# goruck/radar-ml

Hardware: AMD Instinct MI355X
Metric: radar frames/s (3D-proj->SVM) (higher is better)
Workload: dtype f32 volumes -> u8 codes, i8 MFMA (exact int32 dot), f64 epilogue; 1 GPU; configs[2]: max-projection + RBF-SVM decision_function, 3-class, 2562 SVs, batch 65536 frames/GPU of 64x64x128 f32 resident in HBM; parallelism=single GPU, global_frames=65536

## Files before the change

include/radarml.h:

```cpp
#ifndef RADARML_H
#define RADARML_H

#include <stdint.h>
#include <stddef.h>

#ifdef __cplusplus
extern "C" {
#endif

typedef enum rml_status {
    RML_OK = 0,
    RML_ERR_INVALID = -1,
    RML_ERR_UNSUPPORTED = -2,
    RML_ERR_HIP = -3,
    RML_ERR_NOMEM = -4,
    RML_ERR_STATE = -5
} rml_status;

typedef struct rml_ctx rml_ctx;
typedef struct rml_svm rml_svm;
typedef struct rml_linear rml_linear;

#define RML_MODE_MAX   0
#define RML_MODE_SLICE 1
#define RML_MODE_SUM   2
#define RML_MODE_MAX_NAN 3

#define RML_VOL_F32    0
#define RML_VOL_U8     1

#define RML_MASK_XZ 1u
#define RML_MASK_YZ 2u
#define RML_MASK_XY 4u
#define RML_MASK_ALL 7u

#define RML_KERNEL_RBF    0
#define RML_KERNEL_LINEAR 1

#define RML_PATH_AUTO  0
#define RML_PATH_F32   1
#define RML_PATH_I8    2
#define RML_PATH_F64   3
#define RML_PATH_DIGITS 4

const char* rml_version(void);
const char* rml_last_error(void);

int rml_ctx_create(int device, rml_ctx** out);
int rml_ctx_destroy(rml_ctx* ctx);
int rml_ctx_device(const rml_ctx* ctx);

#define RML_OPT_PROJECT_SHARE_CU 1
#define RML_OPT_WAVEFRAME 2
#define RML_OPT_LINPLANE 3
#define RML_OPT_STAGE_CODES 4
#define RML_OPT_SLICE_WAVE 5
#define RML_OPT_DERIVE_FUSED 6
#define RML_OPT_CODE_RMW 7
#define RML_OPT_GEMM_BIG 8
#define RML_OPT_CHUNK 9
#define RML_OPT_C1_PK 10
#define RML_OPT_SMO_LDS_ROWS 11
#define RML_SMO_LDS_ROWS_MAX 2768
#define RML_OPT_SGD_RESIDENT_D 12
#define RML_SGD_RESIDENT_D_MAX 10240
#define RML_OPT_CONV7 13
#define RML_CONV7_DEFAULT 3
#define RML_OPT_ZOOM_ROWS 14
int rml_ctx_set_option(rml_ctx* ctx, int option, int value);
int rml_ctx_get_option(const rml_ctx* ctx, int option, int* value);

int rml_ctx_reserve_workspace(rml_ctx* ctx, int64_t bytes);
int64_t rml_ctx_workspace_bytes(const rml_ctx* ctx);

int rml_profile_enable(rml_ctx* ctx, int on);
int rml_profile_read(rml_ctx* ctx, int64_t* launches, double* total_ms, int64_t* frames);
int rml_profile_read_gemm(rml_ctx* ctx, int64_t* launches, double* total_ms, double* ops);

int rml_probe_stream(rml_ctx* ctx, const void* buf, int64_t bytes, int reps, double* gb_per_s, void* stream);

int rml_code_rmw_default(int64_t D, int64_t frame_bytes, int derive, int u8);

int64_t rml_feature_len(int X, int Y, int Z, uint32_t mask);

int rml_project(rml_ctx* ctx, const void* V, int vdtype, int64_t B, int X, int Y, int Z, int mode,
                const int32_t* ijk, float scale_div, uint32_t mask,
                float* feat, int64_t ld_feat,
                uint8_t* feat_q, int64_t ld_q, int32_t* row_isum, int64_t* row_isq, int32_t* row_flags,
                void* stream);

int rml_project_slices(rml_ctx* ctx, const void* V, int vdtype, int64_t B, int X, int Y, int Z, int T,
                       const int32_t* ijk, float scale_div, uint32_t mask,
                       float* feat, int64_t ld_feat,
                       uint8_t* feat_q, int64_t ld_q, int32_t* row_isum, int64_t* row_isq, int32_t* row_flags,
                       void* stream);

int rml_project_planes(rml_ctx* ctx, const void* V, int vdtype, int64_t B, int X, int Y, int Z, int mode,
                       const int32_t* ijk, float* xz, float* yz, float* xy, void* stream);

int rml_derive_targets(rml_ctx* ctx, const void* V, int vdtype, int64_t B, int X, int Y, int Z,
                       int num_targets, int32_t* ijk, float* profiles, void* stream);

int rml_derive_slice(rml_ctx* ctx, const void* V, int vdtype, int64_t B, int X, int Y, int Z, int num_targets,
                     int32_t* ijk, float* profiles, float scale_div, uint32_t mask,
                     float* feat, int64_t ld_feat,
                     uint8_t* feat_q, int64_t ld_q, int32_t* row_isum, int64_t* row_isq, int32_t* row_flags,
                     void* stream);
int rml_derive_slice_supported(const rml_ctx* ctx, const void* V, int vdtype, int X, int Y, int Z, int num_targets);

int rml_assemble_features(rml_ctx* ctx, const float* xz, const float* yz, const float* xy,
                          int64_t B, int X, int Y, int Z, float scale_div, uint32_t mask,
                          float* feat, int64_t ld_feat, void* stream);

int rml_zoom_features(rml_ctx* ctx, const float* xz, const float* yz, const float* xy,
                      int64_t B, int X, int Y, int Z, const int32_t* out_shape,
                      float scale_div, uint32_t mask, float* feat, int64_t ld_feat, void* stream);

int rml_project_zoom(rml_ctx* ctx, const void* V, int vdtype, int64_t B, int X, int Y, int Z, int mode, const int32_t* ijk, int T,
                     const int32_t* out_shape, float scale_div, uint32_t mask, float* feat, int64_t ld_feat, void* stream);

int rml_quantize_rows(rml_ctx* ctx, const float* feat, int64_t N, int64_t D, int64_t ld_feat,
                      float scale_div, uint8_t* feat_q, int64_t ld_q,
                      int32_t* row_isum, int64_t* row_isq, int32_t* row_flags, void* stream);

int rml_svm_load(rml_ctx* ctx, const double* sv, int64_t M, int64_t D,
                 const double* dual_coef, const double* intercept, const int32_t* n_support,
                 int n_classes, int kernel, double gamma, double code_scale ,
                 const double* calib_a, const double* calib_b, rml_svm** out);
int rml_svm_free(rml_ctx* ctx, rml_svm* m);
int rml_svm_is_exact(const rml_svm* m);
int64_t rml_svm_num_sv(const rml_svm* m);
int64_t rml_svm_dim(const rml_svm* m);

int rml_svm_decision(rml_ctx* ctx, const rml_svm* m, int path,
// ... 277 lines not shown
```

radar-ml_amd/_lib.py:

```python
import ctypes as C
import os
import threading

HERE = os.path.dirname(os.path.abspath(__file__))
LIB_PATH = os.environ.get("RML_LIB") or os.path.join(HERE, "libradarml_hip.so")


class RadarMLError(RuntimeError):
    pass


_lib = None
_lock = threading.RLock()
_ctx = {}

c_void_p, c_int, c_int64, c_uint32, c_uint64, c_float, c_double = (
    C.c_void_p, C.c_int, C.c_int64, C.c_uint32, C.c_uint64, C.c_float, C.c_double)

SIGNATURES = {
    "rml_version": (C.c_char_p, []),
    "rml_last_error": (C.c_char_p, []),
    "rml_ctx_create": (c_int, [c_int, C.POINTER(c_void_p)]),
    "rml_ctx_destroy": (c_int, [c_void_p]),
    "rml_ctx_device": (c_int, [c_void_p]),
# ... 105 lines not shown
                                  c_void_p, c_void_p, c_float, c_int, c_void_p, c_void_p, c_int64, c_void_p]),
    "rml_dense_tail_lrelu_f32": (c_int, [c_void_p, c_void_p, c_int64, c_int64, c_int64, c_void_p, c_void_p, c_void_p, c_void_p, c_void_p,
                                         c_void_p, c_int, c_float, c_void_p, c_int64, c_void_p, c_void_p]),
    "rml_dnn_train_supported":(c_int, [c_int, c_int, c_int]),
    "rml_dnn_train_workspace_bytes": (c_int64, [c_int, c_int, c_int, c_int]),
    "rml_dnn_train_step": (c_int, [c_void_p, c_void_p, c_void_p, c_void_p, c_void_p, c_void_p, c_int, c_int64, c_int, c_int, c_void_p, c_int,
                                   c_void_p, c_void_p, c_int, c_uint64, c_int64, c_float, c_int, c_void_p, c_int64, c_void_p, c_void_p,
                                   c_void_p, c_void_p]),
    "rml_dnn_dropout_mask": (c_int, [c_uint64, c_int64, c_int, c_int, c_int, c_float, c_void_p]),
    "rml_bn_workspace_floats": (c_int64, [c_void_p, c_int]),
    "rml_bn_lrelu_pad_forward": (c_int, [c_void_p, c_void_p, c_int, c_int64, c_int, c_int, c_int, c_int, c_int, c_void_p, c_void_p,
                                         c_float, c_float, c_float, c_void_p, c_void_p, c_void_p, c_void_p, c_void_p, c_void_p, c_void_p]),
    "rml_bn_lrelu_pad_backward": (c_int, [c_void_p, c_void_p, c_void_p, c_int, c_int64, c_int, c_int, c_int, c_int, c_int, c_void_p,
                                          c_void_p, c_void_p, c_void_p, c_float, c_void_p, c_void_p, c_void_p, c_void_p, c_void_p]),
    "rml_conv1_bn_lrelu_pad_forward": (c_int, [c_void_p, c_void_p, c_void_p, c_int, c_int64, c_int, c_int, c_int, c_int, c_int, c_void_p,
                                               c_void_p, c_float, c_float, c_float, c_void_p, c_void_p, c_void_p, c_void_p, c_void_p,
                                               c_void_p, c_void_p, c_void_p]),
    "rml_conv1_bn_lrelu_pad_backward": (c_int, [c_void_p, c_void_p, c_void_p, c_void_p, c_int, c_int64, c_int, c_int, c_int, c_int, c_int,
                                                c_void_p, c_void_p, c_void_p, c_void_p, c_void_p, c_float, c_void_p, c_void_p, c_void_p,
                                                c_void_p, c_void_p]),
    "rml_conv7_tanh_supported": (c_int, [c_int, c_int, c_int]),
    "rml_conv7_workspace_floats": (c_int64, [c_void_p, c_int64, c_int, c_int, c_int]),
    "rml_conv7_tanh_forward": (c_int, [c_void_p, c_void_p, c_int, c_int64, c_int, c_int, c_int, c_void_p, c_void_p, c_void_p, c_void_p]),
    "rml_conv7_tanh_backward": (c_int, [c_void_p, c_void_p, c_void_p, c_void_p, c_int, c_int64, c_int, c_int, c_int, c_void_p, c_void_p,
                                        c_void_p, c_void_p, c_void_p, c_void_p]),
    "rml_gen_up_supported": (c_int, [c_int, c_int, c_int]),
    "rml_gen_up_forward": (c_int, [c_void_p, c_void_p, c_int, c_int64, c_int, c_int, c_int, c_void_p, c_void_p, c_void_p, c_void_p]),
    "rml_sgan_generate_workspace_bytes": (c_int64, [c_int64, c_int, c_int, c_int]),
    "rml_sgan_generate": (c_int, [c_void_p, c_void_p, c_int64, c_int, c_int, c_int, c_int, c_int, c_void_p, c_void_p, c_void_p, c_void_p,
                                  c_void_p, c_void_p, c_void_p, c_void_p, c_void_p, c_void_p, c_int64, c_void_p]),
    "rml_conv3s2_supported": (c_int, [c_int, c_int, c_int, c_int]),
    "rml_conv3s2_workspace_bytes": (c_int64, [c_void_p, c_int64, c_int, c_int, c_int, c_int, c_int]),
    "rml_conv3s2_forward": (c_int, [c_void_p, c_void_p, c_void_p, c_int, c_int64, c_int, c_int, c_int, c_int, c_void_p, c_void_p, c_int64,
                                    c_void_p]),
    "rml_conv3s2_dgrad": (c_int, [c_void_p, c_void_p, c_void_p, c_int, c_int64, c_int, c_int, c_int, c_int, c_void_p, c_void_p, c_int64,
                                  c_void_p]),
    "rml_conv3s2_wgrad": (c_int, [c_void_p, c_void_p, c_void_p, c_int, c_int64, c_int, c_int, c_int, c_int, c_void_p, c_void_p, c_int64,
                                  c_void_p]),
    "rml_convt4s2_supported": (c_int, [c_int, c_int, c_int, c_int]),
    "rml_convt4s2_workspace_bytes": (c_int64, [c_void_p, c_int64, c_int, c_int, c_int, c_int, c_int]),
    "rml_convt4s2_forward": (c_int, [c_void_p, c_void_p, c_void_p, c_int, c_int64, c_int, c_int, c_int, c_int, c_void_p, c_void_p, c_int64,
                                     c_void_p]),
    "rml_convt4s2_dgrad": (c_int, [c_void_p, c_void_p, c_void_p, c_int, c_int64, c_int, c_int, c_int, c_int, c_void_p, c_void_p, c_int64,
                                   c_void_p]),
    "rml_convt4s2_wgrad": (c_int, [c_void_p, c_void_p, c_void_p, c_int, c_int64, c_int, c_int, c_int, c_int, c_void_p, c_void_p, c_int64,
                                   c_void_p]),
    "rml_adam_entry_bytes": (c_int, []),
    "rml_adam_step": (c_int, [c_void_p, c_void_p, c_int, c_int64, c_float, c_float, c_float, c_float, c_void_p, c_void_p, c_void_p,
                              c_void_p, c_int, c_float, c_float, c_int, c_void_p]),
    "rml_augment": (c_int, [c_void_p, c_int, c_void_p, c_int64, c_int, c_int, c_void_p, c_void_p, c_void_p]),
    "rml_augment_chain": (c_int, [c_void_p, c_int, c_void_p, c_int64, c_int64, c_int, c_int, c_float, c_float, c_float, c_float, c_void_p,
                                  c_void_p, c_void_p]),
    "rml_code_rmw_default": (c_int, [c_int64, c_int64, c_int, c_int]),
    "rml_probe_stream": (c_int, [c_void_p, c_void_p, c_int64, c_int, c_void_p, c_void_p]),
    "rml_synth_volumes": (c_int, [c_void_p, c_uint64, c_int64, c_int64, c_int, c_int, c_int, c_int, c_void_p, c_void_p,
                                  c_void_p]),
}

MODE_MAX, MODE_SLICE, MODE_SUM, MODE_MAX_NAN = 0, 1, 2, 3
OPT_PROJECT_SHARE_CU, OPT_WAVEFRAME, OPT_LINPLANE, OPT_STAGE_CODES, OPT_SLICE_WAVE, OPT_DERIVE_FUSED, OPT_CODE_RMW, OPT_GEMM_BIG, OPT_CHUNK, OPT_C1_PK, OPT_SMO_LDS_ROWS, OPT_SGD_RESIDENT_D, OPT_CONV7, OPT_ZOOM_ROWS = range(1, 15)
OPTIONS = {"project_share_cu": OPT_PROJECT_SHARE_CU, "waveframe": OPT_WAVEFRAME, "linplane": OPT_LINPLANE, "stage_codes": OPT_STAGE_CODES,
           "slice_wave": OPT_SLICE_WAVE, "derive_fused": OPT_DERIVE_FUSED, "code_rmw": OPT_CODE_RMW, "gemm_big": OPT_GEMM_BIG,
           "chunk": OPT_CHUNK, "c1_pk": OPT_C1_PK}
SOLVER_OPTIONS = {"smo_lds_rows": OPT_SMO_LDS_ROWS, "sgd_resident_d": OPT_SGD_RESIDENT_D}
NN_OPTIONS = {"conv7": OPT_CONV7}
ZOOM_OPTIONS = {"zoom_rows": OPT_ZOOM_ROWS}
SMO_LDS_ROWS_MAX = 2768
SGD_RESIDENT_D_MAX = 10240
SGD_MAX_ROWS = 8192
SGD_L1, SGD_L2, SGD_ELASTICNET = 1, 2, 3
DNN_TRAIN, DNN_EVAL = 0, 1
DNN_TRAIN_MAX_BATCH = 64
ENV_OPTIONS = {"RML_WAVE_SHARE": "project_share_cu", "RML_WAVEFRAME": "waveframe", "RML_LINPLANE": "linplane", "RML_STAGE_CODES": "stage_codes",
               "RML_SLICE_WAVE": "slice_wave", "RML_DERIVE_FUSED": "derive_fused", "RML_CODE_RMW": "code_rmw", "RML_GEMM_BIG": "gemm_big",
               "RML_CHUNK": "chunk", "RML_C1_PK": "c1_pk", "RML_SMO_LDS_ROWS": "smo_lds_rows", "RML_SGD_RESIDENT_D": "sgd_resident_d",
               "RML_CONV7": "conv7"}
AUG_ROTATE, AUG_ZOOM, AUG_NOISE = 0, 1, 2
CHAIN_ROTATE, CHAIN_ZOOM, CHAIN_NOISE = 1, 2, 4
VOL_F32, VOL_U8 = 0, 1
MODES = {"max": MODE_MAX, "slice": MODE_SLICE, "sum": MODE_SUM, "max_nan": MODE_MAX_NAN}
KERNEL_RBF, KERNEL_LINEAR = 0, 1
PATH_AUTO, PATH_F32, PATH_I8, PATH_F64, PATH_DIGITS = 0, 1, 2, 3, 4
GRAM_LINEAR, GRAM_RBF = 0, 1
PATHS = {"auto": PATH_AUTO, "f32": PATH_F32, "i8": PATH_I8, "f64": PATH_F64, "digits": PATH_DIGITS}


def option_id(name):
    name = name.lower()
    for table in (OPTIONS, SOLVER_OPTIONS, ZOOM_OPTIONS):
        if name in table:
            return table[name]
    return NN_OPTIONS[name]


def load():
    global _lib
    with _lock:
        if _lib is not None:
            return _lib
        if not os.path.exists(LIB_PATH):
            raise RadarMLError(
                "libradarml_hip.so is not built (%s missing): run `python radar-ml_amd/build.py`; "
                "there is no CPU fallback for the HIP path" % LIB_PATH)
        try:
            import torch
        except Exception:
            pass
        try:
            lib = C.CDLL(LIB_PATH, mode=C.RTLD_GLOBAL)
        except OSError as e:
            raise RadarMLError("cannot load %s: %s" % (LIB_PATH, e))
        for name, (res, args) in SIGNATURES.items():
            try:
                fn = getattr(lib, name)
            except AttributeError:
                raise RadarMLError("libradarml_hip.so does not export %s" % name)
            fn.restype = res
            fn.argtypes = args
        _lib = lib
        return lib


def check(rc, what=""):
    if rc != 0:
        msg = load().rml_last_error()
        raise RadarMLError("%s failed (status %d): %s" % (what or "radarml call", rc, msg.decode() if msg else ""))


def context(device=None):
    import torch
    if not torch.cuda.is_available():
        raise RadarMLError("no HIP device is visible: the radar-ml HIP path needs an MI355X (no CPU fallback)")
    if device is None:
        device = torch.cuda.current_device()
    elif isinstance(device, torch.device):
        device = device.index if device.index is not None else torch.cuda.current_device()
    index = int(device)
    lib = load()
    with _lock:
        h = _ctx.get(device)
    if h is None:
        new = c_void_p()
# ... 62 lines not shown
```

radar-ml_amd/csrc/context.hip:

```cpp
#include "rml_internal.h"
#include <stdarg.h>
#include <stdio.h>
#include <stdlib.h>
#include <new>

namespace {
thread_local char g_err[512] = "";
}

void rml_set_error(const char* fmt, ...) {
    va_list ap;
    va_start(ap, fmt);
    vsnprintf(g_err, sizeof(g_err), fmt, ap);
    va_end(ap);
}

int rml_hip_fail(hipError_t e, const char* what, const char* file, int line) {
    rml_set_error("HIP error %d (%s) in %s at %s:%d", (int)e, hipGetErrorString(e), what, file, line);
    return RML_ERR_HIP;
}

static void ws_release_retired(rml_ctx* ctx, bool all) {
    size_t k = 0;
    for (size_t i = 0; i < ctx->ws_retired.size(); ++i) {
// ... 82 lines not shown
    RML_HIP(hipEventRecord(ctx->ev_stage, st));
    ctx->ev_stage_valid = true;
    return RML_OK;
}

extern "C" int rml_ctx_reserve_workspace(rml_ctx* ctx, int64_t bytes) {
    RML_REQUIRE(ctx != nullptr && bytes >= 0, RML_ERR_INVALID, "rml_ctx_reserve_workspace: bad arguments");
    std::lock_guard<std::recursive_mutex> lk(ctx->mu);
    int prev = -1;
    RML_HIP(hipGetDevice(&prev));
    RML_HIP(hipSetDevice(ctx->device));
    RML_HIP(hipDeviceSynchronize());
    ws_release_retired(ctx, true);
    int rc = RML_OK;
    if ((size_t)bytes > ctx->ws_bytes) {
        if (ctx->ws) { (void)hipFree(ctx->ws); ctx->ws = nullptr; ctx->ws_bytes = 0; }
        rc = ws_grow(ctx, (size_t)bytes, nullptr, false);
    }
    if (prev >= 0) (void)hipSetDevice(prev);
    return rc;
}

extern "C" int64_t rml_ctx_workspace_bytes(const rml_ctx* ctx) { return ctx ? (int64_t)ctx->ws_bytes : 0; }

extern "C" const char* rml_version(void) { return "radarml-hip 0.1 (gfx950)"; }
extern "C" const char* rml_last_error(void) { return g_err; }

extern "C" int rml_ctx_create(int device, rml_ctx** out) {
    RML_REQUIRE(out != nullptr, RML_ERR_INVALID, "rml_ctx_create: out is NULL");
    *out = nullptr;
    int n = 0;
    RML_HIP(hipGetDeviceCount(&n));
    RML_REQUIRE(device >= 0 && device < n, RML_ERR_INVALID, "rml_ctx_create: device %d out of range (%d devices)", device, n);
    struct restore_device {
        int prev = -1;
        restore_device() { if (hipGetDevice(&prev) != hipSuccess) { (void)hipGetLastError(); prev = -1; } }
        ~restore_device() { if (prev >= 0) (void)hipSetDevice(prev); }
    } restore;
    RML_HIP(hipSetDevice(device));
    hipDeviceProp_t prop;
    RML_HIP(hipGetDeviceProperties(&prop, device));
    rml_ctx* c = new (std::nothrow) rml_ctx();
    RML_REQUIRE(c != nullptr, RML_ERR_NOMEM, "rml_ctx_create: out of host memory");
    c->device = device;
    c->num_cu = prop.multiProcessorCount;
    hipError_t e = hipStreamCreateWithFlags(&c->aux_stream, hipStreamNonBlocking);
    if (e == hipSuccess) e = hipEventCreateWithFlags(&c->ev_fork, hipEventDisableTiming);
    if (e == hipSuccess) e = hipEventCreateWithFlags(&c->ev_join, hipEventDisableTiming);
    if (e == hipSuccess) e = hipEventCreateWithFlags(&c->ev_last, hipEventDisableTiming);
    for (int i = 0; i < 2 && e == hipSuccess; ++i) {
        e = hipEventCreateWithFlags(&c->ev_proj[i], hipEventDisableTiming);
        if (e == hipSuccess) e = hipEventCreateWithFlags(&c->ev_done[i], hipEventDisableTiming);
    }
    if (e != hipSuccess) {
        delete c;
        return rml_hip_fail(e, "stream/event creation", __FILE__, __LINE__);
    }
    *out = c;
    return RML_OK;
}

extern "C" int rml_ctx_destroy(rml_ctx* ctx) {
    if (!ctx) return RML_OK;
    int prev = -1;
    if (hipGetDevice(&prev) != hipSuccess) { (void)hipGetLastError(); prev = -1; }
    (void)hipSetDevice(ctx->device);
    (void)hipDeviceSynchronize();
    ws_release_retired(ctx, true);
    if (ctx->ws) (void)hipFree(ctx->ws);
    if (ctx->ev_fork) (void)hipEventDestroy(ctx->ev_fork);
    if (ctx->ev_join) (void)hipEventDestroy(ctx->ev_join);
    if (ctx->ev_last) (void)hipEventDestroy(ctx->ev_last);
    if (ctx->ev_stage) (void)hipEventDestroy(ctx->ev_stage);
    if (ctx->stage) (void)hipHostFree(ctx->stage);
    for (int i = 0; i < 2; ++i) {
        if (ctx->ev_proj[i]) (void)hipEventDestroy(ctx->ev_proj[i]);
        if (ctx->ev_done[i]) (void)hipEventDestroy(ctx->ev_done[i]);
    }
    for (hipEvent_t e : ctx->prof_ev) (void)hipEventDestroy(e);
    for (hipEvent_t e : ctx->prof_ev_g) (void)hipEventDestroy(e);
    for (const rml_resize_tab& t : ctx->resize_tabs) (void)hipFree(const_cast<double*>(t.kk));
    for (const rml_pre_tab& t : ctx->pre_tabs) (void)hipFree(t.dev);
    if (ctx->aux_stream) (void)hipStreamDestroy(ctx->aux_stream);
    delete ctx;
    if (prev >= 0) (void)hipSetDevice(prev);
    return RML_OK;
}

static bool stream_is_capturing(hipStream_t st) {
    hipStreamCaptureStatus cs = hipStreamCaptureStatusNone;
    if (hipStreamIsCapturing(st, &cs) != hipSuccess) (void)hipGetLastError();
    return cs != hipStreamCaptureStatusNone;
}

void rml_prof_mark(rml_ctx* ctx, hipStream_t st) {
    if (!ctx->profiling || stream_is_capturing(st)) return;
    if (ctx->prof_used == ctx->prof_ev.size()) {
        hipEvent_t e;
        if (hipEventCreate(&e) != hipSuccess) { (void)hipGetLastError(); return; }
        ctx->prof_ev.push_back(e);
    }
    (void)hipEventRecord(ctx->prof_ev[ctx->prof_used++], st);
}

void rml_prof_mark_gemm(rml_ctx* ctx, hipStream_t st) {
    if (!ctx->profiling || stream_is_capturing(st)) return;
    if (ctx->prof_used_g == ctx->prof_ev_g.size()) {
        hipEvent_t e;
        if (hipEventCreate(&e) != hipSuccess) { (void)hipGetLastError(); return; }
        ctx->prof_ev_g.push_back(e);
    }
    (void)hipEventRecord(ctx->prof_ev_g[ctx->prof_used_g++], st);
}

extern "C" int rml_profile_read_gemm(rml_ctx* ctx, int64_t* launches, double* total_ms, double* ops) {
    RML_REQUIRE(ctx != nullptr, RML_ERR_INVALID, "rml_profile_read_gemm: ctx is NULL");
    std::lock_guard<std::recursive_mutex> lk(ctx->mu);
    RML_HIP(hipSetDevice(ctx->device));
    double tot = 0.0;
    int64_t n = 0;
    for (size_t i = 0; i + 1 < ctx->prof_used_g; i += 2) {
        RML_HIP(hipEventSynchronize(ctx->prof_ev_g[i + 1]));
        float ms = 0.0f;
        RML_HIP(hipEventElapsedTime(&ms, ctx->prof_ev_g[i], ctx->prof_ev_g[i + 1]));
        tot += ms;
        ++n;
    }
    if (launches) *launches = n;
    if (total_ms) *total_ms = tot;
    if (ops) *ops = ctx->prof_ops_g;
    ctx->prof_used_g = 0;
    ctx->prof_ops_g = 0.0;
    return RML_OK;
}

extern "C" int rml_profile_enable(rml_ctx* ctx, int on) {
    RML_REQUIRE(ctx != nullptr, RML_ERR_INVALID, "rml_profile_enable: ctx is NULL");
    std::lock_guard<std::recursive_mutex> lk(ctx->mu);
    ctx->profiling = on != 0;
    ctx->prof_used = 0;
    ctx->prof_frames = 0;
    ctx->prof_used_g = 0;
    ctx->prof_ops_g = 0.0;
    return RML_OK;
}

extern "C" int rml_profile_read(rml_ctx* ctx, int64_t* launches, double* total_ms, int64_t* frames) {
    RML_REQUIRE(ctx != nullptr, RML_ERR_INVALID, "rml_profile_read: ctx is NULL");
    std::lock_guard<std::recursive_mutex> lk(ctx->mu);
    RML_HIP(hipSetDevice(ctx->device));
    double tot = 0.0;
    int64_t n = 0;
    for (size_t i = 0; i + 1 < ctx->prof_used; i += 2) {
        RML_HIP(hipEventSynchronize(ctx->prof_ev[i + 1]));
        float ms = 0.0f;
        RML_HIP(hipEventElapsedTime(&ms, ctx->prof_ev[i], ctx->prof_ev[i + 1]));
        tot += ms;
        ++n;
    }
    if (launches) *launches = n;
    if (total_ms) *total_ms = tot;
    if (frames) *frames = ctx->prof_frames;
    ctx->prof_used = 0;
    ctx->prof_frames = 0;
    return RML_OK;
}

extern "C" int rml_ctx_device(const rml_ctx* ctx) { return ctx ? ctx->device : RML_ERR_INVALID; }

static int* opt_slot(rml_opts& o, int option) {
    switch (option) {
        case RML_OPT_PROJECT_SHARE_CU: return &o.project_share_cu;
        case RML_OPT_WAVEFRAME: return &o.waveframe;
        case RML_OPT_LINPLANE: return &o.linplane;
        case RML_OPT_STAGE_CODES: return &o.stage_codes;
        case RML_OPT_SLICE_WAVE: return &o.slice_wave;
        case RML_OPT_DERIVE_FUSED: return &o.derive_fused;
        case RML_OPT_CODE_RMW: return &o.code_rmw;
        case RML_OPT_GEMM_BIG: return &o.gemm_big;
        case RML_OPT_C1_PK: return &o.c1_pk;
        default: return nullptr;
    }
}

extern "C" int rml_ctx_set_option(rml_ctx* ctx, int option, int value) {
    RML_REQUIRE(ctx != nullptr, RML_ERR_INVALID, "rml_ctx_set_option: ctx is NULL");
    std::lock_guard<std::recursive_mutex> lk(ctx->mu);
    if (option == RML_OPT_SMO_LDS_ROWS) {
        RML_REQUIRE(value >= 0 && value <= RML_SMO_LDS_ROWS_MAX, RML_ERR_INVALID, "rml_ctx_set_option: RML_OPT_SMO_LDS_ROWS is 0..%d rows",
                    RML_SMO_LDS_ROWS_MAX);
        ctx->opt.smo_lds_rows = value;
        return RML_OK;
    }
    if (option == RML_OPT_SGD_RESIDENT_D) {
        RML_REQUIRE(value >= 0 && value <= RML_SGD_RESIDENT_D_MAX, RML_ERR_INVALID, "rml_ctx_set_option: RML_OPT_SGD_RESIDENT_D is 0..%d "
                    "features", RML_SGD_RESIDENT_D_MAX);
        ctx->opt.sgd_resident_d = value;
        return RML_OK;
    }
    if (option == RML_OPT_CONV7) {
        RML_REQUIRE(value >= 0 && value <= 3, RML_ERR_INVALID, "rml_ctx_set_option: RML_OPT_CONV7 is 0..3 (bit 0 forward, bit 1 backward)");
        ctx->opt.conv7 = value;
        return RML_OK;
    }
    if (option == RML_OPT_ZOOM_ROWS) {
        RML_REQUIRE(value >= 0 && value <= 2, RML_ERR_INVALID, "rml_ctx_set_option: RML_OPT_ZOOM_ROWS is 0 (by LDS size), 1 (whole row) or 2 (plane by plane)");
        ctx->opt.zoom_rows = value;
        return RML_OK;
    }
    if (option == RML_OPT_CHUNK) {
        RML_REQUIRE(value == 0 || value >= 128, RML_ERR_INVALID, "rml_ctx_set_option: RML_OPT_CHUNK is 0 (automatic) or >= 128 rows");
        ctx->opt.chunk = value;
        return RML_OK;
    }
    int* slot = opt_slot(ctx->opt, option);
    RML_REQUIRE(slot != nullptr, RML_ERR_INVALID, "rml_ctx_set_option: unknown option %d", option);
    switch (option) {
        case RML_OPT_WAVEFRAME: RML_REQUIRE(value >= 0 && value <= 3, RML_ERR_INVALID, "rml_ctx_set_option: RML_OPT_WAVEFRAME is 0..3"); *slot = value; break;
        case RML_OPT_CODE_RMW: case RML_OPT_GEMM_BIG: *slot = value < 0 ? -1 : (value ? 1 : 0); break;
        default: *slot = value ? 1 : 0;
    }
    return RML_OK;
}

extern "C" int rml_ctx_get_option(const rml_ctx* ctx, int option, int* value) {
    RML_REQUIRE(ctx != nullptr && value != nullptr, RML_ERR_INVALID, "rml_ctx_get_option: NULL argument");
    rml_ctx* c = const_cast<rml_ctx*>(ctx);
    std::lock_guard<std::recursive_mutex> lk(c->mu);
    if (option == RML_OPT_CHUNK) { *value = (int)c->opt.chunk; return RML_OK; }
    if (option == RML_OPT_SMO_LDS_ROWS) { *value = c->opt.smo_lds_rows; return RML_OK; }
    if (option == RML_OPT_SGD_RESIDENT_D) { *value = c->opt.sgd_resident_d; return RML_OK; }
    if (option == RML_OPT_CONV7) { *value = c->opt.conv7; return RML_OK; }
    if (option == RML_OPT_ZOOM_ROWS) { *value = c->opt.zoom_rows; return RML_OK; }
    const int* slot = opt_slot(c->opt, option);
    RML_REQUIRE(slot != nullptr, RML_ERR_INVALID, "rml_ctx_get_option: unknown option %d", option);
    *value = *slot;
    return RML_OK;
}

namespace {
typedef float probe_v4 __attribute__((ext_vector_type(4)));
__global__ __launch_bounds__(256) void k_probe_stream(const probe_v4* __restrict__ src, int64_t n16, float* sink) {
    constexpr int PF = 16;
    const int64_t piece = (int64_t)256 * PF;
    probe_v4 m = {-INFINITY, -INFINITY, -INFINITY, -INFINITY};
    for (int64_t base = (int64_t)blockIdx.x * piece; base < n16; base += (int64_t)gridDim.x * piece) {
        probe_v4 v[PF];
#pragma unroll
        for (int u = 0; u < PF; ++u) {
            int64_t q = base + (int64_t)u * 256 + threadIdx.x;
            q = q < n16 ? q : n16 - 1;
            v[u] = __builtin_nontemporal_load(src + q);
        }
#pragma unroll
        for (int u = 0; u < PF; ++u) {
            m.x = fmaxf(m.x, v[u].x); m.y = fmaxf(m.y, v[u].y); m.z = fmaxf(m.z, v[u].z); m.w = fmaxf(m.w, v[u].w);
        }
    }
    const float r = fmaxf(fmaxf(m.x, m.y), fmaxf(m.z, m.w));
    if (r == 12345.678f) sink[blockIdx.x] = r;
}
}

extern "C" int rml_probe_stream(rml_ctx* ctx, const void* buf, int64_t bytes, int reps, double* gb_per_s, void* stream) {
    RML_REQUIRE(ctx && buf && gb_per_s, RML_ERR_INVALID, "rml_probe_stream: NULL argument");
    RML_REQUIRE(bytes >= (1 << 20) && reps >= 1 && (reinterpret_cast<uintptr_t>(buf) & 15) == 0, RML_ERR_INVALID,
                "rml_probe_stream: needs a 16-byte aligned buffer of at least 1 MiB and reps >= 1");
    RML_HIP(hipSetDevice(ctx->device));
    hipStream_t st = static_cast<hipStream_t>(stream);
    rml_ctx_guard guard(ctx, st);
    void* sink = nullptr;
    int rc = rml_ws_reserve(ctx, (size_t)4 * 2 * ctx->num_cu, &sink, st);
// ... 32 lines not shown
```

radar-ml_amd/csrc/mfma_tile.h:

```cpp
#pragma once
#include <stdint.h>
#include <hip/hip_runtime.h>

namespace {

typedef int v4i __attribute__((ext_vector_type(4)));
typedef float v4f __attribute__((ext_vector_type(4)));
typedef int v16i __attribute__((ext_vector_type(16)));
typedef float v16f __attribute__((ext_vector_type(16)));
typedef double v4d __attribute__((ext_vector_type(4)));

constexpr int kTile = 128;
constexpr int kStepBytes = 128;
constexpr int kTileBytes = kTile * kStepBytes;
constexpr int PATH_I8 = 0, PATH_F32 = 1, PATH_F64 = 2;

__device__ __forceinline__ void glds16(const void* g, void* l) {
    __builtin_amdgcn_global_load_lds((const __attribute__((address_space(1))) void*)g,
                                     (__attribute__((address_space(3))) void*)l, 16, 0, 0);
}

template <bool CLAMP>
__device__ __forceinline__ const uint8_t* stage_src(const uint8_t* base, int64_t ld, int64_t row0, int64_t rows, int wave, int q, int lane) {
    const int s = (wave * 4 + q) * 64 + lane;
    const int r = s >> 3;
    const int c = (s & 7) ^ ((r >> 1) & 7);
    int64_t gr = row0 + r;
    if (CLAMP) gr = gr < rows ? gr : rows - 1;
    return base + gr * ld + c * 16;
}

struct TileStager {
    const uint8_t* ga[4];
    const uint8_t* gb[4];
    int wave;
    template <bool CLAMP_B>
    __device__ __forceinline__ void init(const uint8_t* a, int64_t lda, int64_t a0, const uint8_t* b, int64_t ldb, int64_t b0, int64_t b_rows,
                                         int wave_, int lane) {
        wave = wave_;
#pragma unroll
        for (int q = 0; q < 4; ++q) {
            ga[q] = stage_src<false>(a, lda, a0, 0, wave, q, lane);
            gb[q] = stage_src<CLAMP_B>(b, ldb, b0, b_rows, wave, q, lane);
        }
    }
    __device__ __forceinline__ void stage(unsigned char* smem, int kt, int buf) const {
        unsigned char* base = smem + buf * 2 * kTileBytes;
        const int64_t ko = (int64_t)kt * kStepBytes;
#pragma unroll
        for (int q = 0; q < 4; ++q) {
            glds16(ga[q] + ko, base + (wave * 4 + q) * 1024);
            glds16(gb[q] + ko, base + kTileBytes + (wave * 4 + q) * 1024);
        }
    }
};

template <class KStep>
__device__ __forceinline__ void tile_k_loop(const TileStager& sg, unsigned char* smem, int kt0, int kt1, KStep kstep) {
    sg.stage(smem, kt0, 0);
    for (int kt = kt0; kt < kt1; ++kt) {
        __syncthreads();
        if (kt + 1 < kt1) sg.stage(smem, kt + 1, (kt + 1 - kt0) & 1);
        const unsigned char* sA = smem + ((kt - kt0) & 1) * 2 * kTileBytes;
        kstep(sA, sA + kTileBytes);
    }
}

template <int T>
struct Frag32 {
    int off[T], sw[T];
    __device__ __forceinline__ void init(int row0, int lane) {
#pragma unroll
        for (int t = 0; t < T; ++t) {
            const int r = row0 + t * 32 + (lane & 31);
            off[t] = r * kStepBytes; sw[t] = (r >> 1) & 7;
        }
    }
    __device__ __forceinline__ v4i read(const unsigned char* img, int t, int ch) const {
        return *reinterpret_cast<const v4i*>(img + off[t] + ((ch ^ sw[t]) << 4));
    }
};

struct Frag64 {
    int off[4], sw[4];
    __device__ __forceinline__ void init(int row0, int lane) {
#pragma unroll
        for (int t = 0; t < 4; ++t) {
            const int r = row0 + t * 16 + (lane & 15);
            off[t] = r * kStepBytes; sw[t] = (r >> 1) & 7;
        }
    }
    __device__ __forceinline__ v4f read(const unsigned char* img, int t, int ch) const {
        return *reinterpret_cast<const v4f*>(img + off[t] + ((ch ^ sw[t]) << 4));
    }
};

__device__ __forceinline__ int cd32_row(int row0, int r, int lane) { return row0 + (r & 3) + 8 * (r >> 2) + 4 * (lane >> 5); }
__device__ __forceinline__ int cd32_col(int col0, int lane) { return col0 + (lane & 31); }
__device__ __forceinline__ int cd64_row(int row0, int r, int lane) { return row0 + (lane >> 4) + 4 * r; }
__device__ __forceinline__ int cd64_col(int col0, int lane) { return col0 + (lane & 15); }

template <int PATH, class Acc>
__device__ __forceinline__ void kstep_32(Acc (&acc)[2][2], const unsigned char* sA, const unsigned char* sB, const Frag32<2>& fa,
                                         const Frag32<2>& fb, int chalf) {
    v4i af[2][2], bf[2][2];
#pragma unroll
    for (int t = 0; t < 2; ++t) {
        af[0][t] = fa.read(sA, t, chalf);
        bf[0][t] = fb.read(sB, t, chalf);
    }
#pragma unroll
    for (int kk = 0; kk < 4; ++kk) {
        if (kk < 3) {
            const int ch = 2 * (kk + 1) + chalf;
#pragma unroll
            for (int t = 0; t < 2; ++t) {
                af[(kk + 1) & 1][t] = fa.read(sA, t, ch);
                bf[(kk + 1) & 1][t] = fb.read(sB, t, ch);
            }
        }
// ... 76 lines not shown
```

radar-ml_amd/csrc/project.hip:

```cpp
#include "project_shared.h"

namespace {

using namespace rmlproj;

template <typename VT, int MODE, int LPR, int NM, bool FULL, bool PRED>
__global__ __launch_bounds__(kThreads) void k_project_fast(ProjParams a) {
    extern __shared__ __align__(16) float lds[];
    if constexpr (PRED) { if (*a.o.skip_if_set) return; }
    const int X = a.X, Y = a.Y, Z = a.Z, ZQ = a.ZQ;
    float* xz_lds = lds;
    float* xy_lds = lds + (size_t)X * Z;
    int64_t* red = reinterpret_cast<int64_t*>(xy_lds + (((size_t)X * Y + 3) & ~(size_t)3));

    constexpr int RPW = 64 / LPR;
    constexpr int NSLOT = 4 * RPW;
    const int tid = threadIdx.x, lane = tid & 63, wave = tid >> 6;
    const int slot = wave * RPW + lane / LPR;
    const int kq = lane % LPR;
    const bool act = FULL || (kq < ZQ);
    const int64_t b = blockIdx.x;
    typedef typename Quad<VT>::T QT;
    const QT* __restrict__ Vb = reinterpret_cast<const QT*>(static_cast<const VT*>(a.V) + b * (int64_t)X * Y * Z);

// ... 241 lines not shown
                    if constexpr (j < NY) {
                        float4 v = buf[u & 1][r];
                        if constexpr (MODE == RML_MODE_SUM) v = (act && j < Y) ? v : id4;
                        yz[j] = op4_raw<MODE>(yz[j], v);
                        asm volatile("" : "+v"(yz[j].x), "+v"(yz[j].y), "+v"(yz[j].z), "+v"(yz[j].w));
                        xz = op4_raw<MODE>(xz, v);
                        xyl[j * kXyStride + lane] = op_raw<MODE>(op_raw<MODE>(v.x, v.y), op_raw<MODE>(v.z, v.w));
                    }
                });
                asm volatile("" : "+v"(xz.x), "+v"(xz.y), "+v"(xz.z), "+v"(xz.w));
                __builtin_amdgcn_sched_barrier(0);
                if constexpr (g == NG - 1) {
                    const int i = ci + (NG == 1 ? u : 0);
                    int lane_e = lane;
                    asm volatile("" : "+v"(lane_e));
                    for (int off = ZQr; off < ZQ; off <<= 1) {
                        float4 o;
                        o.x = __shfl_xor(xz.x, off); o.y = __shfl_xor(xz.y, off); o.z = __shfl_xor(xz.z, off); o.w = __shfl_xor(xz.w, off);
                        xz = op4<MODE>(xz, o);
                    }
                    if (lane_e < ZQr) em.put4(0, (int64_t)i * Zr + 4 * lane_e, xz);
                    for (int jr = lane_e; jr < Yr; jr += 64) {
                        const float* rowp = xyl + (jr / RPL) * kXyStride + (jr % RPL) * ZQr;
                        float m = id;
                        for (int q = 0; q < ZQr; q += 4) {
                            const float4 t = *reinterpret_cast<const float4*>(rowp + q);
                            m = Op<MODE>::f(m, Op<MODE>::f(Op<MODE>::f(t.x, t.y), Op<MODE>::f(t.z, t.w)));
                        }
                        em.put1(2, (int64_t)i * Yr + jr, m);
                    }
                    xz = id4;
                }
            });
        }
        int lane_f = lane, Y_f = Y;
        asm volatile("" : "+v"(lane_f), "+s"(Y_f));
        const bool act_f = lane_f < ZQ;
        static_for<NY>([&](auto jc) {
            constexpr int j = decltype(jc)::value;
            if (j < Y_f && act_f) em.put4(1, (int64_t)j * Z + 4 * lane_f, yz[j]);
        });
        em.flush_wave(lane_f);
        em.finish_wave(lane_f);
    }
}

template <typename VT, int MODE, int NY, int G>
void launch_wave(const ProjParams& pp_in, int num_cu, hipStream_t st) {
    ProjParams pp = pp_in;
    constexpr int per_cu_max = (NY + 2 * G) * 4 + 40 > 256 ? 1 : 2;
    const size_t mine = (size_t)4 * NY * 68 * sizeof(float);
    pp.stage_bytes = code_stage_bytes(pp, sizeof(VT));
    if (mine + (size_t)4 * pp.stage_bytes > 160 * 1024) pp.stage_bytes = 0;
    const size_t stage = (size_t)4 * pp.stage_bytes;
    int per_cu = pp.o.share_cu ? 1 : per_cu_max;
    if (per_cu * (mine + stage) > 160 * 1024) per_cu = 1;
    const int64_t want = (pp.B + 3) / 4;
    const int64_t cap = (int64_t)num_cu * per_cu;
    dim3 grid((unsigned)(want < cap ? want : cap)), block(kThreads);
    size_t pad = stage;
    if (pp.o.share_cu && per_cu == 1 && !pp.o.no_pad && mine + stage < 81 * 1024) pad = 81 * 1024 - mine;
    if (pp.o.skip_if_set) {
        RML_MAX_DYN_LDS(160 * 1024 - (int)mine, &k_project_wave<VT, MODE, NY, G, true>);
        hipLaunchKernelGGL((k_project_wave<VT, MODE, NY, G, true>), grid, block, pad, st, pp);
    } else {
        RML_MAX_DYN_LDS(160 * 1024 - (int)mine, &k_project_wave<VT, MODE, NY, G, false>);
        hipLaunchKernelGGL((k_project_wave<VT, MODE, NY, G, false>), grid, block, pad, st, pp);
    }
}

int wave_kernel_rpl(int ZQ, int Y) {
    if (ZQ > 32 && ZQ <= 64) return Y <= 32 ? 1 : 0;
    if (ZQ == 32 || ZQ == 16) {
        const int rpl = 64 / ZQ;
        return (Y % rpl == 0 && Y / rpl <= 32) ? rpl : 0;
    }
    return 0;
}

bool wave_kernel_wanted(int ZQ, int Y, bool share_cu, int64_t B, int num_cu, int knob) {
    if (B < 2 * (int64_t)num_cu) return false;
    const int rpl = wave_kernel_rpl(ZQ, Y);
    if (knob == 0 || rpl == 0) return false;
    return rpl == 1 || share_cu || knob == 3;
}

template <typename VT, int MODE>
bool try_launch_wave(const ProjParams& pp_in, int num_cu, hipStream_t st) {
    const int knob = pp_in.k_waveframe;
    if (!wave_kernel_wanted(pp_in.ZQ, pp_in.Y, pp_in.o.share_cu != 0, pp_in.B, num_cu, knob)) return false;
    ProjParams pp = pp_in;
    pp.rpl = wave_kernel_rpl(pp.ZQ, pp.Y);
    const int Y = pp.Y / wave_kernel_rpl(pp.ZQ, pp.Y);
    const bool quarter = knob == 2 || (pp.X & 1) || pp.o.share_cu;
#define RML_WAVE_CASE(NYV)                                                                     \
    { if (quarter) launch_wave<VT, MODE, NYV, (NYV + 3) / 4>(pp, num_cu, st);                 \
      else launch_wave<VT, MODE, NYV, NYV>(pp, num_cu, st); return true; }
    if (Y <= 8) RML_WAVE_CASE(8)
    if (Y <= 16) RML_WAVE_CASE(16)
    if (Y <= 24) RML_WAVE_CASE(24)
    if (Y == 31) RML_WAVE_CASE(31)
    RML_WAVE_CASE(32)
#undef RML_WAVE_CASE
}

template <typename VT, int MODE>
// ... 141 lines not shown
    } else {
        RML_MAX_DYN_LDS(160 * 1024, &k_project_rowgroup<VT, MODE, NM, false>);
        hipLaunchKernelGGL((k_project_rowgroup<VT, MODE, NM, false>), grid, block, lds_bytes, st, pp, R);
    }
}

int gcd_int(int a, int b) { while (b) { int t = a % b; a = b; b = t; } return a; }

template <typename VT, int MODE>
int launch_mode(const ProjParams& pp, int num_cu, hipStream_t st, bool* used_fast) {
    const int X = pp.X, Y = pp.Y, Z = pp.Z;
    *used_fast = false;
    if constexpr (sizeof(VT) == 1 && MODE == RML_MODE_MAX) {
        if (try_launch_u8_max(pp, st)) { *used_fast = true; return 0; }
    }
    bool fast_ok = (Z % 4 == 0) && (Z / 4 <= 64) && ((reinterpret_cast<uintptr_t>(pp.V) & (4 * sizeof(VT) - 1)) == 0);
    size_t lds_bytes = ((size_t)X * Z + (((size_t)X * Y + 3) & ~(size_t)3)) * 4 + 64 * 8;
    if (lds_bytes > 150 * 1024) fast_ok = false;
    if constexpr (sizeof(VT) == 4) {
        if (fast_ok && wave_kernel_wanted(pp.ZQ, pp.Y, pp.o.share_cu != 0, pp.B, num_cu, pp.k_waveframe) && try_launch_lin(pp, MODE, num_cu, st)) {
            *used_fast = true;
            return 0;
        }
    }
    if (fast_ok && try_launch_wave<VT, MODE>(pp, num_cu, st)) { *used_fast = true; return 0; }
    if (fast_ok && (Z / 4) != next_pow2(Z / 4) && (Z / 4) >= 8) {
        const int zq = Z / 4;
        int R = 64 / gcd_int(zq, 64);
        while (R * zq < 512 && 2 * R * zq <= 1024 && 2 * R <= Y) R *= 2;
        if (R * zq <= 1024) {
            const int nm = (Y + R - 1) / R;
            if (nm <= 2) { launch_rowgroup<VT, MODE, 2>(pp, R, lds_bytes, st); *used_fast = true; return 0; }
            if (nm <= 4) { launch_rowgroup<VT, MODE, 4>(pp, R, lds_bytes, st); *used_fast = true; return 0; }
            if (nm <= 8) { launch_rowgroup<VT, MODE, 8>(pp, R, lds_bytes, st); *used_fast = true; return 0; }
        }
    }
    if (fast_ok) {
        int zq = Z / 4;
        int lpr = next_pow2(zq); if (lpr < 16) lpr = 16;
        int nslot = 4 * (64 / lpr);
        int nm = (Y + nslot - 1) / nslot;
        int rc = 1;
        if (lpr == 16) rc = launch_fast_nm<VT, MODE, 16>(pp, nm, lds_bytes, st);
        else if (lpr == 32) rc = launch_fast_nm<VT, MODE, 32>(pp, nm, lds_bytes, st);
        else rc = launch_fast_nm<VT, MODE, 64>(pp, nm, lds_bytes, st);
        if (rc == 0) { *used_fast = true; return 0; }
    }
    hipLaunchKernelGGL((k_project_generic<VT, MODE>), dim3((unsigned)pp.B), dim3(kThreads), 0, st, pp);
    return 0;
}

void fill_params(ProjParams& pp, const rml_ctx* ctx, const void* V, int64_t B, int X, int Y, int Z, const int32_t* ijk, const ProjOut& o) {
    pp.V = V; pp.B = B; pp.X = X; pp.Y = Y; pp.Z = Z; pp.ZQ = Z / 4; pp.ijk = ijk; pp.tpf = 1; pp.rpl = 1; pp.o = o;
    pp.ntgt = 1; pp.ijk_out = nullptr; pp.profiles = nullptr; pp.wave_lds = 0; pp.stage_bytes = 0;
    const rml_opts def;
    const rml_opts& op = ctx ? ctx->opt : def;
    pp.k_waveframe = op.waveframe; pp.k_linplane = op.linplane; pp.k_stage_codes = op.stage_codes; pp.k_slice_wave = op.slice_wave;
    pp.k_derive_fused = op.derive_fused;
    if (op.project_share_cu) pp.o.share_cu = 1;
    for (int pl = 0; pl < 3; ++pl)
        pp.vec_ok[pl] = o.p[pl] && ((reinterpret_cast<uintptr_t>(o.p[pl]) & 15) == 0) && (o.stride[pl] % 4 == 0);
}

}

namespace {
template <typename VT>
int launch_project_t(const ProjParams& pp, int mode, int num_cu, hipStream_t st) {
    bool fast = false;
    if (mode == RML_MODE_MAX) launch_mode<VT, RML_MODE_MAX>(pp, num_cu, st, &fast);
    else if (mode == RML_MODE_SUM) launch_mode<VT, RML_MODE_SUM>(pp, num_cu, st, &fast);
    else if (mode == RML_MODE_SLICE) {
        RML_REQUIRE(pp.ijk != nullptr, RML_ERR_INVALID, "rml_project: mode SLICE needs ijk");
        if (!try_launch_slice(pp, (int)sizeof(VT), st))
            hipLaunchKernelGGL(k_project_slice<VT>, dim3((unsigned)pp.B), dim3(kThreads), 0, st, pp);
    } else {
        RML_REQUIRE(false, RML_ERR_INVALID, "rml_project: unknown mode %d", mode);
    }
    return RML_OK;
}
}

bool rml_project_uses_wave_kernel(const rml_ctx* ctx, int vdtype, int mode, int X, int Y, int Z, bool share_cu, int64_t B) {
    (void)X;
    const int num_cu = ctx ? ctx->num_cu : 256, knob = ctx ? ctx->opt.waveframe : 1;
    if (mode != RML_MODE_MAX && mode != RML_MODE_SUM) return false;
    if (vdtype == RML_VOL_U8 && mode == RML_MODE_MAX && Z % 16 == 0) return false;
    return Z % 4 == 0 && wave_kernel_wanted(Z / 4, Y, share_cu, B, num_cu, knob);
}

int rml_launch_project(rml_ctx* ctx, const void* V, int vdtype, int64_t B, int X, int Y, int Z, int mode,
                       const int32_t* ijk, const ProjOut& o, hipStream_t st, int targets_per_frame) {
    if (B == 0) return RML_OK;
    RML_REQUIRE(vdtype == RML_VOL_F32 || vdtype == RML_VOL_U8, RML_ERR_INVALID, "rml_project: unknown volume dtype %d", vdtype);
    if (mode == RML_MODE_MAX_NAN) mode = RML_MODE_MAX;
    RML_REQUIRE(targets_per_frame == 1 || mode == RML_MODE_SLICE, RML_ERR_INVALID, "rml_project: several targets per frame only in mode SLICE");
    ProjParams pp;
    fill_params(pp, ctx, V, B, X, Y, Z, ijk, o);
    pp.tpf = targets_per_frame;
    const int num_cu = !ctx ? 256 : ctx->num_cu;
    const int rc = vdtype == RML_VOL_U8 ? launch_project_t<uint8_t>(pp, mode, num_cu, st) : launch_project_t<float>(pp, mode, num_cu, st);
    if (rc) return rc;
    RML_HIP(hipGetLastError());
    return RML_OK;
}

namespace {
constexpr int kFinalThreads = 1024;
__global__ __launch_bounds__(kFinalThreads) void k_project_finalize(ProjParams a, const float* __restrict__ scr, int S, int Xs, int64_t ldv) {
    __shared__ int64_t red[64];
    const int X = a.X, Y = a.Y, Z = a.Z;
    const int64_t b = blockIdx.x;
    const float* __restrict__ fr = scr + b * S * ldv;
    const int64_t oyz = (int64_t)Xs * Z, oxy = oyz + (int64_t)Y * Z;
    Emitter em(a, b);
    em.rmw = false;
    const int tid = threadIdx.x;
    for (int idx = tid; idx < (X * Z) >> 2; idx += kFinalThreads) {
        const int i = (idx * 4) / Z, k = idx * 4 - i * Z, s = i / Xs;
        em.put4(0, (int64_t)idx * 4, *reinterpret_cast<const float4*>(fr + s * ldv + (int64_t)(i - s * Xs) * Z + k));
    }
    for (int idx = tid; idx < (Y * Z) >> 2; idx += kFinalThreads) {
        const float* __restrict__ q0 = fr + oyz + (int64_t)idx * 4;
        float4 v = *reinterpret_cast<const float4*>(q0);
        for (int s0 = 1; s0 < S; s0 += 8) {
            float4 t[8];
#pragma unroll
            for (int u = 0; u < 8; ++u) t[u] = *reinterpret_cast<const float4*>(q0 + (int64_t)(s0 + u < S ? s0 + u : 0) * ldv);
#pragma unroll
            for (int u = 0; u < 8; ++u) v = op4<RML_MODE_MAX>(v, t[u]);
        }
        em.put4(1, (int64_t)idx * 4, v);
    }
    const int nxy = X * Y;
    if ((Y & 3) == 0) {
        for (int idx = tid; idx < nxy >> 2; idx += kFinalThreads) {
            const int i = (idx * 4) / Y, j = idx * 4 - i * Y, s = i / Xs;
            em.put4(2, (int64_t)idx * 4, *reinterpret_cast<const float4*>(fr + s * ldv + oxy + (int64_t)(i - s * Xs) * Y + j));
        }
    } else {
        for (int idx = tid; idx < nxy >> 2; idx += kFinalThreads) {
            float v[4];
#pragma unroll
            for (int e = 0; e < 4; ++e) {
                const int t = idx * 4 + e, i = t / Y, j = t - i * Y, s = i / Xs;
                v[e] = fr[s * ldv + oxy + (int64_t)(i - s * Xs) * Y + j];
            }
            em.put4(2, (int64_t)idx * 4, make_float4(v[0], v[1], v[2], v[3]));
        }
        for (int t = (nxy & ~3) + tid; t < nxy; t += kFinalThreads) {
            const int i = t / Y, j = t - i * Y, s = i / Xs;
            em.put1(2, t, fr[s * ldv + oxy + (int64_t)(i - s * Xs) * Y + j]);
        }
    }
    em.finish(red);
// ... 132 lines not shown
                RML_ERR_INVALID, "rml_derive_slice: feat_q needs ld_q >= D, ld_q %% 4 == 0 and 4-byte alignment");
    RML_HIP(hipSetDevice(ctx->device));
    hipStream_t st = static_cast<hipStream_t>(stream);
    ProjOut o{};
    rows_out(o, X, Y, Z, mask, scale_div, feat, ld_feat, feat_q, ld_q, row_isum, row_isq, row_flags);
    int rc = rml_launch_derive_slice(ctx, V, vdtype, B, X, Y, Z, num_targets, ijk, profiles, o, st);
    if (rc != RML_ERR_UNSUPPORTED) return rc;
    rml_ctx_guard guard(ctx, st);
    int32_t* ijk_w = ijk;
    if (!ijk_w) {
        const size_t planes = (size_t)B * ((size_t)X * Z + (size_t)Y * Z) * sizeof(float);
        void* ws = nullptr;
        rc = rml_ws_reserve(ctx, planes + (size_t)B * num_targets * 3 * sizeof(int32_t), &ws, st);
        if (rc) return rc;
        ijk_w = reinterpret_cast<int32_t*>(static_cast<unsigned char*>(ws) + planes);
    }
    rc = derive_two_kernels(ctx, V, vdtype, B, X, Y, Z, num_targets, ijk_w, profiles, st);
    if (rc) return rc;
    return rml_launch_project(ctx, V, vdtype, B * num_targets, X, Y, Z, RML_MODE_SLICE, ijk_w, o, st, num_targets);
}

static int project_rows(rml_ctx* ctx, const void* V, int vdtype, int64_t B, int X, int Y, int Z, int mode, int tpf,
                        const int32_t* ijk, float scale_div, uint32_t mask,
                        float* feat, int64_t ld_feat, uint8_t* feat_q, int64_t ld_q,
                        int32_t* row_isum, int64_t* row_isq, int32_t* row_flags, void* stream) {
    RML_REQUIRE(ctx && B >= 0 && X > 0 && Y > 0 && Z > 0, RML_ERR_INVALID, "rml_project: bad arguments");
    if (B == 0) return RML_OK;
    RML_REQUIRE(V != nullptr, RML_ERR_INVALID, "rml_project: V is NULL");
    RML_REQUIRE((mask & RML_MASK_ALL) != 0, RML_ERR_INVALID, "rml_project: empty projection mask");
    RML_REQUIRE(B < (int64_t)1 << 31, RML_ERR_UNSUPPORTED, "rml_project: B too large for one launch");
    const int64_t D = rml_feature_len(X, Y, Z, mask);
    RML_REQUIRE(!feat || ld_feat >= D, RML_ERR_INVALID, "rml_project: ld_feat < D");
    RML_REQUIRE(!feat_q || (ld_q >= D && ld_q % 4 == 0 && (reinterpret_cast<uintptr_t>(feat_q) & 3) == 0),
                RML_ERR_INVALID, "rml_project: feat_q needs ld_q >= D, ld_q %% 4 == 0 and 4-byte alignment");
    RML_HIP(hipSetDevice(ctx->device));
    ProjOut o{};
    int64_t off = 0;
    for (int pl = 0; pl < 3; ++pl) {
        if (mask & (1u << pl)) {
            o.p[pl] = feat ? feat + off : nullptr;
            o.stride[pl] = ld_feat;
            o.q[pl] = feat_q ? feat_q + off : nullptr;
            off += plane_len(pl, X, Y, Z);
        }
    }
    o.sel = mask & RML_MASK_ALL;
    o.qstride = ld_q;
    o.qrow = feat_q; o.qD = D;
    o.row_isum = row_isum; o.row_isq = row_isq; o.row_flags = row_flags;
    o.scale_div = scale_div;
    return rml_launch_project(ctx, V, vdtype, B, X, Y, Z, mode, ijk, o, static_cast<hipStream_t>(stream), tpf);
}

extern "C" int rml_project_planes(rml_ctx* ctx, const void* V, int vdtype, int64_t B, int X, int Y, int Z, int mode,
                                  const int32_t* ijk, float* xz, float* yz, float* xy, void* stream) {
    RML_REQUIRE(ctx && B >= 0 && X > 0 && Y > 0 && Z > 0, RML_ERR_INVALID, "rml_project_planes: bad arguments");
    if (B == 0) return RML_OK;
    RML_REQUIRE(V != nullptr, RML_ERR_INVALID, "rml_project_planes: V is NULL");
    RML_REQUIRE(B < (int64_t)1 << 31, RML_ERR_UNSUPPORTED, "rml_project_planes: B too large for one launch");
    RML_HIP(hipSetDevice(ctx->device));
    ProjOut o{};
    o.p[0] = xz; o.stride[0] = (int64_t)X * Z;
    o.p[1] = yz; o.stride[1] = (int64_t)Y * Z;
    o.p[2] = xy; o.stride[2] = (int64_t)X * Y;
    o.sel = (xz ? 1u : 0u) | (yz ? 2u : 0u) | (xy ? 4u : 0u);
    o.scale_div = 0.0f;
    return rml_launch_project(ctx, V, vdtype, B, X, Y, Z, mode, ijk, o, static_cast<hipStream_t>(stream));
}

extern "C" int rml_derive_targets(rml_ctx* ctx, const void* V, int vdtype, int64_t B, int X, int Y, int Z,
                                  int num_targets, int32_t* ijk, float* profiles, void* stream) {
    RML_REQUIRE(ctx && B >= 0 && X > 0 && Y > 0 && Z > 0, RML_ERR_INVALID, "rml_derive_targets: bad arguments");
    if (B == 0) return RML_OK;
    RML_REQUIRE(V && ijk, RML_ERR_INVALID, "rml_derive_targets: NULL argument");
    RML_REQUIRE(num_targets >= 1 && num_targets <= X && num_targets <= Y && num_targets <= Z, RML_ERR_INVALID,
                "rml_derive_targets: num_targets out of range");
    RML_HIP(hipSetDevice(ctx->device));
    if (B == 0) return RML_OK;
    hipStream_t st = static_cast<hipStream_t>(stream);
    ProjOut none{};
    int rc1 = rml_launch_derive_slice(ctx, V, vdtype, B, X, Y, Z, num_targets, ijk, profiles, none, st);
    if (rc1 != RML_ERR_UNSUPPORTED) return rc1;
    rml_ctx_guard guard(ctx, st);
    return derive_two_kernels(ctx, V, vdtype, B, X, Y, Z, num_targets, ijk, profiles, st);
}

static int derive_two_kernels(rml_ctx* ctx, const void* V, int vdtype, int64_t B, int X, int Y, int Z, int num_targets, int32_t* ijk,
                              float* profiles, hipStream_t st) {
    size_t need = (size_t)B * ((size_t)X * Z + (size_t)Y * Z) * sizeof(float);
    void* ws = nullptr;
    int rc = rml_ws_reserve(ctx, need, &ws, st);
    if (rc) return rc;
    return derive_two_kernels_at(ctx, V, vdtype, B, X, Y, Z, num_targets, ijk, profiles, static_cast<float*>(ws), st);
}

static int derive_two_kernels_at(rml_ctx* ctx, const void* V, int vdtype, int64_t B, int X, int Y, int Z, int num_targets, int32_t* ijk,
                                 float* profiles, float* xzs, hipStream_t st) {
    int rc;
    float* yzs = xzs + (size_t)B * X * Z;
    ProjOut o{};
    o.p[0] = xzs; o.stride[0] = (int64_t)X * Z;
    o.p[1] = yzs; o.stride[1] = (int64_t)Y * Z;
    o.sel = 3u;
    o.scale_div = 0.0f;
    rc = rml_launch_project(ctx, V, vdtype, B, X, Y, Z, RML_MODE_SUM, nullptr, o, st);
    if (rc) return rc;
// ... 54 lines not shown
```

radar-ml_amd/csrc/project_lin.hip:

```cpp
#include "project_shared.h"

namespace {

using namespace rmlproj;

template <int MODE, int ZQ4, int NI, int RG, int NGRP, int NMASK, bool PRED>
__global__ __launch_bounds__(256, 2) void k_project_lin(ProjParams a) {
    if constexpr (PRED) { if (*a.o.skip_if_set) return; }
    static_assert(NGRP % 2 == 0 && RG % 8 == 0 && NMASK >= 1 && NMASK <= NGRP,
                  "an even number of groups per plane (the row buffers alternate statically); xz folds 8 rows per wait");
    constexpr int NT = NI * NGRP;
    const int X = a.X, Y = a.Y, Z = a.Z, ZQ = a.ZQ;
    const int lane = threadIdx.x & 63;
    const int wave = __builtin_amdgcn_readfirstlane(threadIdx.x >> 6);
    const int64_t stride = (int64_t)gridDim.x * 4;
    int64_t cf = (int64_t)blockIdx.x * 4 + wave;
    if (cf >= a.B) return;
    const float4* __restrict__ Vall = reinterpret_cast<const float4*>(a.V);
    const int pq = Y * ZQ;
    const int64_t fq = (int64_t)X * pq;
    const float id = Op<MODE>::ident();
    const float4 id4 = make_float4(id, id, id, id);
    extern __shared__ __align__(16) unsigned char lin_smem[];
    float4* img = reinterpret_cast<float4*>(lin_smem) + wave * (NI * 64);
// ... 60 lines not shown
                {
                    int lane_x = lane;
                    asm volatile("" : "+v"(lane_x));
                    const float4* col = img + (lane_x < ZQ ? lane_x : ZQ - 1);
                    static_for<RG / 8>([&](auto hc) {
                        constexpr int h = decltype(hc)::value;
                        float4 c8[8];
                        static_for<8>([&](auto rc) { constexpr int r = decltype(rc)::value; c8[r] = col[(h * 8 + r) * ZQ]; });
                        __builtin_amdgcn_sched_barrier(0);
                        static_for<8>([&](auto rc) { constexpr int r = decltype(rc)::value; xz = op4_raw<MODE>(xz, c8[r]); });
                        __builtin_amdgcn_sched_barrier(0);
                    });
                    asm volatile("" : "+v"(xz.x), "+v"(xz.y), "+v"(xz.z), "+v"(xz.w));
                }
                if constexpr (g == NGRP - 1) {
                    int lane_e = lane;
                    asm volatile("" : "+v"(lane_e));
                    if (lane_e < ZQ) em.put4(0, (int64_t)ci * Z + 4 * lane_e, xz);
                    if (lane_e < Y) {
                        const float* rowp = xyl + lane_e * ZQ;
                        float m = id;
                        float4 r4[ZQ4];
                        static_for<ZQ4>([&](auto qc) { constexpr int q = decltype(qc)::value; r4[q] = *reinterpret_cast<const float4*>(rowp + 4 * q); });
                        static_for<ZQ4>([&](auto qc) {
                            constexpr int q = decltype(qc)::value;
                            m = Op<MODE>::f(m, Op<MODE>::f(Op<MODE>::f(r4[q].x, r4[q].y), Op<MODE>::f(r4[q].z, r4[q].w)));
                        });
                        em.put1(2, (int64_t)ci * Y + lane_e, m);
                    }
                    xz = id4;
                }
                __builtin_amdgcn_sched_barrier(0);
            });
        }
        int lane_f = lane, pq_f = pq;
        asm volatile("" : "+v"(lane_f), "+s"(pq_f));
        static_for<NT>([&](auto tc) {
            constexpr int t = decltype(tc)::value;
            const int q = t * 64 + lane_f;
            if (q < pq_f) em.put4(1, (int64_t)q * 4, yz[t]);
        });
        em.flush_wave(lane_f);
        em.finish_wave(lane_f);
    }
}

template <int MODE, int ZQ4, int NI, int RG, int NGRP, int NMASK>
void launch_lin(const ProjParams& pp_in, int num_cu, hipStream_t st) {
    ProjParams pp = pp_in;
    pp.stage_bytes = code_stage_bytes(pp, 4);
    constexpr size_t kMaxLds = 160 * 1024;
    const size_t images = (size_t)4 * (NI * 64 * 16 + NI * NGRP * 64 * 4);
    if (images + (size_t)4 * pp.stage_bytes > kMaxLds) pp.stage_bytes = 0;
    const size_t mine = images + (size_t)4 * pp.stage_bytes;
    int per_cu = pp.o.share_cu ? 1 : 2;
    if (per_cu * mine > 160 * 1024) per_cu = 1;
    const int64_t want = (pp.B + 3) / 4;
    const int64_t cap = (int64_t)num_cu * per_cu;
    dim3 grid((unsigned)(want < cap ? want : cap)), block(kThreads);
    const size_t lds = (pp.o.share_cu && per_cu == 1 && !pp.o.no_pad && mine < 81 * 1024) ? 81 * 1024 : mine;
    if (pp.o.skip_if_set) {
        RML_MAX_DYN_LDS(kMaxLds, &k_project_lin<MODE, ZQ4, NI, RG, NGRP, NMASK, true>);
        hipLaunchKernelGGL((k_project_lin<MODE, ZQ4, NI, RG, NGRP, NMASK, true>), grid, block, lds, st, pp);
    } else {
        RML_MAX_DYN_LDS(kMaxLds, &k_project_lin<MODE, ZQ4, NI, RG, NGRP, NMASK, false>);
        hipLaunchKernelGGL((k_project_lin<MODE, ZQ4, NI, RG, NGRP, NMASK, false>), grid, block, lds, st, pp);
    }
}

template <int ZQ>
bool launch_lin8(const ProjParams& pp, int num_cu, hipStream_t st) {
    if (pp.Y > 8 && pp.Y <= 16) { launch_lin<RML_MODE_MAX, ZQ / 4, ZQ / 8, 8, 2, 1>(pp, num_cu, st); return true; }
    if (pp.Y > 16 && pp.Y <= 32) { launch_lin<RML_MODE_MAX, ZQ / 4, ZQ / 8, 8, 4, 2>(pp, num_cu, st); return true; }
    return false;
}

}

namespace rmlproj {

bool try_launch_lin(const ProjParams& pp, int mode, int num_cu, hipStream_t st) {
    if (pp.Z != 4 * pp.ZQ) return false;
    if (pp.B < 2 * (int64_t)num_cu) return false;
    if (!pp.k_linplane) return false;
    if (pp.ZQ == 44) {
        if (pp.Y <= 16 || pp.Y > 32) return false;
        if (mode == RML_MODE_MAX) launch_lin<RML_MODE_MAX, 11, 11, 16, 2, 1>(pp, num_cu, st);
        else if (mode == RML_MODE_SUM) launch_lin<RML_MODE_SUM, 11, 11, 16, 2, 1>(pp, num_cu, st);
        else return false;
        return true;
    }
    if (mode != RML_MODE_MAX) return false;
    if (pp.ZQ == 40) return launch_lin8<40>(pp, num_cu, st);
    if (pp.ZQ == 48) return launch_lin8<48>(pp, num_cu, st);
    if (pp.ZQ == 56) return launch_lin8<56>(pp, num_cu, st);
    return false;
}

}
```

radar-ml_amd/csrc/project_shared.h:

```cpp
#pragma once
#include "rml_internal.h"
#include <math.h>
#include <stdlib.h>
#include <type_traits>

namespace rmlproj {

constexpr int kThreads = 256;

struct ProjParams {
    const void* V;
    int64_t B;
    int X, Y, Z, ZQ;
    const int32_t* ijk;
    int tpf;
    int rpl;
    ProjOut o;
    int vec_ok[3];
    int ntgt;
    int32_t* ijk_out;
    float* profiles;
    int wave_lds;
    int stage_bytes;
    int k_waveframe, k_linplane, k_stage_codes, k_slice_wave, k_derive_fused;
};

template <int MODE> struct Op;
template <> struct Op<RML_MODE_MAX> {
    static __device__ __forceinline__ float ident() { return -INFINITY; }
    static __device__ __forceinline__ float f(float a, float b) { return __builtin_elementwise_maximum(a, b); }
    static __device__ __forceinline__ uint32_t key(float v) {
        const uint32_t b = __float_as_uint(v);
        const uint32_t k = b ^ ((uint32_t)((int32_t)b >> 31) | 0x80000000u);
        return v != v ? 0xFFFFFFFFu : k;
    }
    static __device__ __forceinline__ float lds_ident() { return __uint_as_float(key(-INFINITY)); }
    static __device__ __forceinline__ float lds_value(float stored) {
        const uint32_t k = __float_as_uint(stored);
        const uint32_t b = (k & 0x80000000u) ? (k ^ 0x80000000u) : ~k;
        return k == 0xFFFFFFFFu ? __uint_as_float(0x7FC00000u) : __uint_as_float(b);
    }
    static __device__ __forceinline__ void lds_atomic(float* p, float v) {
        __hip_atomic_fetch_max(reinterpret_cast<uint32_t*>(p), key(v), __ATOMIC_RELAXED, __HIP_MEMORY_SCOPE_WORKGROUP);
    }
};
template <> struct Op<RML_MODE_SUM> {
    static __device__ __forceinline__ float ident() { return 0.0f; }
    static __device__ __forceinline__ float f(float a, float b) { return a + b; }
    static __device__ __forceinline__ float lds_ident() { return 0.0f; }
    static __device__ __forceinline__ float lds_value(float stored) { return stored; }
    static __device__ __forceinline__ void lds_atomic(float* p, float v) {
        __hip_atomic_fetch_add(p, v, __ATOMIC_RELAXED, __HIP_MEMORY_SCOPE_WORKGROUP);
    }
};

template <int MODE> __device__ __forceinline__ float4 op4(float4 a, float4 b) {
    return make_float4(Op<MODE>::f(a.x, b.x), Op<MODE>::f(a.y, b.y), Op<MODE>::f(a.z, b.z), Op<MODE>::f(a.w, b.w));
}

__device__ __forceinline__ float4 bytes_to_float4(uint32_t w) {
    return make_float4((float)(w & 0xFFu), (float)((w >> 8) & 0xFFu), (float)((w >> 16) & 0xFFu), (float)(w >> 24));
}

struct Emitter {
    const ProjParams& a;
    int64_t b;
    __device__ __forceinline__ int64_t qb() const { return b; }
    int32_t isum = 0;
    uint32_t isq = 0;
    int ok = 1;
    double nsq = 0.0;
    bool want_stats;
    bool rmw;
    typedef __attribute__((address_space(3))) uint8_t lds_u8;
    typedef __attribute__((address_space(3))) uint32_t lds_u32;
    typedef uint32_t u32x4 __attribute__((ext_vector_type(4)));
    typedef __attribute__((address_space(3))) u32x4 lds_u128;
    lds_u8* stage = nullptr;
    int staged = 0;
    int stage_xy = 0;
    __device__ __forceinline__ void set_stage(unsigned char* p, int xy_off) { stage = (lds_u8*)p; staged = 1; stage_xy = xy_off; }

    __device__ Emitter(const ProjParams& a_, int64_t b_) : a(a_), b(b_) {
        want_stats = a.o.row_isum || a.o.row_isq || a.o.row_flags || a.o.q[0] || a.o.q[1] || a.o.q[2];
        rmw = a.o.q_rmw != 0;
    }
    __device__ __forceinline__ float scaled(float v) const {
        return (a.o.scale_div > 1.0f) ? __fdiv_rn(v, a.o.scale_div) : v;
    }
    __device__ __forceinline__ uint32_t code(float v) {
        int c = (int)v;
        bool good = ((float)c == v) && c >= 0 && c <= 255;
        ok &= good ? 1 : 0;
        c = good ? c : 0;
        isum += c;
        isq += (uint32_t)(c * c);
        return (uint32_t)(c ^ 0x80);
    }
    __device__ __forceinline__ void put_code1(int pl, int64_t idx, int c, bool good) {
        ok &= good ? 1 : 0;
        c = good ? c : 0;
        isum += c;
        isq += (uint32_t)(c * c);
        if (a.o.q[pl]) a.o.q[pl][b * a.o.qstride + idx] = (uint8_t)(c ^ 0x80);
    }
    __device__ __forceinline__ void put1(int pl, int64_t idx, float v) {
        if (!((a.o.sel >> pl) & 1u)) return;
        if (a.o.p[pl]) a.o.p[pl][b * a.o.stride[pl] + idx] = scaled(v);
        if (a.o.row_nsq) { double t = (double)scaled(v); nsq += t * t; }
        if (want_stats) {
            uint32_t c = code(v);
            if (a.o.q[pl]) {
                if (staged && pl != 1) stage[(pl == 2 ? stage_xy : 0) + idx] = (uint8_t)c;
                else a.o.q[pl][b * a.o.qstride + idx] = (uint8_t)c;
            }
        }
    }
    __device__ __forceinline__ uint32_t old_word(int pl, int64_t idx) const {
        if (!(rmw && a.o.q[pl] && ((a.o.sel >> pl) & 1u))) return 0u;
        return *reinterpret_cast<const uint32_t*>(a.o.q[pl] + qb() * a.o.qstride + idx);
    }
    __device__ __forceinline__ uint32_t old_word_nocheck(int pl, int64_t idx) const {
        return *reinterpret_cast<const uint32_t*>(a.o.q[pl] + qb() * a.o.qstride + idx);
    }
    __device__ __forceinline__ void put_bytes4(int pl, int64_t idx, uint32_t w, bool have_old = false, uint32_t old = 0u) {
        if (!((a.o.sel >> pl) & 1u)) return;
        if (a.o.p[pl] || a.o.row_nsq) { put4(pl, idx, bytes_to_float4(w), have_old, old); return; }
        if (want_stats) {
            isum += (int32_t)__builtin_amdgcn_udot4(w, 0x01010101u, 0u, false);
            isq = __builtin_amdgcn_udot4(w, w, isq, false);
            if (a.o.q[pl]) {
                uint32_t* dq = reinterpret_cast<uint32_t*>(a.o.q[pl] + qb() * a.o.qstride + idx);
                const uint32_t nv = w ^ 0x80808080u;
                if (!rmw || (have_old ? old : *dq) != nv) *dq = nv;
            }
        }
    }
    __device__ __forceinline__ void put4(int pl, int64_t idx, float4 v, bool have_old = false, uint32_t old = 0u) {
        if (!((a.o.sel >> pl) & 1u)) return;
        if (a.o.p[pl]) {
            float* dst = a.o.p[pl] + b * a.o.stride[pl] + idx;
            float4 s = make_float4(scaled(v.x), scaled(v.y), scaled(v.z), scaled(v.w));
            if (a.o.row_nsq) {
                nsq += (double)s.x * (double)s.x + (double)s.y * (double)s.y;
                nsq += (double)s.z * (double)s.z + (double)s.w * (double)s.w;
            }
            if (a.vec_ok[pl]) {
                *reinterpret_cast<float4*>(dst) = s;
            } else {
                typedef float f32x4u __attribute__((ext_vector_type(4), aligned(4)));
                *reinterpret_cast<f32x4u*>(dst) = f32x4u{s.x, s.y, s.z, s.w};
            }
        }
        if (want_stats) {
            uint32_t c0 = code(v.x), c1 = code(v.y), c2 = code(v.z), c3 = code(v.w);
            if (a.o.q[pl]) {
                uint32_t packed = c0 | (c1 << 8) | (c2 << 16) | (c3 << 24);
                if (staged && pl != 1) *(lds_u32*)(stage + (pl == 2 ? stage_xy : 0) + idx) = packed;
                else {
                    uint32_t* dq = reinterpret_cast<uint32_t*>(a.o.q[pl] + qb() * a.o.qstride + idx);
                    if (!rmw || (have_old ? old : *dq) != packed) *dq = packed;
                }
            }
        }
    }
    __device__ __forceinline__ void reset(int64_t b_) { b = b_; isum = 0; isq = 0; ok = 1; nsq = 0.0; }
    __device__ void flush_wave(int lane) {
        if (!staged) return;
        __builtin_amdgcn_fence(__ATOMIC_ACQ_REL, "wavefront");
        const int len[2] = {a.X * a.Z, a.X * a.Y};
        lds_u8* src[2] = {stage, stage + stage_xy};
        uint8_t* dst[2] = {a.o.q[0] + qb() * a.o.qstride, a.o.q[2] + qb() * a.o.qstride};
#pragma unroll
        for (int r = 0; r < 2; ++r) {
            int done = 0;
            if ((reinterpret_cast<uintptr_t>(dst[r]) & 15) == 0) {
                for (int i = lane; i < (len[r] >> 4); i += 64) {
                    reinterpret_cast<u32x4*>(dst[r])[i] = ((lds_u128*)src[r])[i];
                }
                done = len[r] & ~15;
            }
            for (int i = done + 4 * lane; i + 4 <= len[r]; i += 256)
                *reinterpret_cast<uint32_t*>(dst[r] + i) = *(lds_u32*)(src[r] + i);
            for (int i = (len[r] & ~3) + lane; i < len[r]; i += 64) dst[r][i] = src[r][i];
        }
        __builtin_amdgcn_fence(__ATOMIC_ACQ_REL, "wavefront");
    }
    __device__ void finish_wave(int lane) {
        if (a.o.qrow) {
            for (int64_t c = a.o.qD + lane; c < a.o.qstride; c += 64) a.o.qrow[b * a.o.qstride + c] = 0;
        }
        if (a.o.prow) {
            for (int64_t c = a.o.pD + lane; c < a.o.pstride; c += 64) a.o.prow[b * a.o.pstride + c] = 0.0f;
        }
        if (!(a.o.row_isum || a.o.row_isq || a.o.row_flags || a.o.row_nsq)) return;
        int64_t s = isum, q = isq;
        int g = ok;
        double nn = nsq;
#pragma unroll
        for (int off = 32; off >= 1; off >>= 1) {
            s += __shfl_xor(s, off);
            q += __shfl_xor(q, off);
            g &= __shfl_xor(g, off);
            nn += __shfl_xor(nn, off);
        }
        if (lane == 0) {
            if (a.o.row_isum) a.o.row_isum[b] = (int32_t)s;
            if (a.o.row_isq) a.o.row_isq[b] = q;
            if (a.o.row_flags) a.o.row_flags[b] = (int32_t)g;
            if (a.o.row_nsq) a.o.row_nsq[b] = nn;
        }
    }
    __device__ void finish(int64_t* red) {
        if (a.o.qrow) {
            for (int64_t c = a.o.qD + threadIdx.x; c < a.o.qstride; c += blockDim.x) a.o.qrow[b * a.o.qstride + c] = 0;
        }
        if (a.o.prow) {
            for (int64_t c = a.o.pD + threadIdx.x; c < a.o.pstride; c += blockDim.x) a.o.prow[b * a.o.pstride + c] = 0.0f;
        }
        if (!(a.o.row_isum || a.o.row_isq || a.o.row_flags || a.o.row_nsq)) return;
        int64_t s = isum, q = isq;
        int g = ok;
        double nn = nsq;
#pragma unroll
        for (int off = 32; off >= 1; off >>= 1) {
            s += __shfl_xor(s, off);
            q += __shfl_xor(q, off);
            g &= __shfl_xor(g, off);
            nn += __shfl_xor(nn, off);
        }
        int lane = threadIdx.x & 63, wave = threadIdx.x >> 6;
        double* redd = reinterpret_cast<double*>(red + 48);
        __syncthreads();
        if (lane == 0) { red[wave * 3 + 0] = s; red[wave * 3 + 1] = q; red[wave * 3 + 2] = g; redd[wave] = nn; }
        __syncthreads();
        if (threadIdx.x == 0) {
            int64_t S = 0, Q = 0, G = 1;
            double NN = 0.0;
            for (int w = 0; w < (int)(blockDim.x + 63) / 64; ++w) { S += red[w * 3]; Q += red[w * 3 + 1]; G &= red[w * 3 + 2]; NN += redd[w]; }
// ... 19 lines not shown
template <> struct Quad<float> { typedef float4 T; };
template <> struct Quad<uint8_t> { typedef uint32_t T; };

template <int MODE, int LPR> __device__ __forceinline__ float row_reduce(float r) {
#pragma unroll
    for (int off = LPR / 2; off >= 1; off >>= 1) r = Op<MODE>::f(r, __shfl_xor(r, off));
    return r;
}

template <int CTRL, int ROW_MASK, bool BOUND>
__device__ __forceinline__ float dpp_mov(float old, float v) {
    return __int_as_float(__builtin_amdgcn_update_dpp(__float_as_int(old), __float_as_int(v), CTRL, ROW_MASK, 0xF, BOUND));
}
template <int MODE> __device__ __forceinline__ float wave_reduce_uniform(float r) {
    const float id = Op<MODE>::ident();
    r = Op<MODE>::f(r, dpp_mov<0xB1, 0xF, true>(id, r));
    r = Op<MODE>::f(r, dpp_mov<0x4E, 0xF, true>(id, r));
    r = Op<MODE>::f(r, dpp_mov<0x141, 0xF, true>(id, r));
    r = Op<MODE>::f(r, dpp_mov<0x140, 0xF, true>(id, r));
    r = Op<MODE>::f(r, dpp_mov<0x142, 0xA, false>(id, r));
    r = Op<MODE>::f(r, dpp_mov<0x143, 0xC, false>(id, r));
    return __int_as_float(__builtin_amdgcn_readlane(__float_as_int(r), 63));
}

template <int N, typename F> __device__ __forceinline__ void static_for(F&& f) {
    if constexpr (N > 0) {
        static_for<N - 1>(f);
        f(std::integral_constant<int, N - 1>{});
    }
}
template <int J> __device__ __forceinline__ float park_lane(float acc, float uniform_val) {
    asm("v_writelane_b32 %0, %1, %2" : "+v"(acc) : "s"(uniform_val), "n"(J));
    return acc;
}

template <int MODE> __device__ __forceinline__ float op_raw(float a, float b) {
    if constexpr (MODE == RML_MODE_MAX) {
        float r;
        asm("v_maximum3_f32 %0, %1, %2, %2" : "=v"(r) : "v"(a), "v"(b));
        return r;
    } else
    {
        return Op<MODE>::f(a, b);
    }
}
template <int MODE> __device__ __forceinline__ float4 op4_raw(float4 a, float4 b) {
    return make_float4(op_raw<MODE>(a.x, b.x), op_raw<MODE>(a.y, b.y), op_raw<MODE>(a.z, b.z), op_raw<MODE>(a.w, b.w));
}

inline int code_stage_bytes(const ProjParams& pp, size_t voxel_bytes) {
    const ProjOut& o = pp.o;
    if (voxel_bytes != 4 || o.p[0] || o.p[1] || o.p[2] || o.row_nsq || !o.q[0] || !o.q[2] || o.skip_if_set) return 0;
    if (!pp.k_stage_codes) return 0;
    const int bytes = ((pp.X * pp.Z + 15) & ~15) + ((pp.X * pp.Y + 15) & ~15);
    return bytes <= 16 * 1024 ? bytes : 0;
}

bool try_launch_lin(const ProjParams& pp, int mode, int num_cu, hipStream_t st);

bool try_launch_slice(const ProjParams& pp, int vbytes, hipStream_t st);
bool try_launch_derive_slice(const ProjParams& pp, int vbytes, int num_cu, hipStream_t st);
bool derive_slice_shape_ok(int X, int Y, int Z, int ntgt);

bool try_launch_u8_max(const ProjParams& pp, hipStream_t st);

}
```

radar-ml_amd/csrc/rml_internal.h:

```cpp
#pragma once
#include <hip/hip_runtime.h>
#include <stdint.h>
#include <cstdlib>
#include <atomic>
#include <mutex>
#include <string>
#include <vector>
#include "../../include/radarml.h"

struct rml_resize_tab {
    int in, out, ksize;
    const int* bounds;
    const double* kk;
};

struct rml_pre_tab {
    int X, Y, Z, OH, OW;
    void* dev;
    size_t off[6];
};

struct rml_opts {
    int project_share_cu = 0;
    int waveframe = 1;
    int linplane = 1;
    int stage_codes = 1;
    int slice_wave = 1;
    int derive_fused = 1;
    int code_rmw = -1;
    int gemm_big = -1;
    int c1_pk = 1;
    int64_t chunk = 0;
    int smo_lds_rows = RML_SMO_LDS_ROWS_MAX;
    int conv7 = RML_CONV7_DEFAULT;
    int sgd_resident_d = RML_SGD_RESIDENT_D_MAX;
    int zoom_rows = 0;
};

struct rml_ws_retired {
    void* p;
    hipEvent_t ev;
};

struct rml_ctx {
    int device = 0;
    int num_cu = 256;
    void* ws = nullptr;
    size_t ws_bytes = 0;
    std::vector<rml_ws_retired> ws_retired;
    rml_opts opt;
    hipEvent_t ev_fork = nullptr, ev_join = nullptr;
    hipEvent_t ev_proj[2] = {nullptr, nullptr}, ev_done[2] = {nullptr, nullptr};
    hipStream_t aux_stream = nullptr;
    bool profiling = false;
    std::vector<hipEvent_t> prof_ev;
    size_t prof_used = 0;
    int64_t prof_frames = 0;
    std::vector<hipEvent_t> prof_ev_g;
    size_t prof_used_g = 0;
    double prof_ops_g = 0.0;
    std::vector<rml_resize_tab> resize_tabs;
    std::vector<rml_pre_tab> pre_tabs;
    std::recursive_mutex mu;
    hipEvent_t ev_last = nullptr;
    bool ev_last_valid = false;
    void* stage = nullptr;
    size_t stage_bytes = 0;
    hipEvent_t ev_stage = nullptr;
    bool ev_stage_valid = false;
};

struct rml_ctx_guard {
    rml_ctx* ctx;
    hipStream_t st;
    bool capturing = false;
    explicit rml_ctx_guard(rml_ctx* c, hipStream_t stream) : ctx(c), st(stream) {
        ctx->mu.lock();
        hipStreamCaptureStatus cs = hipStreamCaptureStatusNone;
        if (hipStreamIsCapturing(st, &cs) != hipSuccess) (void)hipGetLastError();
        capturing = cs != hipStreamCaptureStatusNone;
        if (!capturing && ctx->ev_last_valid) (void)hipStreamWaitEvent(st, ctx->ev_last, 0);
    }
    ~rml_ctx_guard() {
        if (!capturing && ctx->ev_last && hipEventRecord(ctx->ev_last, st) == hipSuccess) ctx->ev_last_valid = true;
        ctx->mu.unlock();
    }
    rml_ctx_guard(const rml_ctx_guard&) = delete;
    rml_ctx_guard& operator=(const rml_ctx_guard&) = delete;
};

void rml_prof_mark(rml_ctx* ctx, hipStream_t st);
void rml_prof_mark_gemm(rml_ctx* ctx, hipStream_t st);

struct rml_once_per_device {
    std::atomic<uint64_t> mask{0};
    bool first(int dev) { const uint64_t bit = 1ull << (dev & 63); return !(mask.fetch_or(bit) & bit); }
};
#define RML_MAX_DYN_LDS(bytes, ...)                                                                                     \
    do {                                                                                                                \
        static rml_once_per_device _once;                                                                               \
        int _dev = 0;                                                                                                   \
        (void)hipGetDevice(&_dev);                                                                                      \
        if (_once.first(_dev))                                                                                          \
            (void)hipFuncSetAttribute(reinterpret_cast<const void*>(__VA_ARGS__), hipFuncAttributeMaxDynamicSharedMemorySize, (bytes)); \
    } while (0)

void rml_set_error(const char* fmt, ...);
int rml_hip_fail(hipError_t e, const char* what, const char* file, int line);

#define RML_HIP(call)                                                        \
    do {                                                                     \
        hipError_t _e = (call);                                              \
        if (_e != hipSuccess) return rml_hip_fail(_e, #call, __FILE__, __LINE__); \
    } while (0)

#define RML_REQUIRE(cond, status, ...)      \
    do {                                    \
        if (!(cond)) {                      \
            rml_set_error(__VA_ARGS__);     \
            return (status);                \
        }                                   \
    } while (0)

int rml_ws_reserve(rml_ctx* ctx, size_t bytes, void** out, hipStream_t st);

int rml_stage_reserve(rml_ctx* ctx, size_t bytes, void** host);
int rml_stage_upload(rml_ctx* ctx, void* dst, size_t bytes, hipStream_t st);

struct ProjOut {
    float* p[3];
    int64_t stride[3];
    uint32_t sel;
    uint8_t* q[3];
    int64_t qstride;
    uint8_t* qrow;
    int64_t qD;
    int32_t* row_isum;
    int64_t* row_isq;
    int32_t* row_flags;
    float scale_div;
    float* prow;
    int64_t pD, pstride;
    double* row_nsq;
    const int32_t* skip_if_set;
    int share_cu;
    int no_pad;
    int q_rmw;
};
inline int rml_code_rmw(int64_t D, int64_t frame_bytes, bool derive, bool u8) {
    if (derive) return 0;
    return u8 && D * 64 >= frame_bytes && D * 16 <= frame_bytes;
}

bool rml_project_uses_wave_kernel(const rml_ctx* ctx, int vdtype, int mode, int X, int Y, int Z, bool share_cu, int64_t B);

int rml_launch_project(rml_ctx* ctx, const void* V, int vdtype, int64_t B, int X, int Y, int Z, int mode,
                       const int32_t* ijk, const ProjOut& o, hipStream_t st, int targets_per_frame = 1);

constexpr int RML_SMALL_FRAMES = 8;
int rml_project_split_pieces(int X, int Y, int Z);
size_t rml_project_split_scratch_bytes(int64_t B, int X, int Y, int Z, int S);
int rml_launch_project_split(rml_ctx* ctx, const void* V, int vdtype, int64_t B, int X, int Y, int Z, const ProjOut& o, float* scratch, int S,
                             hipStream_t st);

int rml_launch_derive_slice(rml_ctx* ctx, const void* V, int vdtype, int64_t B, int X, int Y, int Z, int num_targets,
                            int32_t* ijk_out, float* profiles, const ProjOut& o, hipStream_t st);

int rml_launch_derive(rml_ctx* ctx, const void* V, int vdtype, int64_t B, int X, int Y, int Z, int num_targets, int32_t* ijk,
                      float* sums, hipStream_t st);

struct rml_zoom_plan {
    int vdtype, X, Y, Z, T; uint32_t mask; int32_t out_shape[6];
    bool codes;
    bool derive;
    int64_t Dsrc, Dout, ld_src;
    size_t lds; int by_plane;
};
int rml_zoom_plan_make(const rml_ctx* ctx, const char* who, int vdtype, int mode, int X, int Y, int Z, int T, bool derive, const int32_t* out_shape,
                       uint32_t mask, rml_zoom_plan* zp);
size_t rml_zoom_stage_bytes(const rml_zoom_plan& zp, int64_t frames);
int rml_zoom_stage_run(rml_ctx* ctx, const rml_zoom_plan& zp, void* scratch, const void* V, int64_t frames, int mode, const int32_t* ijk,
                       float scale_div, float* feat, int64_t ld_feat, int64_t pad_to, double* row_nsq, int32_t* row_flags, hipStream_t st);

struct rml_svm {
    int64_t M = 0, Mpad = 0, D = 0;
    int64_t Kq = 0;
    int64_t Kf = 0;
    int64_t Dq = 0;
    int64_t Df = 0;
    int C = 0, P = 0, PT = 0, kernel = 0;
    double gamma = 0, code_scale = 1;
    bool exact = false, has_calib = false;
    float* sv_f32 = nullptr;
    double* sv_nsq = nullptr;
    uint8_t* sv_q = nullptr;
    double* sv_term_q = nullptr;
    double* W = nullptr;
    double* intercept = nullptr;
    double* calib = nullptr;
    double* platt = nullptr;
    bool dig_ok = false;
    double dig_c0 = 0, dig_s = 1;
    int8_t* sv_dig = nullptr;
    double* sv_dig_nsq = nullptr;
    uint32_t mask_hint = 0;
};

struct rml_svm_pack {
    std::vector<double> W, nsq, term, dnsq;
    std::vector<float> svf;
    std::vector<uint8_t> svq;
    std::vector<int8_t> svd;
};
int rml_svm_pack_host(const double* sv, int64_t M, int64_t D, const double* dual_coef, const int32_t* n_support,
                      int n_classes, int kernel, double gamma, double code_scale, bool has_calib, rml_svm* m, rml_svm_pack* pk);
size_t rml_svm_ws_bytes(const rml_svm* m, int64_t CH, unsigned needs);

struct rml_linear {
    int64_t D = 0;
    int C = 0;
    bool has_calib = false;
    double* coef = nullptr;
    double* intercept = nullptr;
    double* calib = nullptr;
};
```

radar-ml_amd/csrc/svm.hip:

```cpp
#include "rml_internal.h"
#include "svm_tile.h"
#include "svm_ring.h"
#include "svm_small.h"
#include "svm_rows.h"
#include "svm_finish.h"
#include <math.h>
#include <vector>
#include <stdlib.h>
#include <type_traits>
#include <algorithm>
#include <new>

namespace {

inline bool use_dig_gemm(const rml_svm* m, int policy, int64_t n, int num_cu) {
    if (!m->dig_ok) return false;
    if (policy == RML_PATH_DIGITS) return true;
    if (policy != RML_PATH_AUTO) return false;
    const int64_t wgs = ((n + kBig - 1) / kBig) * ((m->Mpad + kBig - 1) / kBig);
    return wgs * 2 >= (int64_t)num_cu;
}

inline bool use_big_gemm(const rml_svm* m, int64_t n, int num_cu, int knob) {
    if (knob == 0 || m->PT > 6) return false;
// ... 9 lines not shown
    RML_HIP(hipMalloc(reinterpret_cast<void**>(dst), h.size() * sizeof(T)));
    RML_HIP(hipMemcpy(*dst, h.data(), h.size() * sizeof(T), hipMemcpyHostToDevice));
    return RML_OK;
}

RingArgs ring_args_from(const GemmArgs& ga) {
    RingArgs ra{};
    ra.sv = ga.sv; ra.x = ga.x; ra.ld_sv = ga.ld_sv; ra.ld_x = ga.ld_x; ra.KT = ga.KT;
    ra.N = ga.N; ra.Mpad = ga.Mpad; ra.sv_rows = ga.sv_rows; ra.ST = ga.ST; ra.FT = ga.FT;
    ra.tile_exact = ga.tile_exact; ra.want = ga.want; ra.x_isum = ga.x_isum; ra.x_isq = ga.x_isq;
    ra.sv_term = ga.sv_term; ra.W = ga.W; ra.gs = ga.gs; ra.kernel = ga.kernel; ra.partial = ga.partial; ra.Npart = ga.Npart;
    return ra;
}
int launch_gemm_big(const rml_svm* m, const GemmArgs& ga, hipStream_t st) { return launch_gemm_ring<0>(m, ring_args_from(ga), st); }
SmallArgs small_args_from(const GemmArgs& ga, int32_t* G, int64_t g_sm, int64_t g_sn) {
    SmallArgs sa{};
    sa.N = (int)ga.N; sa.Mpad = ga.Mpad; sa.tile_exact = ga.tile_exact; sa.G = G; sa.g_sm = g_sm; sa.g_sn = g_sn;
    sa.x_isum = ga.x_isum; sa.x_isq = ga.x_isq; sa.sv_term = ga.sv_term; sa.W = ga.W; sa.gs = ga.gs; sa.kernel = ga.kernel;
    sa.partial = ga.partial; sa.Npart = ga.Npart;
    return sa;
}
inline bool ring_takes(const rml_ctx* ctx, const rml_svm* m, int64_t n) { return use_big_gemm(m, n, ctx->num_cu, ctx->opt.gemm_big); }

int64_t pick_chunk_opt(const rml_ctx* ctx, int64_t fallback) { return ctx->opt.chunk >= 128 ? round_up(ctx->opt.chunk, kTile) : fallback; }
int64_t pick_chunk(const rml_ctx* ctx, const rml_svm* m, int64_t rows, int64_t fallback, bool dig) {
    const int64_t env = pick_chunk_opt(ctx, 0);
    const int num_cu = ctx->num_cu;
    int64_t ch = fallback;
    if (env) ch = env;
    else if (dig || (m->exact && ring_takes(ctx, m, 32768))) {
        const int64_t st2 = (m->Mpad + kBig - 1) / kBig;
        auto rounds = [&](int64_t n) { return n <= 0 ? (int64_t)0 : (((n + kBig - 1) / kBig) * st2 + num_cu - 1) / num_cu; };
        const int64_t total = round_up(rows, kBig);
        int64_t best = -1;
        const int64_t cmax = dig ? std::max<int64_t>(4096 / 4, std::min<int64_t>(32768, (2048 / st2) * kBig)) : 32768;
        for (int64_t c = std::min<int64_t>(4096, cmax); c <= cmax; c += kBig) {
            const int64_t nfull = total / c, rem = total % c;
            const int64_t cost = 20 * (nfull * rounds(c) + rounds(rem)) + 3 * (nfull + (rem ? 1 : 0));
            if (best < 0 || cost <= best) { best = cost; ch = c; }
            if (c >= total) break;
        }
    }
    return std::min<int64_t>(round_up(rows, kTile), ch);
}

struct ChunkWs {
    uint8_t* q; float* f32; int32_t* isum; int64_t* isq; double* nsq; int32_t* flags;
    int32_t* tile_exact; int32_t* all_exact; double* partial;
    int8_t* dig; int64_t dig_plane; double* dnsq; int32_t* dflags;
    int32_t* stash;
    int32_t* ijk;
    int32_t* gsmall;
    int32_t* gsplit;
    size_t bytes;
};

struct ChunkNeeds { bool q, f32, dig, ijk; };
constexpr int64_t kSplitRows = 2048;

ChunkWs carve(const rml_svm* m, int64_t CH, unsigned char* base, const ChunkNeeds& need) {
    ChunkWs w{}; size_t off = 0;
    auto take = [&](size_t bytes) { size_t o = off; off = (off + bytes + 255) & ~(size_t)255; return base && bytes ? base + o : (unsigned char*)nullptr; };
    w.q = (uint8_t*)take(need.q ? (size_t)CH * m->Dq : 0);
    w.f32 = (float*)take(need.f32 ? (size_t)CH * m->Df * 4 : 0);
    w.isum = (int32_t*)take((size_t)CH * 4); w.isq = (int64_t*)take((size_t)CH * 8);
    w.nsq = (double*)take((size_t)CH * 8); w.flags = (int32_t*)take((size_t)CH * 4);
    w.tile_exact = (int32_t*)take((size_t)(CH / kTile + 1) * 4); w.all_exact = (int32_t*)take(256);
    w.partial = (double*)take((size_t)(m->Mpad / kTile) * CH * m->PT * 8);
    w.dig_plane = CH * m->Dq;
    w.dig = (int8_t*)take(need.dig ? (size_t)4 * CH * m->Dq : 0);
    w.dnsq = (double*)take(need.dig ? (size_t)CH * 8 : 0); w.dflags = (int32_t*)take(need.dig ? (size_t)CH * 4 : 0);
    w.stash = (int32_t*)take(need.dig ? (size_t)ring_grid((int)((CH + kBig - 1) / kBig), (int)((m->Mpad + kBig - 1) / kBig)) * 2 * kDigStashBytes : 0);
    w.ijk = (int32_t*)take(need.ijk ? (size_t)CH * 12 : 0);
    w.gsmall = (int32_t*)take(need.q ? (size_t)RML_SMALL_FRAMES * m->Mpad * 4 : 0);
    w.gsplit = (int32_t*)take(need.q && CH <= kSplitRows ? (size_t)m->Mpad * CH * 4 : 0);
    w.bytes = off;
    return w;
}

int reserve_chunks(rml_ctx* ctx, const rml_svm* m, int64_t CH, const ChunkNeeds& need, hipStream_t st, ChunkWs* w, int nbuf,
                   size_t extra = 0, void** extra_at = nullptr) {
    const size_t each = carve(m, CH, nullptr, need).bytes;
    void* ws = nullptr;
    if (int rc = rml_ws_reserve(ctx, (size_t)nbuf * each + extra, &ws, st)) return rc;
    unsigned char* base = static_cast<unsigned char*>(ws);
    for (int i = 0; i < nbuf; ++i) w[i] = carve(m, CH, base + (size_t)i * each, need);
    if (extra_at) *extra_at = base + (size_t)nbuf * each;
    return RML_OK;
}

struct DecisionOut {
    double* dec_ovo; double* dec_ovr; double* proba; int32_t* label_vote; int32_t* label_calib;
    DecisionOut at(int64_t r0, int C, int P) const {
        auto adv = [r0](auto* p, int64_t per_row) { return p ? p + r0 * per_row : p; };
        return DecisionOut{adv(dec_ovo, P), adv(dec_ovr, C == 2 ? 1 : C), adv(proba, C), adv(label_vote, 1), adv(label_calib, 1)};
    }
};

struct ChunkOps { int64_t n; const uint8_t* q; int64_t ld_q; const int32_t* isum; const int64_t* isq; const int32_t* flags; const float* f32; const double* nsq; };
ChunkOps ws_rows(const rml_svm* m, const ChunkWs& w, int64_t n) { return ChunkOps{n, w.q, m->Dq, w.isum, w.isq, w.flags, w.f32, w.nsq}; }

struct ChunkPlan {
    int policy;
    bool tiles_done;
    bool all_exact_known;
    bool allow_big;
    bool dig_ready;
    double* kmat; int64_t ld_k;
    int FT, ST, group; bool run_i8, run_gen, gen_f32, big, run_dig, small, split;
};

ChunkPlan plan_chunk(const rml_ctx* ctx, const rml_svm* m, ChunkPlan p, const ChunkOps& x, const ChunkWs& w) {
    p.FT = (int)((x.n + kTile - 1) / kTile); p.ST = (int)(m->Mpad / kTile);
    p.run_i8 = m->exact && x.q && (p.policy == RML_PATH_AUTO || p.policy == RML_PATH_I8);
    p.run_gen = x.f32 && p.policy != RML_PATH_I8; p.gen_f32 = (p.policy == RML_PATH_F32);
    p.big = p.allow_big && p.run_i8 && !p.kmat && ring_takes(ctx, m, x.n);
    p.run_dig = p.dig_ready && w.dig && p.run_gen && !p.gen_f32 && !p.kmat && m->dig_ok;
    p.group = (p.big || p.run_dig) ? 2 : 1;
    p.small = p.run_i8 && !p.kmat && x.n <= RML_SMALL_FRAMES && w.gsmall && (m->Mpad % kSmallSv) == 0;
    p.split = p.run_i8 && !p.kmat && !p.small && !p.big && w.gsplit && x.n <= kSplitRows && (int64_t)p.FT * p.ST < ctx->num_cu &&
              m->Kq / kStepBytes >= 8;
    return p;
}

void launch_tile_flags(const rml_svm* m, const ChunkOps& x, const ChunkPlan& p, const ChunkWs& w, int32_t* all_exact, hipStream_t st) {
    const int blocks = (p.FT + p.group - 1) / p.group + (all_exact ? 1 : 0);
    hipLaunchKernelGGL(k_tile_flags, dim3(blocks), dim3(128 * p.group), 0, st, x.flags, x.n, p.FT, p.run_i8 ? (p.run_gen ? 0 : 2) : 1,
                       (int)m->exact, w.tile_exact, all_exact, p.group);
}
void launch_tile_dig(const ChunkOps& x, const ChunkPlan& p, const ChunkWs& w, hipStream_t st) {
    hipLaunchKernelGGL(k_tile_dig, dim3((p.FT + 1) / 2), dim3(256), 0, st, w.dflags, x.n, p.FT, w.tile_exact, (const int32_t*)nullptr);
}
void launch_digit_rows(const rml_svm* m, const ChunkWs& w, int64_t n, hipStream_t st) {
    hipLaunchKernelGGL(k_digit_rows, dim3((unsigned)n), dim3(256), 0, st, w.f32, m->Df, m->D, m->Dq, w.dig_plane, w.dig, w.dnsq,
                       w.dflags, m->dig_c0, 2147483648.0 / m->dig_s, (const int32_t*)nullptr);
}

int run_finish(const rml_svm* m, const ChunkOps& x, const ChunkPlan& p, const ChunkWs& w, const DecisionOut& out, hipStream_t st) {
    FinishArgs fa{};
    fa.partial = w.partial; fa.Npart = x.n; fa.ST = p.ST; fa.PT = m->PT; fa.N = x.n; fa.C = m->C; fa.P = m->P;
    fa.intercept = m->intercept; fa.calib = m->calib; fa.has_calib = m->has_calib;
    fa.row_flags = p.all_exact_known ? nullptr : x.flags; fa.tile_exact = p.all_exact_known ? nullptr : w.tile_exact;
    fa.forced_i8 = p.run_i8 && !p.run_gen;
    fa.dec_ovo = out.dec_ovo; fa.dec_ovr = out.dec_ovr; fa.proba = out.proba; fa.label_vote = out.label_vote; fa.label_calib = out.label_calib;
    hipLaunchKernelGGL(k_svm_finish, dim3((unsigned)((x.n + 255) / 256)), dim3(256), 0, st, fa);
    RML_HIP(hipGetLastError());
    return RML_OK;
}

int launch_epi(const rml_svm* m, const SmallArgs& sa, int ST, int64_t n, hipStream_t st) {
    const dim3 ge((unsigned)ST, (unsigned)n);
    switch (m->PT) {
        case 1: hipLaunchKernelGGL(k_svm_epi_small<1>, ge, dim3(128), 0, st, sa); break;
        case 3: hipLaunchKernelGGL(k_svm_epi_small<3>, ge, dim3(128), 0, st, sa); break;
        case 6: hipLaunchKernelGGL(k_svm_epi_small<6>, ge, dim3(128), 0, st, sa); break;
        case 10: hipLaunchKernelGGL(k_svm_epi_small<10>, ge, dim3(128), 0, st, sa); break;
        case 15: hipLaunchKernelGGL(k_svm_epi_small<15>, ge, dim3(128), 0, st, sa); break;
        default: RML_REQUIRE(false, RML_ERR_UNSUPPORTED, "svm: unsupported pair count");
    }
    RML_HIP(hipGetLastError());
    return RML_OK;
}

int launch_small(const rml_svm* m, const GemmArgs& ga, int32_t* G, hipStream_t st) {
    SmallArgs sa = small_args_from(ga, G, 1, ga.Mpad);
    sa.sv = ga.sv; sa.ld_sv = ga.ld_sv; sa.x = ga.x; sa.ld_x = ga.ld_x; sa.Kb = (int64_t)ga.KT * kStepBytes;
    const dim3 gd((unsigned)(ga.Mpad / kSmallSv));
    if (ga.N <= 1) hipLaunchKernelGGL(k_svm_dot_small<1>, gd, dim3(256), 0, st, sa);
    else if (ga.N <= 2) hipLaunchKernelGGL(k_svm_dot_small<2>, gd, dim3(256), 0, st, sa);
    else if (ga.N <= 4) hipLaunchKernelGGL(k_svm_dot_small<4>, gd, dim3(256), 0, st, sa);
    else hipLaunchKernelGGL(k_svm_dot_small<8>, gd, dim3(256), 0, st, sa);
    return launch_epi(m, sa, ga.ST, ga.N, st);
}

int launch_split(const rml_svm* m, const GemmArgs& ga, int32_t* G, int num_cu, hipStream_t st) {
    const int64_t ldg = (int64_t)ga.FT * kTile;
    const int64_t n16 = ga.Mpad * ldg / 4;
    hipLaunchKernelGGL(k_zero16, dim3((unsigned)((n16 + 255) / 256)), dim3(256), 0, st, reinterpret_cast<v4i*>(G), n16);
    SplitArgs sp{};
    sp.sv = ga.sv; sp.ld_sv = ga.ld_sv; sp.x = ga.x; sp.ld_x = ga.ld_x; sp.KT = ga.KT; sp.N = ga.N; sp.FT = ga.FT;
    sp.tile_exact = ga.tile_exact; sp.G = G; sp.ldg = ldg;
    const int tiles = ga.FT * ga.ST;
    int KS = (2 * num_cu + tiles - 1) / tiles;
    if (KS > ga.KT / 4) KS = ga.KT / 4;
    if (KS < 1) KS = 1;
    sp.per = (ga.KT + KS - 1) / KS;
    KS = (ga.KT + sp.per - 1) / sp.per;
    hipLaunchKernelGGL(k_svm_gemm_splitk, dim3((unsigned)tiles, (unsigned)KS), dim3(256), 0, st, sp);
    return launch_epi(m, small_args_from(ga, G, ldg, 1), ga.ST, ga.N, st);
}

RingArgs digit_args(const rml_svm* m, const ChunkOps& x, const ChunkPlan& p, const ChunkWs& w) {
    RingArgs ra{};
    ra.sv = reinterpret_cast<const uint8_t*>(m->sv_dig); ra.x = reinterpret_cast<const uint8_t*>(w.dig);
    ra.ld_sv = m->Dq; ra.ld_x = m->Dq; ra.sv_plane = m->Mpad * m->Dq; ra.x_plane = w.dig_plane;
    ra.KT = (int)(m->Kq / kStepBytes); ra.N = x.n; ra.Mpad = m->Mpad; ra.sv_rows = m->Mpad; ra.ST = p.ST; ra.FT = p.FT;
    ra.tile_exact = w.tile_exact; ra.want = 2; ra.x_nsq = w.dnsq; ra.sv_term = m->sv_dig_nsq; ra.W = m->W;
    ra.gs = m->gamma * m->dig_s * m->dig_s; ra.kernel = RML_KERNEL_RBF; ra.partial = w.partial; ra.Npart = x.n; ra.stash = w.stash;
    return ra;
}

int run_chunk(const rml_ctx* ctx, const rml_svm* m, const ChunkOps& x, const ChunkPlan& asked, const ChunkWs& w, const DecisionOut& out,
              hipStream_t st) {
    const ChunkPlan p = plan_chunk(ctx, m, asked, x, w);
    RML_REQUIRE(p.run_i8 || p.run_gen, RML_ERR_STATE, "svm: no usable operand path (model exact=%d)", (int)m->exact);
    if (!p.tiles_done) {
        launch_tile_flags(m, x, p, w, nullptr, st);
        if (p.run_dig) launch_tile_dig(x, p, w, st);
    }
    GemmArgs ga{};
    ga.N = x.n; ga.ST = p.ST; ga.FT = p.FT; ga.tile_exact = p.all_exact_known ? nullptr : w.tile_exact;
    ga.W = m->W; ga.Mpad = m->Mpad; ga.kernel = m->kernel; ga.partial = w.partial; ga.Npart = x.n;
    ga.kmat = p.kmat; ga.ld_k = p.ld_k; ga.M = m->M; ga.sv_rows = m->Mpad;
    int rc = RML_OK;
    if (p.run_i8) {
        ga.sv = m->sv_q; ga.ld_sv = m->Dq; ga.x = x.q; ga.ld_x = x.ld_q; ga.KT = (int)(m->Kq / kStepBytes);
        ga.want = 1; ga.x_isum = x.isum; ga.x_isq = x.isq; ga.sv_term = m->sv_term_q;
        ga.gs = (m->kernel == RML_KERNEL_RBF ? m->gamma : 1.0) / (m->code_scale * m->code_scale);
        if (p.kmat) rc = launch_gemm<PATH_I8, true>(m, ga, st);
        else if (p.small) rc = launch_small(m, ga, w.gsmall, st);
        else if (p.split) rc = launch_split(m, ga, w.gsplit, ctx->num_cu, st);
        else if (p.big) rc = launch_gemm_big(m, ga, st);
        else rc = launch_gemm<PATH_I8>(m, ga, st);
        if (rc) return rc;
    }
    if (p.run_dig && (rc = launch_gemm_ring<1>(m, digit_args(m, x, p, w), st))) return rc;
    if (p.run_gen) {
        ga.sv = reinterpret_cast<const uint8_t*>(m->sv_f32); ga.ld_sv = m->Df * 4;
        ga.x = reinterpret_cast<const uint8_t*>(x.f32); ga.ld_x = m->Df * 4; ga.KT = (int)(m->Kf * 4 / kStepBytes);
        ga.want = 0; ga.x_nsq = x.nsq; ga.sv_term = m->sv_nsq; ga.gs = m->gamma;
        rc = p.gen_f32 ? launch_gemm<PATH_F32>(m, ga, st)
                       : (p.kmat ? launch_gemm<PATH_F64, true>(m, ga, st) : launch_gemm<PATH_F64>(m, ga, st));
        if (rc) return rc;
    }
    if (p.kmat) { RML_HIP(hipGetLastError()); return RML_OK; }
    return run_finish(m, x, p, w, out, st);
}
}

int rml_svm_pack_host(const double* sv, int64_t M, int64_t D, const double* dual_coef, const int32_t* n_support,
                      int n_classes, int kernel, double gamma, double code_scale, bool has_calib, rml_svm* m, rml_svm_pack* pk) {
    RML_REQUIRE(sv && dual_coef && n_support && m && pk, RML_ERR_INVALID, "rml_svm_load: NULL argument");
    RML_REQUIRE(M > 0 && D > 0, RML_ERR_INVALID, "rml_svm_load: empty model");
    RML_REQUIRE(n_classes >= 2 && n_classes <= kMaxC, RML_ERR_UNSUPPORTED, "rml_svm_load: %d classes (supported: 2..%d)", n_classes, kMaxC);
    RML_REQUIRE(kernel == RML_KERNEL_RBF || kernel == RML_KERNEL_LINEAR, RML_ERR_UNSUPPORTED, "rml_svm_load: kernel %d", kernel);
    int64_t msum = 0;
    for (int c = 0; c < n_classes; ++c) { RML_REQUIRE(n_support[c] >= 0, RML_ERR_INVALID, "rml_svm_load: negative n_support"); msum += n_support[c]; }
    RML_REQUIRE(msum == M, RML_ERR_INVALID, "rml_svm_load: sum(n_support)=%lld != M=%lld", (long long)msum, (long long)M);
    m->M = M; m->D = D; m->C = n_classes; m->P = n_classes * (n_classes - 1) / 2;
    m->PT = m->P <= 1 ? 1 : (m->P <= 3 ? 3 : (m->P <= 6 ? 6 : (m->P <= 10 ? 10 : 15)));
    m->kernel = kernel; m->gamma = gamma; m->code_scale = code_scale > 1.0 ? code_scale : 1.0;
    m->Mpad = round_up(M, kTile);
    m->Kq = round_up(D, kStepBytes); m->Kf = round_up(D, 32);
    m->Dq = ((m->Kq / 128) & 1) ? m->Kq : m->Kq + 128;
    m->Df = ((m->Kf / 32) & 1) ? m->Kf : m->Kf + 32;
    m->has_calib = has_calib;

    std::vector<double>& W = pk->W;
    W.assign((size_t)m->PT * m->Mpad, 0.0);
    {
        std::vector<int64_t> start(n_classes, 0);
        for (int c = 1; c < n_classes; ++c) start[c] = start[c - 1] + n_support[c - 1];
        int p = 0;
        for (int i = 0; i < n_classes; ++i)
            for (int j = i + 1; j < n_classes; ++j, ++p) {
                for (int64_t k = 0; k < n_support[i]; ++k) W[(size_t)p * m->Mpad + start[i] + k] = dual_coef[(size_t)(j - 1) * M + start[i] + k];
                for (int64_t k = 0; k < n_support[j]; ++k) W[(size_t)p * m->Mpad + start[j] + k] = dual_coef[(size_t)i * M + start[j] + k];
            }
    }
    std::vector<float>& svf = pk->svf;
    std::vector<double>& nsq = pk->nsq;
    svf.assign((size_t)m->Mpad * m->Df, 0.0f);
    nsq.assign(m->Mpad, 0.0);
    std::vector<uint8_t>& svq = pk->svq;
    std::vector<double>& term = pk->term;
    svq.assign((size_t)m->Mpad * m->Dq, 0);
    term.assign(m->Mpad, 0.0);
    bool exact = true;
    const float fscale = (float)m->code_scale;
    for (int64_t r = 0; r < M; ++r) {
        double nn = 0.0; int64_t isum = 0, isq = 0;
        for (int64_t d = 0; d < D; ++d) {
            const double v = sv[(size_t)r * D + d];
            const float vf = (float)v;
            svf[(size_t)r * m->Df + d] = vf;
            nn += (double)vf * (double)vf;
            if (exact) {
                double c = nearbyint(v * m->code_scale);
                bool good = c >= 0.0 && c <= 255.0;
                if (good) {
                    double back = m->code_scale > 1.0 ? (double)((float)c / fscale) : c;
                    good = (back == v);
                }
                if (!good) exact = false;
                else { int ci = (int)c; svq[(size_t)r * m->Dq + d] = (uint8_t)(ci ^ 0x80); isum += ci; isq += (int64_t)ci * ci; }
            }
        }
        nsq[r] = nn;
        term[r] = (kernel == RML_KERNEL_RBF) ? (double)(isq - 256 * isum + 32768 * D) : (double)(128 * isum - 16384 * D);
    }
    if (m->Kq >= 131072) exact = false;
    m->exact = exact;
    std::vector<int8_t>& svd = pk->svd;
    std::vector<double>& dnsq = pk->dnsq;
    svd.clear(); dnsq.clear();
    m->dig_ok = false;
    if (kernel == RML_KERNEL_RBF && m->Kq < 32768 && m->PT <= 6) {
        double lo = sv[0], hi = sv[0];
        bool finite = true;
        for (size_t i = 0; i < (size_t)M * D; ++i) { const double v = sv[i]; finite &= std::isfinite(v); lo = v < lo ? v : lo; hi = v > hi ? v : hi; }
        if (finite && hi > lo) {
            int e = 0;
            (void)frexp(hi - lo, &e);
            double sd = ldexp(1.0, e);
            if (ldexp(1.0, e - 1) == hi - lo) sd = hi - lo;
            const double c0 = nearbyint(0.5 * (lo + hi) / sd * 256.0) / 256.0 * sd;
            const double k31 = 2147483648.0 / sd;
            svd.assign((size_t)4 * m->Mpad * m->Dq, 0);
            dnsq.assign(m->Mpad, 0.0);
            const size_t plane = (size_t)m->Mpad * m->Dq;
            bool ok = true;
            for (int64_t r = 0; r < M && ok; ++r) {
                double nn = 0.0;
                for (int64_t d = 0; d < D; ++d) {
                    const double t = nearbyint((sv[(size_t)r * D + d] - c0) * k31);
                    if (!(t >= -2147483648.0 && t <= 2139062143.0)) { ok = false; break; }
                    const int32_t I = (int32_t)t;
                    const double u = (double)I * 0x1p-31;
                    nn += u * u;
                    const uint32_t pk4 = ((uint32_t)I + 0x00808080u) ^ 0x00808080u;
                    for (int dg = 0; dg < 4; ++dg) svd[(size_t)dg * plane + (size_t)r * m->Dq + d] = (int8_t)((pk4 >> (8 * (3 - dg))) & 255u);
                }
                dnsq[r] = nn;
            }
            if (ok) { m->dig_ok = true; m->dig_c0 = c0; m->dig_s = sd; }
        }
    }
    return RML_OK;
}

extern "C" int rml_svm_load(rml_ctx* ctx, const double* sv, int64_t M, int64_t D,
                            const double* dual_coef, const double* intercept, const int32_t* n_support,
                            int n_classes, int kernel, double gamma, double code_scale,
                            const double* calib_a, const double* calib_b, rml_svm** out) {
    RML_REQUIRE(ctx && sv && dual_coef && intercept && n_support && out, RML_ERR_INVALID, "rml_svm_load: NULL argument");
    RML_REQUIRE((calib_a == nullptr) == (calib_b == nullptr), RML_ERR_INVALID, "rml_svm_load: calib_a/calib_b must both be given");
    *out = nullptr;
    rml_svm* m = new (std::nothrow) rml_svm();
    RML_REQUIRE(m != nullptr, RML_ERR_NOMEM, "rml_svm_load: out of host memory");
    rml_svm_pack pk;
    int rc = rml_svm_pack_host(sv, M, D, dual_coef, n_support, n_classes, kernel, gamma, code_scale, calib_a != nullptr, m, &pk);
    if (rc) { delete m; return rc; }
    {
        hipError_t e = hipSetDevice(ctx->device);
        if (e != hipSuccess) { delete m; RML_HIP(e); }
    }
    const bool exact = m->exact;
    do {
        if ((rc = dev_upload(&m->W, pk.W))) break;
        if ((rc = dev_upload(&m->sv_f32, pk.svf))) break;
        if ((rc = dev_upload(&m->sv_nsq, pk.nsq))) break;
        if (exact) {
            if ((rc = dev_upload(&m->sv_q, pk.svq))) break;
            if ((rc = dev_upload(&m->sv_term_q, pk.term))) break;
        }
        if (m->dig_ok) {
            if ((rc = dev_upload(&m->sv_dig, pk.svd))) break;
            if ((rc = dev_upload(&m->sv_dig_nsq, pk.dnsq))) break;
        }
        std::vector<double> ic(intercept, intercept + m->P);
        if ((rc = dev_upload(&m->intercept, ic))) break;
        if (m->has_calib) {
            std::vector<double> cal(2 * n_classes);
            const int ncal = n_classes == 2 ? 1 : n_classes;
            for (int c = 0; c < n_classes; ++c) { cal[c] = c < ncal ? calib_a[c] : 0.0; cal[n_classes + c] = c < ncal ? calib_b[c] : 0.0; }
            if ((rc = dev_upload(&m->calib, cal))) break;
        }
    } while (0);
    if (rc) { rml_svm_free(ctx, m); return rc; }
    *out = m;
    return RML_OK;
}

extern "C" int rml_svm_free(rml_ctx* ctx, rml_svm* m) {
    if (!m) return RML_OK;
    if (ctx) (void)hipSetDevice(ctx->device);
    (void)hipDeviceSynchronize();
    void* bufs[] = {m->sv_f32, m->sv_nsq, m->sv_q, m->sv_term_q, m->W, m->intercept, m->calib, m->platt, m->sv_dig, m->sv_dig_nsq};
    for (void* b : bufs) if (b) (void)hipFree(b);
    delete m;
    return RML_OK;
}

extern "C" int rml_svm_is_exact(const rml_svm* m) { return m && m->exact ? 1 : 0; }
extern "C" int64_t rml_svm_num_sv(const rml_svm* m) { return m ? m->M : 0; }
extern "C" int64_t rml_svm_dim(const rml_svm* m) { return m ? m->D : 0; }

size_t rml_svm_ws_bytes(const rml_svm* m, int64_t CH, unsigned needs) {
    return carve(m, CH, nullptr, ChunkNeeds{(needs & 1u) != 0, (needs & 2u) != 0, (needs & 4u) != 0, (needs & 8u) != 0}).bytes;
}

namespace {
int run_float_rows(const rml_ctx* ctx, const rml_svm* m, const float* feat, int64_t ld_feat, int64_t N, int64_t CH, const ChunkWs& w,
                   const ChunkPlan& plan, const DecisionOut& out, hipStream_t st) {
    for (int64_t r0 = 0; r0 < N; r0 += CH) {
        const int64_t n = std::min(CH, N - r0);
        hipLaunchKernelGGL(k_prepare_rows, dim3((unsigned)n), dim3(256), 0, st, feat + r0 * ld_feat, ld_feat, m->D,
                           (float)m->code_scale, w.f32, m->Df, w.nsq, w.q, m->Dq, w.isum, w.isq, w.flags);
        if (w.dig) launch_digit_rows(m, w, n, st);
        RML_HIP(hipGetLastError());
        ChunkPlan p = plan; if (p.kmat) p.kmat += r0 * p.ld_k;
        if (int rc = run_chunk(ctx, m, ws_rows(m, w, n), p, w, out.at(r0, m->C, m->P), st)) return rc;
    }
    return RML_OK;
}
}

extern "C" int rml_svm_decision(rml_ctx* ctx, const rml_svm* m, int path,
                                const float* feat, int64_t ld_feat,
                                const uint8_t* feat_q, int64_t ld_q, const int32_t* row_isum, const int64_t* row_isq,
                                const int32_t* row_flags, int64_t N,
                                double* dec_ovo, double* dec_ovr, double* proba,
                                int32_t* label_vote, int32_t* label_calib, void* stream) {
    RML_REQUIRE(ctx && m && N >= 0, RML_ERR_INVALID, "rml_svm_decision: bad arguments");
    if (N == 0) return RML_OK;
    RML_REQUIRE(feat || feat_q, RML_ERR_INVALID, "rml_svm_decision: need feat or feat_q");
    RML_REQUIRE(!feat || ld_feat >= m->D, RML_ERR_INVALID, "rml_svm_decision: ld_feat < D");
    RML_REQUIRE(path >= RML_PATH_AUTO && path <= RML_PATH_DIGITS, RML_ERR_INVALID, "rml_svm_decision: bad path %d", path);
    RML_REQUIRE(path != RML_PATH_DIGITS || m->dig_ok, RML_ERR_STATE, "rml_svm_decision: multi-digit path requested but the model has no digit frame "
                "(RBF kernel, D < 32768 and at most 6 class pairs)");
    RML_REQUIRE(!(proba || label_calib) || m->has_calib, RML_ERR_STATE, "rml_svm_decision: model has no calibrators");
    RML_REQUIRE(path != RML_PATH_I8 || m->exact, RML_ERR_STATE, "rml_svm_decision: exact path requested but the model is not on the code grid");
    if (!feat) {
        RML_REQUIRE(m->exact, RML_ERR_STATE, "rml_svm_decision: code rows given but the model is not on the code grid");
        RML_REQUIRE(path == RML_PATH_AUTO || path == RML_PATH_I8, RML_ERR_INVALID, "rml_svm_decision: the float paths need float rows");
        RML_REQUIRE(row_isum && row_isq, RML_ERR_INVALID, "rml_svm_decision: code rows need row_isum/row_isq");
        RML_REQUIRE(ld_q >= m->Kq && ld_q % 16 == 0 && (reinterpret_cast<uintptr_t>(feat_q) & 15) == 0, RML_ERR_INVALID,
                    "rml_svm_decision: code rows need ld_q >= %lld, ld_q %% 16 == 0 and 16-byte alignment", (long long)m->Kq);
    }
    RML_HIP(hipSetDevice(ctx->device));
    hipStream_t st = static_cast<hipStream_t>(stream);
    rml_ctx_guard guard(ctx, st);
    const DecisionOut out{dec_ovo, dec_ovr, proba, label_vote, label_calib};
    ChunkNeeds need{};
    need.q = feat && m->exact && (path == RML_PATH_AUTO || path == RML_PATH_I8); need.f32 = feat != nullptr;
    need.dig = feat && use_dig_gemm(m, path, N, ctx->num_cu);
    const bool dig_rounds = need.dig && !m->exact;
    const int64_t CH = (dig_rounds || m->exact) ? pick_chunk(ctx, m, N, 8192, dig_rounds) : std::min<int64_t>(round_up(N, kTile), 8192);
    ChunkWs w; int rc = reserve_chunks(ctx, m, CH, need, st, &w, 1);
    if (rc) return rc;
    ChunkPlan plan{};
    plan.policy = feat ? path : RML_PATH_I8; plan.allow_big = true; plan.dig_ready = need.dig;
    if (feat) return run_float_rows(ctx, m, feat, ld_feat, N, CH, w, plan, out, st);
    for (int64_t r0 = 0; r0 < N && !rc; r0 += CH) {
        const ChunkOps x{std::min(CH, N - r0), feat_q + r0 * ld_q, ld_q, row_isum + r0, row_isq + r0, row_flags ? row_flags + r0 : nullptr,
                         nullptr, nullptr};
        rc = run_chunk(ctx, m, x, plan, w, out.at(r0, m->C, m->P), st);
    }
    return rc;
}

extern "C" int rml_svm_kernel_matrix(rml_ctx* ctx, const rml_svm* m, int path, const float* feat, int64_t ld_feat, int64_t N,
                                     double* kmat, int64_t ld_k, void* stream) {
    RML_REQUIRE(ctx && m && N >= 0, RML_ERR_INVALID, "rml_svm_kernel_matrix: bad arguments");
    if (N == 0) return RML_OK;
    RML_REQUIRE(feat && kmat, RML_ERR_INVALID, "rml_svm_kernel_matrix: NULL argument");
    RML_REQUIRE(ld_feat >= m->D && ld_k >= m->M, RML_ERR_INVALID, "rml_svm_kernel_matrix: ld_feat < D or ld_k < M");
    RML_REQUIRE(path == RML_PATH_AUTO || path == RML_PATH_I8 || path == RML_PATH_F64, RML_ERR_INVALID,
                "rml_svm_kernel_matrix: path must be AUTO, I8 or F64");
    RML_REQUIRE(path != RML_PATH_I8 || m->exact, RML_ERR_STATE, "rml_svm_kernel_matrix: exact path requested but the model is not on the code grid");
    RML_HIP(hipSetDevice(ctx->device));
    hipStream_t st = static_cast<hipStream_t>(stream);
    rml_ctx_guard guard(ctx, st);
    const int64_t CH = std::min<int64_t>(round_up(N, kTile), 8192);
    ChunkNeeds need{};
    need.q = m->exact && (path == RML_PATH_AUTO || path == RML_PATH_I8); need.f32 = true;
    ChunkWs w; ChunkPlan plan{};
    if (int rc = reserve_chunks(ctx, m, CH, need, st, &w, 1)) return rc;
    plan.policy = path; plan.kmat = kmat; plan.ld_k = ld_k;
    return run_float_rows(ctx, m, feat, ld_feat, N, CH, w, plan, DecisionOut{}, st);
}

namespace {
struct FrontCall {
    rml_ctx* ctx; const rml_svm* m; hipStream_t caller;
    const void* V; int vdtype; int64_t B; int X, Y, Z; int mode; const int32_t* ijk; bool derive; int32_t* ijk_out;
    float scale_div; uint32_t mask; DecisionOut out;
    bool grid_ok;
    int share_cu, q_rmw;
    bool use_dig; ChunkPlan plan;
    bool u8() const { return vdtype == RML_VOL_U8; }
    int64_t frame_bytes() const { return (int64_t)X * Y * Z * (u8() ? 1 : 4); }
    int64_t plane_len(int pl) const { return pl == 0 ? (int64_t)X * Z : (pl == 1 ? (int64_t)Y * Z : (int64_t)X * Y); }
};

ProjOut code_rows_out(const FrontCall& f, const ChunkWs& w) {
    ProjOut o{}; int64_t off = 0;
    for (int pl = 0; pl < 3; ++pl)
        if (f.mask & (1u << pl)) { o.q[pl] = w.q + off; off += f.plane_len(pl); }
    o.sel = f.mask & RML_MASK_ALL;
    o.qstride = f.m->Dq; o.qrow = w.q; o.qD = f.m->D;
    o.row_isum = w.isum; o.row_isq = w.isq; o.row_flags = f.u8() ? nullptr : w.flags; o.scale_div = f.scale_div;
    o.share_cu = f.share_cu; o.q_rmw = f.q_rmw;
    return o;
}
ProjOut float_rows_out(const FrontCall& f, const ChunkWs& w) {
    ProjOut o{}; int64_t off = 0;
    for (int pl = 0; pl < 3; ++pl)
        if (f.mask & (1u << pl)) { o.p[pl] = w.f32 + off; o.stride[pl] = f.m->Df; off += f.plane_len(pl); }
    o.sel = f.mask & RML_MASK_ALL;
    o.scale_div = f.scale_div; o.prow = w.f32; o.pD = f.m->D; o.pstride = f.m->Df; o.row_nsq = w.nsq;
    o.share_cu = f.share_cu;
    return o;
}

int front_single_tile(const FrontCall& f) {
    rml_ctx* ctx = f.ctx; const rml_svm* m = f.m; hipStream_t st = f.caller;
    const int S = (f.vdtype == RML_VOL_F32 && f.mode == RML_MODE_MAX && f.B <= 64) ? rml_project_split_pieces(f.X, f.Y, f.Z) : 0;
    const size_t sbytes = S ? ((rml_project_split_scratch_bytes(f.B, f.X, f.Y, f.Z, S) + 255) & ~(size_t)255) : 0;
    ChunkNeeds need{};
    need.q = true; need.f32 = !f.u8();
    ChunkWs w; void* scratch = nullptr;
    int rc = reserve_chunks(ctx, m, kTile, need, st, &w, 1, sbytes, &scratch);
    if (rc) return rc;
    const ProjOut o = code_rows_out(f, w);
    rc = S ? rml_launch_project_split(ctx, f.V, f.vdtype, f.B, f.X, f.Y, f.Z, o, static_cast<float*>(scratch), S, st)
           : rml_launch_project(ctx, f.V, f.vdtype, f.B, f.X, f.Y, f.Z, f.mode, f.ijk, o, st);
    if (rc) return rc;
    const ChunkOps x = ws_rows(m, w, f.B);
    ChunkPlan plan{};
    plan.policy = f.u8() ? RML_PATH_I8 : RML_PATH_AUTO; plan.tiles_done = true; plan.all_exact_known = f.u8();
    if (f.u8()) return run_chunk(ctx, m, x, plan, w, f.out, st);
    launch_tile_flags(m, x, plan_chunk(ctx, m, plan, x, w), w, w.all_exact, st);
    ProjOut of = float_rows_out(f, w);
    of.skip_if_set = w.all_exact;
    rc = rml_launch_project(ctx, f.V, f.vdtype, f.B, f.X, f.Y, f.Z, f.mode, f.ijk, of, st);
    return rc ? rc : run_chunk(ctx, m, x, plan, w, f.out, st);
}

struct FrontChunk {
    int64_t r0, n; const ChunkWs& w; hipEvent_t ev_proj; const void* V; const int32_t* ijk; int32_t* ijkd;
};

int caller_stage(const FrontCall& f, const FrontChunk& ck, const ProjOut& po) {
    rml_prof_mark(f.ctx, f.caller);
    const int rc = f.derive ? rml_launch_derive_slice(f.ctx, ck.V, f.vdtype, ck.n, f.X, f.Y, f.Z, 1, ck.ijkd, nullptr, po, f.caller)
                            : rml_launch_project(f.ctx, ck.V, f.vdtype, ck.n, f.X, f.Y, f.Z, f.mode, ck.ijk, po, f.caller);
    rml_prof_mark(f.ctx, f.caller);
    if (f.ctx->profiling) f.ctx->prof_frames += ck.n;
    if (rc) return rc;
    if (f.use_dig) { launch_digit_rows(f.m, ck.w, ck.n, f.caller); RML_HIP(hipGetLastError()); }
    RML_HIP(hipEventRecord(ck.ev_proj, f.caller));
    RML_HIP(hipStreamWaitEvent(f.ctx->aux_stream, ck.ev_proj, 0));
    return RML_OK;
}
int gemm_stage(const FrontCall& f, const FrontChunk& ck) {
    hipStream_t aux = f.ctx->aux_stream;
    rml_prof_mark_gemm(f.ctx, aux);
    const int rc = run_chunk(f.ctx, f.m, ws_rows(f.m, ck.w, ck.n), f.plan, ck.w, f.out.at(ck.r0, f.m->C, f.m->P), aux);
    rml_prof_mark_gemm(f.ctx, aux);
    if (f.ctx->profiling) f.ctx->prof_ops_g += 2.0 * (double)ck.n * (double)f.m->M * (double)f.m->D;
    return rc;
}

int chunk_u8(const FrontCall& f, const FrontChunk& ck) {
    const int rc = caller_stage(f, ck, code_rows_out(f, ck.w));
    return rc ? rc : gemm_stage(f, ck);
}

int chunk_on_grid(const FrontCall& f, const FrontChunk& ck) {
    int rc = caller_stage(f, ck, code_rows_out(f, ck.w));
    if (rc) return rc;
    const ChunkOps x = ws_rows(f.m, ck.w, ck.n); hipStream_t aux = f.ctx->aux_stream;
    launch_tile_flags(f.m, x, plan_chunk(f.ctx, f.m, f.plan, x, ck.w), ck.w, ck.w.all_exact, aux);
    ProjOut of = float_rows_out(f, ck.w);
    of.no_pad = 1; of.skip_if_set = ck.w.all_exact;
    rc = rml_launch_project(f.ctx, ck.V, f.vdtype, ck.n, f.X, f.Y, f.Z, f.derive ? RML_MODE_SLICE : f.mode, f.derive ? ck.ijkd : ck.ijk, of, aux);
    return rc ? rc : gemm_stage(f, ck);
}

int chunk_off_grid(const FrontCall& f, const FrontChunk& ck) {
    ProjOut of = float_rows_out(f, ck.w);
    of.row_flags = ck.w.flags;
    const int rc = caller_stage(f, ck, of);
    return rc ? rc : gemm_stage(f, ck);
}

int front_chunked(FrontCall f) {
    rml_ctx* ctx = f.ctx; const rml_svm* m = f.m;
    const bool wave_proj = f.derive || rml_project_uses_wave_kernel(ctx, f.vdtype, f.mode, f.X, f.Y, f.Z, true, std::min<int64_t>(f.B, 8192));
    f.use_dig = !f.grid_ok && !f.u8() && use_dig_gemm(m, RML_PATH_AUTO, f.B, ctx->num_cu);
    f.share_cu = 1;
    f.q_rmw = ctx->opt.code_rmw >= 0 ? ctx->opt.code_rmw : rml_code_rmw(m->D, f.frame_bytes(), f.derive, f.u8());
    const bool u8_exact = f.grid_ok && f.u8();
    f.plan.policy = u8_exact ? RML_PATH_I8 : (f.grid_ok ? RML_PATH_AUTO : RML_PATH_F64);
    f.plan.tiles_done = f.grid_ok;
    f.plan.all_exact_known = u8_exact; f.plan.allow_big = !wave_proj; f.plan.dig_ready = f.use_dig;
    const int64_t small_chunk = (f.u8() && (int64_t)f.X * f.Y * f.Z <= 200000) ? 16384
                                : (f.derive && !f.u8() && f.frame_bytes() <= (1 << 20)) ? 12288 : 8192;
    const int64_t CH = (f.grid_ok && !wave_proj) ? pick_chunk(ctx, m, f.B, small_chunk, false)
                       : f.use_dig               ? pick_chunk(ctx, m, f.B, 8192, f.use_dig)
                                                 : std::min<int64_t>(round_up(f.B, kTile), f.grid_ok ? pick_chunk_opt(ctx, small_chunk) : 8192);
    ChunkNeeds need{};
    need.q = f.grid_ok; need.f32 = true; need.dig = f.use_dig; need.ijk = f.derive && !f.ijk_out;
    constexpr int NBUF = 2;
    ChunkWs w2[NBUF];
    int rc = reserve_chunks(ctx, m, CH, need, f.caller, w2, NBUF);
    if (rc) return rc;
    RML_HIP(hipEventRecord(ctx->ev_fork, f.caller));
    RML_HIP(hipStreamWaitEvent(ctx->aux_stream, ctx->ev_fork, 0));
    int64_t c = 0;
    for (int64_t r0 = 0; r0 < f.B; r0 += CH, ++c) {
        const int b = (int)(c % NBUF);
        if (c >= NBUF) RML_HIP(hipStreamWaitEvent(f.caller, ctx->ev_done[b], 0));
        const FrontChunk ck{r0, std::min(CH, f.B - r0), w2[b], ctx->ev_proj[b], static_cast<const unsigned char*>(f.V) + r0 * f.frame_bytes(),
                            f.ijk ? f.ijk + r0 * 3 : nullptr, f.derive ? (f.ijk_out ? f.ijk_out + r0 * 3 : w2[b].ijk) : nullptr};
        rc = !f.grid_ok ? chunk_off_grid(f, ck) : (f.u8() ? chunk_u8(f, ck) : chunk_on_grid(f, ck));
        if (rc) return rc;
        RML_HIP(hipEventRecord(ctx->ev_done[b], ctx->aux_stream));
    }
    RML_HIP(hipEventRecord(ctx->ev_join, ctx->aux_stream));
    RML_HIP(hipStreamWaitEvent(f.caller, ctx->ev_join, 0));
    return RML_OK;
}

int project_svm_front(rml_ctx* ctx, const rml_svm* m, const void* V, int vdtype, int64_t B, int X, int Y, int Z,
                      int mode, const int32_t* ijk, bool derive, int32_t* ijk_out, float scale_div, uint32_t mask,
                      const DecisionOut& out, void* stream) {
    RML_REQUIRE(ctx && m && B >= 0, RML_ERR_INVALID, "rml_project_svm: bad arguments");
    if (B == 0) return RML_OK;
    RML_REQUIRE(V != nullptr, RML_ERR_INVALID, "rml_project_svm: V is NULL");
    RML_REQUIRE(vdtype == RML_VOL_F32 || vdtype == RML_VOL_U8, RML_ERR_INVALID, "rml_project_svm: unknown volume dtype %d", vdtype);
    RML_REQUIRE(rml_feature_len(X, Y, Z, mask) == m->D, RML_ERR_INVALID, "rml_project_svm: grid/mask give D=%lld, model has D=%lld",
                (long long)rml_feature_len(X, Y, Z, mask), (long long)m->D);
    RML_REQUIRE(!(out.proba || out.label_calib) || m->has_calib, RML_ERR_STATE, "rml_project_svm: model has no calibrators");
    RML_REQUIRE(mode != RML_MODE_SLICE || ijk || derive, RML_ERR_INVALID, "rml_project_svm: mode SLICE needs ijk");
    if (mode == RML_MODE_MAX_NAN) mode = RML_MODE_MAX;
    const bool scaled = scale_div > 1.0f;
    const bool grid_ok = m->exact && ((scaled && (double)scale_div == m->code_scale) || (!scaled && m->code_scale == 1.0));
    RML_HIP(hipSetDevice(ctx->device));
    hipStream_t caller = static_cast<hipStream_t>(stream);
    rml_ctx_guard guard(ctx, caller);
    const FrontCall f{ctx, m, caller, V, vdtype, B, X, Y, Z, mode, ijk, derive, ijk_out, scale_div, mask, out, grid_ok};
    if (B <= kTile && grid_ok && !derive && (mode == RML_MODE_MAX || (mode == RML_MODE_SLICE && ijk))) return front_single_tile(f);
    return front_chunked(f);
}
}

extern "C" int rml_project_svm(rml_ctx* ctx, const rml_svm* m, const void* V, int vdtype, int64_t B, int X, int Y, int Z,
                               int mode, const int32_t* ijk, float scale_div, uint32_t mask,
                               double* dec_ovo, double* dec_ovr, double* proba,
                               int32_t* label_vote, int32_t* label_calib, void* stream) {
    return project_svm_front(ctx, m, V, vdtype, B, X, Y, Z, mode, ijk, false, nullptr, scale_div, mask,
                             DecisionOut{dec_ovo, dec_ovr, proba, label_vote, label_calib}, stream);
}

extern "C" int rml_derive_project_svm(rml_ctx* ctx, const rml_svm* m, const void* V, int vdtype, int64_t B, int X, int Y, int Z,
// ... 157 lines not shown
```

radar-ml_amd/csrc/svm_tile.h:

```cpp
#pragma once
#include "mfma_tile.h"
#include "svm_epilogue.h"
#include <type_traits>

namespace {

struct GemmArgs {
    const uint8_t* sv; int64_t ld_sv;
    const uint8_t* x;  int64_t ld_x;
    int KT;
    int64_t N;
    int ST, FT;
    const int32_t* tile_exact; int want;
    const int32_t* x_isum; const int64_t* x_isq;
    const double* x_nsq;
    const double* sv_term;
    const double* W; int64_t Mpad;
    double gs;
    int kernel;
    double* partial; int64_t Npart;
    double* kmat; int64_t ld_k; int64_t M;
    int64_t sv_rows;
};

template <int PATH, int PT, bool KM = false>
__global__ __launch_bounds__(256, 2) void k_svm_gemm(GemmArgs a) {
    extern __shared__ __align__(16) unsigned char smem[];
    const int tid = threadIdx.x, lane = tid & 63, wave = tid >> 6;
    const int wr = wave >> 1, wc = wave & 1;
    const int id = blockIdx.x;
    const int xcd = id & 7, slot = id >> 3;
    const int XPX = (a.FT + 7) >> 3;
    const int ftile = (slot % XPX) * 8 + xcd;
    const int stile = slot / XPX;
    if (ftile >= a.FT) return;
    if (a.tile_exact && a.tile_exact[ftile] != a.want) return;
    const int64_t f0 = (int64_t)ftile * kTile;
    const int64_t m0 = (int64_t)stile * kTile;

    double* svw = reinterpret_cast<double*>(smem + 4 * kTileBytes);
    const double* etab = load_sv_table<PT, kTile, 256, false>(svw, a.sv_term, a.W, a.Mpad, m0, tid);

    auto store_k = [&](int64_t n, int ml, double kv) {
        if constexpr (KM) {
            const int64_t mg = (int64_t)stile * kTile + ml;
            if (n < a.N && mg < a.M) a.kmat[n * a.ld_k + mg] = kv;
        }
    };

    if constexpr (PATH == PATH_F64) {
        const uint8_t* gsv[4];
        const uint8_t* gx[4];
#pragma unroll
        for (int q = 0; q < 4; ++q) {
            int s = (wave * 4 + q) * 64 + lane;
            int r = s >> 3;
            int c = (s & 7) ^ ((r >> 1) & 7);
            gsv[q] = a.sv + (m0 + r) * a.ld_sv + c * 16;
            int64_t xr = f0 + r; xr = xr < a.N ? xr : a.N - 1;
            gx[q] = a.x + xr * a.ld_x + c * 16;
        }
        auto stage = [&](int kt, int buf) {
            unsigned char* base = smem + buf * 2 * kTileBytes;
            const int64_t ko = (int64_t)kt * kStepBytes;
#pragma unroll
            for (int q = 0; q < 4; ++q) {
                glds16(gsv[q] + ko, base + (wave * 4 + q) * 1024);
                glds16(gx[q] + ko, base + kTileBytes + (wave * 4 + q) * 1024);
            }
        };
        v4d accd[4][4];
        zero_acc(accd);
        int doff_a[4], dsw_a[4], doff_b[4], dsw_b[4];
#pragma unroll
        for (int t = 0; t < 4; ++t) {
            int ra = wr * 64 + t * 16 + (lane & 15);
            int rb = wc * 64 + t * 16 + (lane & 15);
            doff_a[t] = ra * kStepBytes; dsw_a[t] = (ra >> 1) & 7;
            doff_b[t] = rb * kStepBytes; dsw_b[t] = (rb >> 1) & 7;
// ... 26 lines not shown
                            accd[i][j] = __builtin_amdgcn_mfma_f64_16x16x4f64(ad[i], bd[j], accd[i][j], 0, 0, 0);
                }
            }
        }

        const bool rbf = (a.kernel == RML_KERNEL_RBF);
        double* gd = reinterpret_cast<double*>(smem);
        const int nq = tid & 63, qd = tid >> 6;
        for (int pass = 0; pass < 2; ++pass) {
            __syncthreads();
            if (wc == pass) {
#pragma unroll
                for (int i = 0; i < 4; ++i)
#pragma unroll
                    for (int j = 0; j < 4; ++j)
#pragma unroll
                        for (int r = 0; r < 4; ++r) {
                            const int ml = cd64_row(wr * 64 + i * 16, r, lane);
                            const int nl = cd64_col(j * 16, lane);
                            gd[ml * 64 + nl] = accd[i][j][r];
                        }
            }
            __syncthreads();
            const int64_t n = f0 + pass * 64 + nq;
            const int64_t nc = n < a.N ? n : a.N - 1;
            const double xt = rbf ? a.x_nsq[nc] : 0.0;
            double S[PT];
#pragma unroll
            for (int p = 0; p < PT; ++p) S[p] = 0.0;
#pragma unroll 2
            for (int mm = 0; mm < 32; ++mm) {
                const int ml = qd * 32 + mm;
                const double* e = svw + ml * (1 + PT);
                const double kv = kernel_value<false>(rbf, gd[ml * 64 + nq], xt, e[0], a.gs, etab);
                store_k(n, ml, kv);
                chain_link<PT>(S, e + 1, 1, kv);
            }
            __syncthreads();
            double* x4 = gd;
#pragma unroll
            for (int p = 0; p < PT; ++p) x4[(qd * 64 + nq) * PT + p] = S[p];
            __syncthreads();
            if (qd == 0 && n < a.N) {
#pragma unroll
                for (int p = 0; p < PT; ++p) {
                    double t = x4[(0 * 64 + nq) * PT + p] + x4[(1 * 64 + nq) * PT + p];
                    t += x4[(2 * 64 + nq) * PT + p] + x4[(3 * 64 + nq) * PT + p];
                    a.partial[((int64_t)stile * a.Npart + n) * PT + p] = t;
                }
            }
        }
    } else {
        using acc_t = typename std::conditional<PATH == PATH_I8, v16i, v16f>::type;
        TileStager sg;
        sg.init<true>(a.sv, a.ld_sv, m0, a.x, a.ld_x, f0, a.N, wave, lane);
        Frag32<2> fa, fb;
        fa.init(wr * 64, lane); fb.init(wc * 64, lane);
        const int chalf = lane >> 5;
        acc_t acc[2][2];
        zero_acc(acc);
        auto ks32 = [&](const unsigned char* sA, const unsigned char* sB) { kstep_32<PATH>(acc, sA, sB, fa, fb, chalf); };
        tile_k_loop(sg, smem, 0, a.KT, ks32);

        const bool rbf = (a.kernel == RML_KERNEL_RBF);
        __syncthreads();
        {
            int* gl = reinterpret_cast<int*>(smem);
#pragma unroll
            for (int i = 0; i < 2; ++i)
#pragma unroll
                for (int j = 0; j < 2; ++j)
#pragma unroll
                    for (int r = 0; r < 16; ++r) {
                        const int ml = cd32_row(wr * 64 + i * 32, r, lane);
                        const int nl = cd32_col(wc * 64 + j * 32, lane);
                        int bits;
                        if constexpr (PATH == PATH_I8) bits = acc[i][j][r]; else bits = __float_as_int(acc[i][j][r]);
                        gl[ml * kTile + nl] = bits;
                    }
        }
        __syncthreads();
        const int nl = tid & 127, h = tid >> 7;
        int64_t n = f0 + nl;
        const int64_t nc = n < a.N ? n : a.N - 1;
        double xt;
        if constexpr (PATH == PATH_I8) xt = exact_sample_term(rbf, a.x_isum, a.x_isq, nc);
        else xt = rbf ? a.x_nsq[nc] : 0.0;
        double S[PT];
        const int* gcol = reinterpret_cast<const int*>(smem) + nl;
        chain_run<PT, 64, PATH == PATH_I8>(S, svw, h * 64, rbf, xt, a.gs, etab,
                                          [&](int ml) {
                                              const int bits = gcol[ml * kTile];
                                              return (PATH == PATH_I8) ? (double)bits : (double)__int_as_float(bits);
                                          },
                                          [&](int ml, double kv) { store_k(n, ml, kv); });
        double* xch = reinterpret_cast<double*>(smem);
        __syncthreads();
        if (h == 1) {
#pragma unroll
            for (int p = 0; p < PT; ++p) xch[nl * PT + p] = S[p];
        }
        __syncthreads();
        if (h == 0 && n < a.N) {
#pragma unroll
            for (int p = 0; p < PT; ++p) a.partial[((int64_t)stile * a.Npart + n) * PT + p] = S[p] + xch[nl * PT + p];
        }
    }
}

__global__ __launch_bounds__(256) void k_zero16(v4i* p, int64_t n16) {
    const int64_t i = (int64_t)blockIdx.x * 256 + threadIdx.x;
    if (i < n16) p[i] = v4i{0, 0, 0, 0};
}

struct SplitArgs {
    const uint8_t* sv; int64_t ld_sv;
    const uint8_t* x; int64_t ld_x;
    int KT, per;
    int64_t N; int FT;
    const int32_t* tile_exact;
    int32_t* G; int64_t ldg;
};

__global__ __launch_bounds__(256, 2) void k_svm_gemm_splitk(SplitArgs a) {
    __shared__ __align__(16) unsigned char smem[4 * kTileBytes];
    const int tid = threadIdx.x, lane = tid & 63, wave = tid >> 6;
    const int wr = wave >> 1, wc = wave & 1;
    const int ftile = blockIdx.x % a.FT, stile = blockIdx.x / a.FT;
    if (a.tile_exact && a.tile_exact[ftile] != 1) return;
    const int kt0 = blockIdx.y * a.per;
    const int kt1 = a.KT < kt0 + a.per ? a.KT : kt0 + a.per;
    if (kt0 >= kt1) return;
    const int64_t f0 = (int64_t)ftile * kTile, m0 = (int64_t)stile * kTile;
    TileStager sg;
    sg.init<true>(a.sv, a.ld_sv, m0, a.x, a.ld_x, f0, a.N, wave, lane);
    Frag32<2> fa, fb;
    fa.init(wr * 64, lane); fb.init(wc * 64, lane);
    const int chalf = lane >> 5;
    v16i acc[2][2];
    zero_acc(acc);
    auto ks = [&](const unsigned char* sA, const unsigned char* sB) { kstep_i8_plain(acc, sA, sB, fa, fb, chalf); };
    tile_k_loop(sg, smem, kt0, kt1, ks);
#pragma unroll
    for (int i = 0; i < 2; ++i)
#pragma unroll
        for (int j = 0; j < 2; ++j)
#pragma unroll
            for (int r = 0; r < 16; ++r) {
                const int ml = cd32_row(wr * 64 + i * 32, r, lane);
                const int nl = cd32_col(wc * 64 + j * 32, lane);
                __hip_atomic_fetch_add(a.G + (m0 + ml) * a.ldg + f0 + nl, acc[i][j][r], __ATOMIC_RELAXED, __HIP_MEMORY_SCOPE_AGENT);
            }
}

template <int PATH, bool KM = false>
int launch_gemm(const rml_svm* m, const GemmArgs& ga, hipStream_t st) {
    const size_t lds = 4 * kTileBytes + (size_t)kTile * (1 + m->PT) * sizeof(double) + kExpTabBytes;
    const int FT8 = (ga.FT + 7) / 8 * 8;
    dim3 grid((unsigned)(FT8 * ga.ST)), block(256);
#define RML_GEMM_CASE(PTV)                                                                                         \
    case PTV: {                                                                                                    \
        RML_MAX_DYN_LDS(144 * 1024, &k_svm_gemm<PATH, PTV, KM>);                                                   \
        hipLaunchKernelGGL((k_svm_gemm<PATH, PTV, KM>), grid, block, lds, st, ga);                                 \
    } break;
    switch (m->PT) {
        RML_GEMM_CASE(1)
        RML_GEMM_CASE(3)
        RML_GEMM_CASE(6)
        RML_GEMM_CASE(10)
        RML_GEMM_CASE(15)
        default: RML_REQUIRE(false, RML_ERR_UNSUPPORTED, "svm: unsupported pair count");
    }
#undef RML_GEMM_CASE
    RML_HIP(hipGetLastError());
    return RML_OK;
}

}
```

Before: 2.886 million frames/s.

## Skip loading all-background code lines in SVM GEMM using occupancy bitmaps

The projection pass now records, per frame, a bitmap of which 128-byte code lines contain non-background values, and the SVM build computes the same bitmap for the support vectors. A sparse variant of the i8 MFMA GEMM reads these bitmaps into LDS and, for empty lines, stages a shared constant background line instead of loading from HBM. This is meant to cut global memory traffic for sparse radar projections. It adds atomic ORs in LDS during projection, extra workspace and LDS for the bitmaps, and a heuristic gate that decides when the path is used.

```diff
diff --git a/include/radarml.h b/include/radarml.h
--- a/include/radarml.h
+++ b/include/radarml.h
@@ -67,6 +67,7 @@
 #define RML_OPT_CONV7 13
 #define RML_CONV7_DEFAULT 3
 #define RML_OPT_ZOOM_ROWS 14
+#define RML_OPT_SPARSE_ROWS 15
 int rml_ctx_set_option(rml_ctx* ctx, int option, int value);
 int rml_ctx_get_option(const rml_ctx* ctx, int option, int* value);
 
@@ -80,6 +81,12 @@
 int rml_probe_stream(rml_ctx* ctx, const void* buf, int64_t bytes, int reps, double* gb_per_s, void* stream);
 
 int rml_code_rmw_default(int64_t D, int64_t frame_bytes, int derive, int u8);
+
+int rml_svm_sv_occupancy(rml_ctx* ctx, const rml_svm* m, uint32_t* out, int64_t n_words);
+int rml_project_occupancy(rml_ctx* ctx, const void* V, int vdtype, int64_t B, int X, int Y, int Z, int mode, float scale_div,
+                          uint32_t mask, uint8_t* feat_q, int64_t ld_q, int32_t* row_isum, int64_t* row_isq, int32_t* row_flags,
+                          uint32_t* occ, int occ_words, void* stream);
+int64_t rml_ctx_sparse_gemm_launches(const rml_ctx* ctx);
 
 int64_t rml_feature_len(int X, int Y, int Z, uint32_t mask);
 
diff --git a/radar-ml_amd/_lib.py b/radar-ml_amd/_lib.py
--- a/radar-ml_amd/_lib.py
+++ b/radar-ml_amd/_lib.py
@@ -181,19 +181,24 @@
     "rml_augment_chain": (c_int, [c_void_p, c_int, c_void_p, c_int64, c_int64, c_int, c_int, c_float, c_float, c_float, c_float, c_void_p,
                                   c_void_p, c_void_p]),
     "rml_code_rmw_default": (c_int, [c_int64, c_int64, c_int, c_int]),
+    "rml_ctx_sparse_gemm_launches": (c_int64, [c_void_p]),
+    "rml_svm_sv_occupancy": (c_int, [c_void_p, c_void_p, c_void_p, c_int64]),
+    "rml_project_occupancy": (c_int, [c_void_p, c_void_p, c_int, c_int64, c_int, c_int, c_int, c_int, c_float, c_uint32, c_void_p, c_int64,
+                                      c_void_p, c_void_p, c_void_p, c_void_p, c_int, c_void_p]),
     "rml_probe_stream": (c_int, [c_void_p, c_void_p, c_int64, c_int, c_void_p, c_void_p]),
     "rml_synth_volumes": (c_int, [c_void_p, c_uint64, c_int64, c_int64, c_int, c_int, c_int, c_int, c_void_p, c_void_p,
                                   c_void_p]),
 }
 
 MODE_MAX, MODE_SLICE, MODE_SUM, MODE_MAX_NAN = 0, 1, 2, 3
-OPT_PROJECT_SHARE_CU, OPT_WAVEFRAME, OPT_LINPLANE, OPT_STAGE_CODES, OPT_SLICE_WAVE, OPT_DERIVE_FUSED, OPT_CODE_RMW, OPT_GEMM_BIG, OPT_CHUNK, OPT_C1_PK, OPT_SMO_LDS_ROWS, OPT_SGD_RESIDENT_D, OPT_CONV7, OPT_ZOOM_ROWS = range(1, 15)
+OPT_PROJECT_SHARE_CU, OPT_WAVEFRAME, OPT_LINPLANE, OPT_STAGE_CODES, OPT_SLICE_WAVE, OPT_DERIVE_FUSED, OPT_CODE_RMW, OPT_GEMM_BIG, OPT_CHUNK, OPT_C1_PK, OPT_SMO_LDS_ROWS, OPT_SGD_RESIDENT_D, OPT_CONV7, OPT_ZOOM_ROWS, OPT_SPARSE_ROWS = range(1, 16)
 OPTIONS = {"project_share_cu": OPT_PROJECT_SHARE_CU, "waveframe": OPT_WAVEFRAME, "linplane": OPT_LINPLANE, "stage_codes": OPT_STAGE_CODES,
            "slice_wave": OPT_SLICE_WAVE, "derive_fused": OPT_DERIVE_FUSED, "code_rmw": OPT_CODE_RMW, "gemm_big": OPT_GEMM_BIG,
            "chunk": OPT_CHUNK, "c1_pk": OPT_C1_PK}
 SOLVER_OPTIONS = {"smo_lds_rows": OPT_SMO_LDS_ROWS, "sgd_resident_d": OPT_SGD_RESIDENT_D}
 NN_OPTIONS = {"conv7": OPT_CONV7}
 ZOOM_OPTIONS = {"zoom_rows": OPT_ZOOM_ROWS}
+SVM_OPTIONS = {"sparse_rows": OPT_SPARSE_ROWS}
 SMO_LDS_ROWS_MAX = 2768
 SGD_RESIDENT_D_MAX = 10240
 SGD_MAX_ROWS = 8192
@@ -203,7 +208,7 @@
 ENV_OPTIONS = {"RML_WAVE_SHARE": "project_share_cu", "RML_WAVEFRAME": "waveframe", "RML_LINPLANE": "linplane", "RML_STAGE_CODES": "stage_codes",
                "RML_SLICE_WAVE": "slice_wave", "RML_DERIVE_FUSED": "derive_fused", "RML_CODE_RMW": "code_rmw", "RML_GEMM_BIG": "gemm_big",
                "RML_CHUNK": "chunk", "RML_C1_PK": "c1_pk", "RML_SMO_LDS_ROWS": "smo_lds_rows", "RML_SGD_RESIDENT_D": "sgd_resident_d",
-               "RML_CONV7": "conv7"}
+               "RML_CONV7": "conv7", "RML_SPARSE_ROWS": "sparse_rows"}
 AUG_ROTATE, AUG_ZOOM, AUG_NOISE = 0, 1, 2
 CHAIN_ROTATE, CHAIN_ZOOM, CHAIN_NOISE = 1, 2, 4
 VOL_F32, VOL_U8 = 0, 1
@@ -216,7 +221,7 @@
 
 def option_id(name):
     name = name.lower()
-    for table in (OPTIONS, SOLVER_OPTIONS, ZOOM_OPTIONS):
+    for table in (OPTIONS, SOLVER_OPTIONS, ZOOM_OPTIONS, SVM_OPTIONS):
         if name in table:
             return table[name]
     return NN_OPTIONS[name]
diff --git a/radar-ml_amd/csrc/context.hip b/radar-ml_amd/csrc/context.hip
--- a/radar-ml_amd/csrc/context.hip
+++ b/radar-ml_amd/csrc/context.hip
@@ -158,7 +158,10 @@
         e = hipEventCreateWithFlags(&c->ev_proj[i], hipEventDisableTiming);
         if (e == hipSuccess) e = hipEventCreateWithFlags(&c->ev_done[i], hipEventDisableTiming);
     }
+    if (e == hipSuccess) e = hipMalloc(reinterpret_cast<void**>(&c->bg_line), 128);
+    if (e == hipSuccess) e = hipMemset(c->bg_line, 0x80, 128);
     if (e != hipSuccess) {
+        if (c->bg_line) (void)hipFree(c->bg_line);
         delete c;
         return rml_hip_fail(e, "stream/event creation", __FILE__, __LINE__);
     }
@@ -188,6 +191,7 @@
     for (const rml_resize_tab& t : ctx->resize_tabs) (void)hipFree(const_cast<double*>(t.kk));
     for (const rml_pre_tab& t : ctx->pre_tabs) (void)hipFree(t.dev);
     if (ctx->aux_stream) (void)hipStreamDestroy(ctx->aux_stream);
+    if (ctx->bg_line) (void)hipFree(ctx->bg_line);
     delete ctx;
     if (prev >= 0) (void)hipSetDevice(prev);
     return RML_OK;
@@ -285,6 +289,7 @@
         case RML_OPT_CODE_RMW: return &o.code_rmw;
         case RML_OPT_GEMM_BIG: return &o.gemm_big;
         case RML_OPT_C1_PK: return &o.c1_pk;
+        case RML_OPT_SPARSE_ROWS: return &o.sparse_rows;
         default: return nullptr;
     }
 }
@@ -323,7 +328,7 @@
     RML_REQUIRE(slot != nullptr, RML_ERR_INVALID, "rml_ctx_set_option: unknown option %d", option);
     switch (option) {
         case RML_OPT_WAVEFRAME: RML_REQUIRE(value >= 0 && value <= 3, RML_ERR_INVALID, "rml_ctx_set_option: RML_OPT_WAVEFRAME is 0..3"); *slot = value; break;
-        case RML_OPT_CODE_RMW: case RML_OPT_GEMM_BIG: *slot = value < 0 ? -1 : (value ? 1 : 0); break;
+        case RML_OPT_CODE_RMW: case RML_OPT_GEMM_BIG: case RML_OPT_SPARSE_ROWS: *slot = value < 0 ? -1 : (value ? 1 : 0); break;
         default: *slot = value ? 1 : 0;
     }
     return RML_OK;
diff --git a/radar-ml_amd/csrc/mfma_tile.h b/radar-ml_amd/csrc/mfma_tile.h
--- a/radar-ml_amd/csrc/mfma_tile.h
+++ b/radar-ml_amd/csrc/mfma_tile.h
@@ -66,6 +66,66 @@
     }
 }
 
+constexpr int kSparseMaxWords = 8;
+struct SparseStager {
+    const uint8_t* ga[4];
+    const uint8_t* gb[4];
+    const uint8_t* bg;
+    const uint32_t* la;
+    uint32_t ca[4], cb[4];
+    int wave, ow;
+    static __device__ __forceinline__ void fill(uint32_t* occ_l, const uint32_t* a_occ, int64_t a0, const uint32_t* b_occ, int64_t b0,
+                                                int64_t b_rows, int ow, int tid) {
+        int64_t gr = b0 + (tid - kTile);
+        gr = gr < b_rows ? gr : b_rows - 1;
+        const uint32_t* src = tid < kTile ? a_occ + (a0 + tid) * ow : b_occ + gr * ow;
+        for (int w = 0; w < ow; ++w) occ_l[tid * ow + w] = src[w];
+    }
+    __device__ __forceinline__ void init(const uint8_t* a, int64_t lda, int64_t a0, const uint8_t* b, int64_t ldb, int64_t b0, int64_t b_rows,
+                                         const uint32_t* occ_l, int ow_, const uint8_t* bg_line, int wave_, int lane) {
+        wave = wave_; ow = ow_;
+        bg = bg_line + (lane & 7) * 16;
+        la = occ_l + (((wave * 4) * 64 + lane) >> 3) * ow;
+#pragma unroll
+        for (int q = 0; q < 4; ++q) {
+            ga[q] = stage_src<false>(a, lda, a0, 0, wave, q, lane);
+            gb[q] = stage_src<true>(b, ldb, b0, b_rows, wave, q, lane);
+        }
+    }
+    __device__ __forceinline__ void take(int blk) {
+#pragma unroll
+        for (int q = 0; q < 4; ++q) {
+            ca[q] = la[q * 8 * ow + blk];
+            cb[q] = la[(kTile + q * 8) * ow + blk];
+        }
+    }
+    __device__ __forceinline__ void stage(unsigned char* smem, int kt, int buf) {
+        unsigned char* base = smem + buf * 2 * kTileBytes;
+        const int64_t ko = (int64_t)kt * kStepBytes;
+#pragma unroll
+        for (int q = 0; q < 4; ++q) {
+            glds16((ca[q] & 1u) ? ga[q] + ko : bg, base + (wave * 4 + q) * 1024);
+            glds16((cb[q] & 1u) ? gb[q] + ko : bg, base + kTileBytes + (wave * 4 + q) * 1024);
+            ca[q] >>= 1; cb[q] >>= 1;
+        }
+    }
+};
+
+template <class KStep>
+__device__ __forceinline__ void tile_k_loop_sparse(SparseStager& sg, unsigned char* smem, int KT, KStep kstep) {
+    sg.take(0);
+    sg.stage(smem, 0, 0);
+    for (int kt = 0; kt < KT; ++kt) {
+        __syncthreads();
+        if (kt + 1 < KT) {
+            if (((kt + 1) & 31) == 0) sg.take((kt + 1) >> 5);
+            sg.stage(smem, kt + 1, (kt + 1) & 1);
+        }
+        const unsigned char* sA = smem + (kt & 1) * 2 * kTileBytes;
+        kstep(sA, sA + kTileBytes);
+    }
+}
+
 template <int T>
 struct Frag32 {
     int off[T], sw[T];
diff --git a/radar-ml_amd/csrc/project.hip b/radar-ml_amd/csrc/project.hip
--- a/radar-ml_amd/csrc/project.hip
+++ b/radar-ml_amd/csrc/project.hip
@@ -317,6 +317,8 @@
     const size_t mine = (size_t)4 * NY * 68 * sizeof(float);
     pp.stage_bytes = code_stage_bytes(pp, sizeof(VT));
     if (mine + (size_t)4 * pp.stage_bytes > 160 * 1024) pp.stage_bytes = 0;
+    if (!pp.stage_bytes) pp.o.occ = nullptr;
+    else if (pp.o.occ && pp.occ_done) *pp.occ_done = 1;
     const size_t stage = (size_t)4 * pp.stage_bytes;
     int per_cu = pp.o.share_cu ? 1 : per_cu_max;
     if (per_cu * (mine + stage) > 160 * 1024) per_cu = 1;
@@ -564,7 +566,7 @@
 
 void fill_params(ProjParams& pp, const rml_ctx* ctx, const void* V, int64_t B, int X, int Y, int Z, const int32_t* ijk, const ProjOut& o) {
     pp.V = V; pp.B = B; pp.X = X; pp.Y = Y; pp.Z = Z; pp.ZQ = Z / 4; pp.ijk = ijk; pp.tpf = 1; pp.rpl = 1; pp.o = o;
-    pp.ntgt = 1; pp.ijk_out = nullptr; pp.profiles = nullptr; pp.wave_lds = 0; pp.stage_bytes = 0;
+    pp.ntgt = 1; pp.ijk_out = nullptr; pp.profiles = nullptr; pp.wave_lds = 0; pp.stage_bytes = 0; pp.occ_done = nullptr;
     const rml_opts def;
     const rml_opts& op = ctx ? ctx->opt : def;
     pp.k_waveframe = op.waveframe; pp.k_linplane = op.linplane; pp.k_stage_codes = op.stage_codes; pp.k_slice_wave = op.slice_wave;
@@ -593,6 +595,13 @@
 }
 }
 
+namespace {
+__global__ __launch_bounds__(256) void k_fill_u32(uint32_t* p, int64_t n, uint32_t v) {
+    const int64_t i = (int64_t)blockIdx.x * 256 + threadIdx.x;
+    if (i < n) p[i] = v;
+}
+}
+
 bool rml_project_uses_wave_kernel(const rml_ctx* ctx, int vdtype, int mode, int X, int Y, int Z, bool share_cu, int64_t B) {
     (void)X;
     const int num_cu = ctx ? ctx->num_cu : 256, knob = ctx ? ctx->opt.waveframe : 1;
@@ -607,12 +616,20 @@
     RML_REQUIRE(vdtype == RML_VOL_F32 || vdtype == RML_VOL_U8, RML_ERR_INVALID, "rml_project: unknown volume dtype %d", vdtype);
     if (mode == RML_MODE_MAX_NAN) mode = RML_MODE_MAX;
     RML_REQUIRE(targets_per_frame == 1 || mode == RML_MODE_SLICE, RML_ERR_INVALID, "rml_project: several targets per frame only in mode SLICE");
+    RML_REQUIRE(!o.occ || (o.qrow && (int64_t)o.occ_words * 32 >= (o.qD + 127) / 128), RML_ERR_INVALID,
+                "rml_project: occupancy words need code rows and a bit per 128-byte line");
     ProjParams pp;
     fill_params(pp, ctx, V, B, X, Y, Z, ijk, o);
     pp.tpf = targets_per_frame;
+    int occ_done = 0;
+    pp.occ_done = &occ_done;
     const int num_cu = !ctx ? 256 : ctx->num_cu;
     const int rc = vdtype == RML_VOL_U8 ? launch_project_t<uint8_t>(pp, mode, num_cu, st) : launch_project_t<float>(pp, mode, num_cu, st);
     if (rc) return rc;
+    if (o.occ && !occ_done) {
+        const int64_t n = B * o.occ_words;
+        hipLaunchKernelGGL(k_fill_u32, dim3((unsigned)((n + 255) / 256)), dim3(256), 0, st, o.occ, n, 0xFFFFFFFFu);
+    }
     RML_HIP(hipGetLastError());
     return RML_OK;
 }
@@ -851,6 +868,26 @@
     return rml_launch_project(ctx, V, vdtype, B, X, Y, Z, mode, ijk, o, static_cast<hipStream_t>(stream), tpf);
 }
 
+extern "C" int rml_project_occupancy(rml_ctx* ctx, const void* V, int vdtype, int64_t B, int X, int Y, int Z, int mode, float scale_div,
+                                     uint32_t mask, uint8_t* feat_q, int64_t ld_q, int32_t* row_isum, int64_t* row_isq, int32_t* row_flags,
+                                     uint32_t* occ, int occ_words, void* stream) {
+    RML_REQUIRE(ctx && B >= 0 && X > 0 && Y > 0 && Z > 0, RML_ERR_INVALID, "rml_project_occupancy: bad arguments");
+    if (B == 0) return RML_OK;
+    RML_REQUIRE(V && feat_q && occ, RML_ERR_INVALID, "rml_project_occupancy: NULL argument");
+    RML_REQUIRE(mode == RML_MODE_MAX || mode == RML_MODE_SUM || mode == RML_MODE_MAX_NAN, RML_ERR_INVALID, "rml_project_occupancy: mode MAX or SUM");
+    RML_REQUIRE((mask & RML_MASK_ALL) != 0, RML_ERR_INVALID, "rml_project_occupancy: empty projection mask");
+    RML_REQUIRE(B < (int64_t)1 << 31, RML_ERR_UNSUPPORTED, "rml_project_occupancy: B too large for one launch");
+    const int64_t D = rml_feature_len(X, Y, Z, mask);
+    RML_REQUIRE(ld_q >= D && ld_q % 128 == 0 && (reinterpret_cast<uintptr_t>(feat_q) & 127) == 0, RML_ERR_INVALID,
+                "rml_project_occupancy: code rows need ld_q >= D, ld_q %% 128 == 0 and 128-byte alignment");
+    RML_REQUIRE(occ_words == (int)(((D + 127) / 128 + 31) / 32), RML_ERR_INVALID, "rml_project_occupancy: occ_words must be ceil(ceil(D / 128) / 32)");
+    RML_HIP(hipSetDevice(ctx->device));
+    ProjOut o{};
+    rows_out(o, X, Y, Z, mask, scale_div, nullptr, 0, feat_q, ld_q, row_isum, row_isq, row_flags);
+    o.occ = occ; o.occ_words = occ_words;
+    return rml_launch_project(ctx, V, vdtype, B, X, Y, Z, mode, nullptr, o, static_cast<hipStream_t>(stream));
+}
+
 extern "C" int rml_project_planes(rml_ctx* ctx, const void* V, int vdtype, int64_t B, int X, int Y, int Z, int mode,
                                   const int32_t* ijk, float* xz, float* yz, float* xy, void* stream) {
     RML_REQUIRE(ctx && B >= 0 && X > 0 && Y > 0 && Z > 0, RML_ERR_INVALID, "rml_project_planes: bad arguments");
diff --git a/radar-ml_amd/csrc/project_lin.hip b/radar-ml_amd/csrc/project_lin.hip
--- a/radar-ml_amd/csrc/project_lin.hip
+++ b/radar-ml_amd/csrc/project_lin.hip
@@ -136,6 +136,8 @@
     constexpr size_t kMaxLds = 160 * 1024;
     const size_t images = (size_t)4 * (NI * 64 * 16 + NI * NGRP * 64 * 4);
     if (images + (size_t)4 * pp.stage_bytes > kMaxLds) pp.stage_bytes = 0;
+    if (!pp.stage_bytes) pp.o.occ = nullptr;
+    else if (pp.o.occ && pp.occ_done) *pp.occ_done = 1;
     const size_t mine = images + (size_t)4 * pp.stage_bytes;
     int per_cu = pp.o.share_cu ? 1 : 2;
     if (per_cu * mine > 160 * 1024) per_cu = 1;
diff --git a/radar-ml_amd/csrc/project_shared.h b/radar-ml_amd/csrc/project_shared.h
--- a/radar-ml_amd/csrc/project_shared.h
+++ b/radar-ml_amd/csrc/project_shared.h
@@ -23,6 +23,7 @@
     int wave_lds;
     int stage_bytes;
     int k_waveframe, k_linplane, k_stage_codes, k_slice_wave, k_derive_fused;
+    int* occ_done;
 };
 
 template <int MODE> struct Op;
@@ -79,7 +80,20 @@
     lds_u8* stage = nullptr;
     int staged = 0;
     int stage_xy = 0;
-    __device__ __forceinline__ void set_stage(unsigned char* p, int xy_off) { stage = (lds_u8*)p; staged = 1; stage_xy = xy_off; }
+    int occ_on = 0;
+    int occ_off = 0;
+    __device__ __forceinline__ void set_stage(unsigned char* p, int xy_off) {
+        stage = (lds_u8*)p; staged = 1; stage_xy = xy_off;
+        if (a.o.occ) {
+            occ_on = 1; occ_off = xy_off + ((a.X * a.Y + 15) & ~15);
+            for (int w = threadIdx.x & 63; w < a.o.occ_words; w += 64) *(lds_u32*)(stage + occ_off + 4 * w) = 0u;
+        }
+    }
+    __device__ __forceinline__ void occ_mark(int at) {
+        const int k = at >> 7;
+        __hip_atomic_fetch_or((lds_u32*)(stage + occ_off + 4 * (k >> 5)), 1u << (k & 31), __ATOMIC_RELAXED, __HIP_MEMORY_SCOPE_WAVEFRONT);
+    }
+    __device__ __forceinline__ int plane_at(int pl) const { return (int)(a.o.q[pl] - a.o.qrow); }
 
     __device__ Emitter(const ProjParams& a_, int64_t b_) : a(a_), b(b_) {
         want_stats = a.o.row_isum || a.o.row_isq || a.o.row_flags || a.o.q[0] || a.o.q[1] || a.o.q[2];
@@ -112,7 +126,10 @@
             uint32_t c = code(v);
             if (a.o.q[pl]) {
                 if (staged && pl != 1) stage[(pl == 2 ? stage_xy : 0) + idx] = (uint8_t)c;
-                else a.o.q[pl][b * a.o.qstride + idx] = (uint8_t)c;
+                else {
+                    a.o.q[pl][b * a.o.qstride + idx] = (uint8_t)c;
+                    if (occ_on && c != 0x80u) occ_mark(plane_at(pl) + (int)idx);
+                }
             }
         }
     }
@@ -160,6 +177,7 @@
                 else {
                     uint32_t* dq = reinterpret_cast<uint32_t*>(a.o.q[pl] + qb() * a.o.qstride + idx);
                     if (!rmw || (have_old ? old : *dq) != packed) *dq = packed;
+                    if (occ_on && packed != 0x80808080u) occ_mark(plane_at(pl) + (int)idx);
                 }
             }
         }
@@ -171,20 +189,41 @@
         const int len[2] = {a.X * a.Z, a.X * a.Y};
         lds_u8* src[2] = {stage, stage + stage_xy};
         uint8_t* dst[2] = {a.o.q[0] + qb() * a.o.qstride, a.o.q[2] + qb() * a.o.qstride};
+        const int at[2] = {occ_on ? plane_at(0) : 0, occ_on ? plane_at(2) : 0};
 #pragma unroll
         for (int r = 0; r < 2; ++r) {
             int done = 0;
             if ((reinterpret_cast<uintptr_t>(dst[r]) & 15) == 0) {
                 for (int i = lane; i < (len[r] >> 4); i += 64) {
-                    reinterpret_cast<u32x4*>(dst[r])[i] = ((lds_u128*)src[r])[i];
+                    const u32x4 v = ((lds_u128*)src[r])[i];
+                    reinterpret_cast<u32x4*>(dst[r])[i] = v;
+                    if (occ_on && ((v.x ^ 0x80808080u) | (v.y ^ 0x80808080u) | (v.z ^ 0x80808080u) | (v.w ^ 0x80808080u))) occ_mark(at[r] + 16 * i);
                 }
                 done = len[r] & ~15;
             }
-            for (int i = done + 4 * lane; i + 4 <= len[r]; i += 256)
-                *reinterpret_cast<uint32_t*>(dst[r] + i) = *(lds_u32*)(src[r] + i);
-            for (int i = (len[r] & ~3) + lane; i < len[r]; i += 64) dst[r][i] = src[r][i];
+            for (int i = done + 4 * lane; i + 4 <= len[r]; i += 256) {
+                const uint32_t v = *(lds_u32*)(src[r] + i);
+                *reinterpret_cast<uint32_t*>(dst[r] + i) = v;
+                if (occ_on && v != 0x80808080u) occ_mark(at[r] + i);
+            }
+            for (int i = (len[r] & ~3) + lane; i < len[r]; i += 64) {
+                const uint8_t v = src[r][i];
+                dst[r][i] = v;
+                if (occ_on && v != 0x80u) occ_mark(at[r] + i);
+            }
         }
         __builtin_amdgcn_fence(__ATOMIC_ACQ_REL, "wavefront");
+        if (occ_on) {
+            const int kpad = (int)(a.o.qD >> 7);
+            for (int w = lane; w < a.o.occ_words; w += 64) {
+                lds_u32* lw = (lds_u32*)(stage + occ_off + 4 * w);
+                uint32_t v = *lw;
+                if ((a.o.qD & 127) && (kpad >> 5) == w) v |= 1u << (kpad & 31);
+                a.o.occ[qb() * a.o.occ_words + w] = v;
+                *lw = 0u;
+            }
+            __builtin_amdgcn_fence(__ATOMIC_ACQ_REL, "wavefront");
+        }
     }
     __device__ void finish_wave(int lane) {
         if (a.o.qrow) {
@@ -310,7 +349,7 @@
     const ProjOut& o = pp.o;
     if (voxel_bytes != 4 || o.p[0] || o.p[1] || o.p[2] || o.row_nsq || !o.q[0] || !o.q[2] || o.skip_if_set) return 0;
     if (!pp.k_stage_codes) return 0;
-    const int bytes = ((pp.X * pp.Z + 15) & ~15) + ((pp.X * pp.Y + 15) & ~15);
+    const int bytes = ((pp.X * pp.Z + 15) & ~15) + ((pp.X * pp.Y + 15) & ~15) + (o.occ ? (4 * o.occ_words + 15) & ~15 : 0);
     return bytes <= 16 * 1024 ? bytes : 0;
 }
 
diff --git a/radar-ml_amd/csrc/rml_internal.h b/radar-ml_amd/csrc/rml_internal.h
--- a/radar-ml_amd/csrc/rml_internal.h
+++ b/radar-ml_amd/csrc/rml_internal.h
@@ -34,6 +34,7 @@
     int smo_lds_rows = RML_SMO_LDS_ROWS_MAX;
     int conv7 = RML_CONV7_DEFAULT;
     int sgd_resident_d = RML_SGD_RESIDENT_D_MAX;
+    int sparse_rows = -1;
     int zoom_rows = 0;
 };
 
@@ -52,6 +53,8 @@
     hipEvent_t ev_fork = nullptr, ev_join = nullptr;
     hipEvent_t ev_proj[2] = {nullptr, nullptr}, ev_done[2] = {nullptr, nullptr};
     hipStream_t aux_stream = nullptr;
+    mutable int64_t sparse_gemm_launches = 0;
+    uint8_t* bg_line = nullptr;
     bool profiling = false;
     std::vector<hipEvent_t> prof_ev;
     size_t prof_used = 0;
@@ -146,10 +149,16 @@
     int share_cu;
     int no_pad;
     int q_rmw;
+    uint32_t* occ;
+    int occ_words;
 };
 inline int rml_code_rmw(int64_t D, int64_t frame_bytes, bool derive, bool u8) {
     if (derive) return 0;
     return u8 && D * 64 >= frame_bytes && D * 16 <= frame_bytes;
+}
+
+inline int rml_sparse_rows(int X, int Y, int Z) {
+    return (Z % 128 == 0 || 128 % Z == 0) && ((int64_t)X * Z) % 128 == 0 && ((int64_t)Y * Z) % 128 == 0;
 }
 
 bool rml_project_uses_wave_kernel(const rml_ctx* ctx, int vdtype, int mode, int X, int Y, int Z, bool share_cu, int64_t B);
@@ -204,6 +213,8 @@
     int8_t* sv_dig = nullptr;
     double* sv_dig_nsq = nullptr;
     uint32_t mask_hint = 0;
+    uint32_t* sv_occ = nullptr;
+    int occ_words = 0;
 };
 
 struct rml_svm_pack {
@@ -211,6 +222,7 @@
     std::vector<float> svf;
     std::vector<uint8_t> svq;
     std::vector<int8_t> svd;
+    std::vector<uint32_t> occ;
 };
 int rml_svm_pack_host(const double* sv, int64_t M, int64_t D, const double* dual_coef, const int32_t* n_support,
                       int n_classes, int kernel, double gamma, double code_scale, bool has_calib, rml_svm* m, rml_svm_pack* pk);
diff --git a/radar-ml_amd/csrc/svm.hip b/radar-ml_amd/csrc/svm.hip
--- a/radar-ml_amd/csrc/svm.hip
+++ b/radar-ml_amd/csrc/svm.hip
@@ -85,10 +85,11 @@
     int32_t* ijk;
     int32_t* gsmall;
     int32_t* gsplit;
+    uint32_t* occ;
     size_t bytes;
 };
 
-struct ChunkNeeds { bool q, f32, dig, ijk; };
+struct ChunkNeeds { bool q, f32, dig, ijk, occ; };
 constexpr int64_t kSplitRows = 2048;
 
 ChunkWs carve(const rml_svm* m, int64_t CH, unsigned char* base, const ChunkNeeds& need) {
@@ -107,6 +108,7 @@
     w.ijk = (int32_t*)take(need.ijk ? (size_t)CH * 12 : 0);
     w.gsmall = (int32_t*)take(need.q ? (size_t)RML_SMALL_FRAMES * m->Mpad * 4 : 0);
     w.gsplit = (int32_t*)take(need.q && CH <= kSplitRows ? (size_t)m->Mpad * CH * 4 : 0);
+    w.occ = (uint32_t*)take(need.q && need.occ ? (size_t)CH * m->occ_words * 4 : 0);
     w.bytes = off;
     return w;
 }
@@ -130,8 +132,9 @@
     }
 };
 
-struct ChunkOps { int64_t n; const uint8_t* q; int64_t ld_q; const int32_t* isum; const int64_t* isq; const int32_t* flags; const float* f32; const double* nsq; };
-ChunkOps ws_rows(const rml_svm* m, const ChunkWs& w, int64_t n) { return ChunkOps{n, w.q, m->Dq, w.isum, w.isq, w.flags, w.f32, w.nsq}; }
+struct ChunkOps { int64_t n; const uint8_t* q; int64_t ld_q; const int32_t* isum; const int64_t* isq; const int32_t* flags; const float* f32; const double* nsq;
+                  const uint32_t* occ; };
+ChunkOps ws_rows(const rml_svm* m, const ChunkWs& w, int64_t n) { return ChunkOps{n, w.q, m->Dq, w.isum, w.isq, w.flags, w.f32, w.nsq, nullptr}; }
 
 struct ChunkPlan {
     int policy;
@@ -140,7 +143,7 @@
     bool allow_big;
     bool dig_ready;
     double* kmat; int64_t ld_k;
-    int FT, ST, group; bool run_i8, run_gen, gen_f32, big, run_dig, small, split;
+    int FT, ST, group; bool run_i8, run_gen, gen_f32, big, run_dig, small, split, sparse;
 };
 
 ChunkPlan plan_chunk(const rml_ctx* ctx, const rml_svm* m, ChunkPlan p, const ChunkOps& x, const ChunkWs& w) {
@@ -153,6 +156,10 @@
     p.small = p.run_i8 && !p.kmat && x.n <= RML_SMALL_FRAMES && w.gsmall && (m->Mpad % kSmallSv) == 0;
     p.split = p.run_i8 && !p.kmat && !p.small && !p.big && w.gsplit && x.n <= kSplitRows && (int64_t)p.FT * p.ST < ctx->num_cu &&
               m->Kq / kStepBytes >= 8;
+    const bool can_sparse = p.run_i8 && !p.kmat && !p.small && !p.big && x.occ && m->sv_occ && ctx->bg_line && ctx->opt.sparse_rows != 0 &&
+                            m->occ_words <= kSparseMaxWords;
+    if (can_sparse && ctx->opt.sparse_rows > 0) p.split = false;
+    p.sparse = can_sparse && !p.split;
     return p;
 }
 
@@ -254,7 +261,11 @@
         else if (p.small) rc = launch_small(m, ga, w.gsmall, st);
         else if (p.split) rc = launch_split(m, ga, w.gsplit, ctx->num_cu, st);
         else if (p.big) rc = launch_gemm_big(m, ga, st);
-        else rc = launch_gemm<PATH_I8>(m, ga, st);
+        else if (p.sparse) {
+            ga.sv_occ = m->sv_occ; ga.x_occ = x.occ; ga.ow = m->occ_words; ga.bg_line = ctx->bg_line;
+            ++ctx->sparse_gemm_launches;
+            rc = launch_gemm<PATH_I8, false, true>(m, ga, st);
+        } else rc = launch_gemm<PATH_I8>(m, ga, st);
         if (rc) return rc;
     }
     if (p.run_dig && (rc = launch_gemm_ring<1>(m, digit_args(m, x, p, w), st))) return rc;
@@ -332,6 +343,15 @@
         nsq[r] = nn;
         term[r] = (kernel == RML_KERNEL_RBF) ? (double)(isq - 256 * isum + 32768 * D) : (double)(128 * isum - 16384 * D);
     }
+    m->occ_words = (int)((m->Kq / kStepBytes + 31) / 32);
+    std::vector<uint32_t>& occ = pk->occ;
+    occ.assign((size_t)m->Mpad * m->occ_words, 0u);
+    for (int64_t r = 0; r < m->Mpad; ++r)
+        for (int64_t k = 0; k < m->Kq / kStepBytes; ++k) {
+            bool bg = r < M && (k + 1) * kStepBytes <= D;
+            for (int t = 0; bg && t < kStepBytes; ++t) bg = svq[(size_t)r * m->Dq + k * kStepBytes + t] == 0x80;
+            if (!bg) occ[(size_t)r * m->occ_words + (k >> 5)] |= 1u << (k & 31);
+        }
     if (m->Kq >= 131072) exact = false;
     m->exact = exact;
     std::vector<int8_t>& svd = pk->svd;
@@ -396,6 +416,7 @@
         if (exact) {
             if ((rc = dev_upload(&m->sv_q, pk.svq))) break;
             if ((rc = dev_upload(&m->sv_term_q, pk.term))) break;
+            if ((rc = dev_upload(&m->sv_occ, pk.occ))) break;
         }
         if (m->dig_ok) {
             if ((rc = dev_upload(&m->sv_dig, pk.svd))) break;
@@ -419,18 +440,28 @@
     if (!m) return RML_OK;
     if (ctx) (void)hipSetDevice(ctx->device);
     (void)hipDeviceSynchronize();
-    void* bufs[] = {m->sv_f32, m->sv_nsq, m->sv_q, m->sv_term_q, m->W, m->intercept, m->calib, m->platt, m->sv_dig, m->sv_dig_nsq};
+    void* bufs[] = {m->sv_f32, m->sv_nsq, m->sv_q, m->sv_term_q, m->W, m->intercept, m->calib, m->platt, m->sv_dig, m->sv_dig_nsq, m->sv_occ};
     for (void* b : bufs) if (b) (void)hipFree(b);
     delete m;
     return RML_OK;
 }
 
+extern "C" int rml_svm_sv_occupancy(rml_ctx* ctx, const rml_svm* m, uint32_t* out, int64_t n_words) {
+    RML_REQUIRE(ctx && m && out, RML_ERR_INVALID, "rml_svm_sv_occupancy: NULL argument");
+    RML_REQUIRE(m->sv_occ != nullptr, RML_ERR_STATE, "rml_svm_sv_occupancy: the model is not on the code grid");
+    RML_REQUIRE(n_words == m->Mpad * m->occ_words, RML_ERR_INVALID, "rml_svm_sv_occupancy: out holds %lld words, the model has %lld",
+                (long long)n_words, (long long)(m->Mpad * m->occ_words));
+    RML_HIP(hipSetDevice(ctx->device));
+    RML_HIP(hipMemcpy(out, m->sv_occ, (size_t)n_words * sizeof(uint32_t), hipMemcpyDeviceToHost));
+    return RML_OK;
+}
+extern "C" int64_t rml_ctx_sparse_gemm_launches(const rml_ctx* ctx) { return ctx ? ctx->sparse_gemm_launches : 0; }
 extern "C" int rml_svm_is_exact(const rml_svm* m) { return m && m->exact ? 1 : 0; }
 extern "C" int64_t rml_svm_num_sv(const rml_svm* m) { return m ? m->M : 0; }
 extern "C" int64_t rml_svm_dim(const rml_svm* m) { return m ? m->D : 0; }
 
 size_t rml_svm_ws_bytes(const rml_svm* m, int64_t CH, unsigned needs) {
-    return carve(m, CH, nullptr, ChunkNeeds{(needs & 1u) != 0, (needs & 2u) != 0, (needs & 4u) != 0, (needs & 8u) != 0}).bytes;
+    return carve(m, CH, nullptr, ChunkNeeds{(needs & 1u) != 0, (needs & 2u) != 0, (needs & 4u) != 0, (needs & 8u) != 0, (needs & 16u) != 0}).bytes;
 }
 
 namespace {
@@ -521,6 +552,7 @@
     float scale_div; uint32_t mask; DecisionOut out;
     bool grid_ok;
     int share_cu, q_rmw;
+    bool occ;
     bool use_dig; ChunkPlan plan;
     bool u8() const { return vdtype == RML_VOL_U8; }
     int64_t frame_bytes() const { return (int64_t)X * Y * Z * (u8() ? 1 : 4); }
@@ -535,6 +567,7 @@
     o.qstride = f.m->Dq; o.qrow = w.q; o.qD = f.m->D;
     o.row_isum = w.isum; o.row_isq = w.isq; o.row_flags = f.u8() ? nullptr : w.flags; o.scale_div = f.scale_div;
     o.share_cu = f.share_cu; o.q_rmw = f.q_rmw;
+    if (f.occ && w.occ) { o.occ = w.occ; o.occ_words = f.m->occ_words; }
     return o;
 }
 ProjOut float_rows_out(const FrontCall& f, const ChunkWs& w) {
@@ -590,7 +623,9 @@
 int gemm_stage(const FrontCall& f, const FrontChunk& ck) {
     hipStream_t aux = f.ctx->aux_stream;
     rml_prof_mark_gemm(f.ctx, aux);
-    const int rc = run_chunk(f.ctx, f.m, ws_rows(f.m, ck.w, ck.n), f.plan, ck.w, f.out.at(ck.r0, f.m->C, f.m->P), aux);
+    ChunkOps x = ws_rows(f.m, ck.w, ck.n);
+    if (f.occ) x.occ = ck.w.occ;
+    const int rc = run_chunk(f.ctx, f.m, x, f.plan, ck.w, f.out.at(ck.r0, f.m->C, f.m->P), aux);
     rml_prof_mark_gemm(f.ctx, aux);
     if (f.ctx->profiling) f.ctx->prof_ops_g += 2.0 * (double)ck.n * (double)f.m->M * (double)f.m->D;
     return rc;
@@ -635,7 +670,9 @@
                        : f.use_dig               ? pick_chunk(ctx, m, f.B, 8192, f.use_dig)
                                                  : std::min<int64_t>(round_up(f.B, kTile), f.grid_ok ? pick_chunk_opt(ctx, small_chunk) : 8192);
     ChunkNeeds need{};
-    need.q = f.grid_ok; need.f32 = true; need.dig = f.use_dig; need.ijk = f.derive && !f.ijk_out;
+    f.occ = f.grid_ok && !f.derive && f.mode != RML_MODE_SLICE && ctx->opt.sparse_rows != 0 &&
+            (ctx->opt.sparse_rows > 0 || (wave_proj && !f.u8() && rml_sparse_rows(f.X, f.Y, f.Z)));
+    need.q = f.grid_ok; need.f32 = true; need.dig = f.use_dig; need.ijk = f.derive && !f.ijk_out; need.occ = f.occ;
     constexpr int NBUF = 2;
     ChunkWs w2[NBUF];
     int rc = reserve_chunks(ctx, m, CH, need, f.caller, w2, NBUF);
diff --git a/radar-ml_amd/csrc/svm_tile.h b/radar-ml_amd/csrc/svm_tile.h
--- a/radar-ml_amd/csrc/svm_tile.h
+++ b/radar-ml_amd/csrc/svm_tile.h
@@ -21,10 +21,12 @@
     double* partial; int64_t Npart;
     double* kmat; int64_t ld_k; int64_t M;
     int64_t sv_rows;
+    const uint32_t* sv_occ; const uint32_t* x_occ; int ow; const uint8_t* bg_line;
 };
 
-template <int PATH, int PT, bool KM = false>
+template <int PATH, int PT, bool KM = false, bool SPARSE = false>
 __global__ __launch_bounds__(256, 2) void k_svm_gemm(GemmArgs a) {
+    static_assert(!SPARSE || (PATH == PATH_I8 && !KM), "occupancy words exist for code rows only");
     extern __shared__ __align__(16) unsigned char smem[];
     const int tid = threadIdx.x, lane = tid & 63, wave = tid >> 6;
     const int wr = wave >> 1, wc = wave & 1;
@@ -157,15 +159,24 @@
         }
     } else {
         using acc_t = typename std::conditional<PATH == PATH_I8, v16i, v16f>::type;
-        TileStager sg;
-        sg.init<true>(a.sv, a.ld_sv, m0, a.x, a.ld_x, f0, a.N, wave, lane);
         Frag32<2> fa, fb;
         fa.init(wr * 64, lane); fb.init(wc * 64, lane);
         const int chalf = lane >> 5;
         acc_t acc[2][2];
         zero_acc(acc);
         auto ks32 = [&](const unsigned char* sA, const unsigned char* sB) { kstep_32<PATH>(acc, sA, sB, fa, fb, chalf); };
-        tile_k_loop(sg, smem, 0, a.KT, ks32);
+        if constexpr (SPARSE) {
+            uint32_t* occ_l = reinterpret_cast<uint32_t*>(smem + 4 * kTileBytes + kTile * (1 + PT) * sizeof(double) + kExpTabBytes);
+            SparseStager::fill(occ_l, a.sv_occ, m0, a.x_occ, f0, a.N, a.ow, tid);
+            __syncthreads();
+            SparseStager sg;
+            sg.init(a.sv, a.ld_sv, m0, a.x, a.ld_x, f0, a.N, occ_l, a.ow, a.bg_line, wave, lane);
+            tile_k_loop_sparse(sg, smem, a.KT, ks32);
+        } else {
+            TileStager sg;
+            sg.init<true>(a.sv, a.ld_sv, m0, a.x, a.ld_x, f0, a.N, wave, lane);
+            tile_k_loop(sg, smem, 0, a.KT, ks32);
+        }
 
         const bool rbf = (a.kernel == RML_KERNEL_RBF);
         __syncthreads();
@@ -258,15 +269,15 @@
             }
 }
 
-template <int PATH, bool KM = false>
+template <int PATH, bool KM = false, bool SPARSE = false>
 int launch_gemm(const rml_svm* m, const GemmArgs& ga, hipStream_t st) {
-    const size_t lds = 4 * kTileBytes + (size_t)kTile * (1 + m->PT) * sizeof(double) + kExpTabBytes;
+    const size_t lds = 4 * kTileBytes + (size_t)kTile * (1 + m->PT) * sizeof(double) + kExpTabBytes + (SPARSE ? (size_t)2 * kTile * ga.ow * 4 : 0);
     const int FT8 = (ga.FT + 7) / 8 * 8;
     dim3 grid((unsigned)(FT8 * ga.ST)), block(256);
 #define RML_GEMM_CASE(PTV)                                                                                         \
     case PTV: {                                                                                                    \
-        RML_MAX_DYN_LDS(144 * 1024, &k_svm_gemm<PATH, PTV, KM>);                                                   \
-        hipLaunchKernelGGL((k_svm_gemm<PATH, PTV, KM>), grid, block, lds, st, ga);                                 \
+        RML_MAX_DYN_LDS(144 * 1024, &k_svm_gemm<PATH, PTV, KM, SPARSE>);                                           \
+        hipLaunchKernelGGL((k_svm_gemm<PATH, PTV, KM, SPARSE>), grid, block, lds, st, ga);                         \
     } break;
     switch (m->PT) {
         RML_GEMM_CASE(1)
```

Result: faster. 3.000 million frames/s (median of 6 runs) (+4.0%).
